# rll/rllab

Hardware: AMD Instinct MI355X
Metric: env steps/sec over full TRPO iterations (sample + process + update), 4096 envs per MI355X (higher is better)
Workload: dtype f32

## Files before the change

include/rllab_amd.h:

```cpp
#ifndef RLLAB_AMD_H
#define RLLAB_AMD_H

#include <stddef.h>
#include <stdint.h>

#ifdef __cplusplus
extern "C" {
#endif

enum rl_env_kind {
    RL_ENV_CARTPOLE = 0,
    RL_ENV_DOUBLE_PENDULUM = 1,
    RL_ENV_SWIMMER = 2,
    RL_ENV_HALF_CHEETAH = 3,
    RL_ENV_CARTPOLE_SWINGUP = 4,
    RL_ENV_WALKER2D = 5,
    RL_ENV_HOPPER = 6,
    RL_ENV_INVERTED_DOUBLE_PENDULUM = 7
};

enum rl_status {
    RL_OK = 0,
    RL_ERR_ARG = -1,
    RL_ERR_UNSUPPORTED = -2,
// ... 59 lines not shown
    double* reward_mean;
    double* reward_var;
    double obs_alpha, reward_alpha;
    int32_t normalize_obs, normalize_reward;
} rl_running_norm;

typedef struct rl_launch_opts {
    int32_t rollout_epw;
    int32_t rollout_wpb;
    int32_t swimmer_lane_kernel;
    int32_t swimmer_coop;
    int32_t two_leg_lane_kernel;
    int32_t two_leg_wave_kernel;
    int32_t fvp_split;
    int32_t fvp_split_wps;
    int32_t lfb_valu;
    int32_t reserved[7];
} rl_launch_opts;

typedef struct rl_rollout_args {
    int32_t kind;
    int32_t n_envs;
    int32_t horizon;
    int32_t max_path_length;
    int32_t normalize;
    int32_t reset_at_start;
    int32_t hidden0, hidden1;
    int32_t hidden2;
    int32_t env_offset;
    float scale_reward;
    float log_min_std;
    uint64_t seed;
    uint64_t step_counter;
    float* state;
    int32_t* ts;
    const float* theta;
    const float* eps;
    const float* reset_draws;
    float* obs;
    float* actions;
    float* means;
    float* rewards;
    uint8_t* dones;
    float* last_obs;
    const rl_env_cfg* cfg;
    const float* theta_std;
    float* log_stds;
    int32_t std_hidden0, std_hidden1, std_hidden2;
    int32_t layer_activations;
    const rl_launch_opts* opts;
    const rl_running_norm* norm;
    int32_t std_layer_activations;
    int32_t reserved_tail;
} rl_rollout_args;

int rl_rollout_gaussian_mlp(const rl_rollout_args* args, void* stream);

enum rl_rollout_kernel {
    RL_ROLLOUT_UNSUPPORTED = 0,
    RL_ROLLOUT_GENERIC = 1,
    RL_ROLLOUT_WIDE = 2,
    RL_ROLLOUT_DUAL = 3,
    RL_ROLLOUT_SWIMMER_QUAD = 4,
    RL_ROLLOUT_SWIMMER_QUAD_WIDE = 5,
    RL_ROLLOUT_SWIMMER_QUAD_COOP = 6,
    RL_ROLLOUT_TWO_LEG_WAVE = 7,
    RL_ROLLOUT_TWO_LEG_QUAD = 8,
    RL_ROLLOUT_TWO_LEG_QUAD_WIDE = 9
};
typedef struct rl_rollout_plan {
    int32_t kernel;
    int32_t envs_per_wavefront;
    int32_t wavefronts;
    int32_t wavefronts_per_workgroup;
    int32_t workgroups;
    int32_t lds_bytes;
    int32_t lds_limit;
    int32_t reserved;
    char name[96];
} rl_rollout_plan;
int rl_rollout_plan_query(const rl_rollout_args* args, rl_rollout_plan* plan);

int rl_rollout_lds_bytes(int env_kind, int hidden0, int hidden1, int hidden2, int std_hidden0, int std_hidden1,
                         int std_hidden2, size_t* bytes, size_t* limit);

typedef struct rl_population_args {
    int32_t kind;
    int32_t n_cand;
    int32_t n_evals;
    int32_t horizon;
    int32_t max_path_length;
    int32_t normalize;
    int32_t hidden;
    int32_t layer_activations;
    int32_t env_offset;
    float scale_reward;
    float log_min_std;
    int32_t reserved_pad;
    double discount;
    uint64_t seed;
    uint64_t step_counter;
    float* state;
    int32_t* ts;
    const float* theta_pop_T;
    const float* eps;
    const float* reset_draws;
// ... 157 lines not shown
                     const float* returns, const uint8_t* valid, void* workspace, size_t workspace_bytes,
                     double* out, int variant, void* stream);


size_t rl_reps_workspace_bytes(int T, int n);

int rl_reps_dual(int T, int n, int obs_dim, const float* obs, const float* rewards, const int32_t* tin,
                 const uint8_t* dones, const uint8_t* valid, double eta, const double* v_host, void* workspace,
                 size_t workspace_bytes, double* out, void* stream);

int rl_reps_weights(int T, int n, int obs_dim, const float* obs, const float* rewards, const int32_t* tin,
                    const uint8_t* dones, const uint8_t* valid, double eta, const double* v_host,
                    const double* dual_out, float* weights, void* stream);

typedef struct rl_policy_batch {
    int32_t n_samples;
    int32_t obs_dim, act_dim;
    int32_t hidden0, hidden1;
    int32_t hidden2;
    float inv_count;
    float log_min_std;
    const float* theta;
    const float* obs;
    const float* actions;
    const float* advantages;
    const float* old_means;
    const float* old_log_std;
    const float* weights;
    float* activations;
    float kl_penalty;
    int32_t activation;
    const rl_launch_opts* opts;
    int32_t layer_activations;
    int32_t reserved_pad;
    const int32_t* gate;
    float* obs_absmax;
} rl_policy_batch;

enum rl_activation { RL_ACT_TANH = 0, RL_ACT_RECTIFY = 1, RL_ACT_IDENTITY = 2 };

size_t rl_policy_workspace_bytes(int obs_dim, int act_dim, int hidden0, int hidden1, int hidden2);

size_t rl_policy_activation_bytes(int n_samples, int hidden0, int hidden1, int hidden2);

int rl_policy_loss_kl(const rl_policy_batch* batch, void* workspace, size_t workspace_bytes,
                      double* out4, void* stream);

int rl_policy_grad(const rl_policy_batch* batch, int vpg, void* workspace, size_t workspace_bytes,
                   double* grad_out, void* stream);

int rl_policy_grad_loss(const rl_policy_batch* batch, int vpg, void* workspace, size_t workspace_bytes,
                        double* grad_out, double* out4, void* stream);

int rl_policy_fvp(const rl_policy_batch* batch, const float* vec, void* workspace,
                  size_t workspace_bytes, double* fvp_out, void* stream);

int rl_policy_fvp_variant(const rl_policy_batch* batch);


int rl_mlp_forward(const rl_policy_batch* batch, const float* vec, float* out, float* dout, void* stream);
int rl_mlp_forward_ws(const rl_policy_batch* batch, const float* vec, void* workspace, size_t workspace_bytes, float* out,
                      float* dout, void* stream);

int rl_mlp_backward(const rl_policy_batch* batch, const float* cotangent, void* workspace, size_t workspace_bytes,
                    double* grad_out, void* stream);

size_t rl_gaussian_head_workspace_bytes(void);
int rl_gaussian_head(size_t n_samples, int act_dim, const float* mean, const float* log_std, const float* actions,
                     const float* advantages, const float* old_means, const float* old_log_stds,
                     const float* weights, float inv_count, float log_min_std, int vpg, float kl_penalty,
                     float* g_mean, float* g_log_std, void* workspace, size_t workspace_bytes, double* out4,
                     void* stream);

int rl_gaussian_fisher(size_t n_samples, int act_dim, const float* dmean, const float* dlog_std, const float* log_std,
                       const float* weights, float inv_count, float log_min_std, float* g_mean, float* g_log_std,
                       void* stream);

typedef struct rl_gridworld_args {
    int32_t n_envs, horizon, max_path_length, reset_at_start;
    int32_t n_row, n_col, n_act, start_state;
    int32_t env_offset, reserved;
    uint64_t seed, step_counter;
    const int8_t* cell;
    const float* prob;
    const float* u;
    int32_t* state;
    int32_t* ts;
    float* obs;
    float* actions;
    float* prob_out;
    float* rewards;
    uint8_t* dones;
} rl_gridworld_args;
int rl_rollout_gridworld(const rl_gridworld_args* args, void* stream);

typedef struct rl_gridworld_gru_args {
    int32_t n_envs, horizon, max_path_length, reset_at_start;
    int32_t n_row, n_col, n_act, start_state;
    int32_t env_offset, hidden, include_action, reserved;
    uint64_t seed, step_counter;
    const int8_t* cell;
    const float* theta;
    const float* u;
    int32_t* state;
    int32_t* ts;
    float* hidden_state;
// ... 62 lines not shown
```

profiles/make_index.py:

```python
#!/usr/bin/env python3
import fnmatch
import os
import subprocess

ROOT = os.path.dirname(os.path.dirname(os.path.abspath(__file__)))

RECIPES = [
    ("pmc_traffic.json", "HBM bytes + vector-instruction counters of the rollout kernels per workload, stamped with sha256(csrc/*); bench.py reads it",
     "profiles/run_profile.sh <tag> (traffic step: profiles/summarize.py traffic ...)"),
    ("gru_bptt_time.json", "loss + KL, gradient and Fisher-vector product of a GaussianGRUPolicy per call, and one whole TRPO update: the recurrent update kernels next to the float32 autograd closures, the sampler's batch for 4096 Cartpole envs, max_path_length 100 (105 rows x 4096 columns), 32 units",
     "python tools/exp/gru_bptt_time.py --out profiles/gru_bptt_time.json"),
    ("categorical_gru_bptt_time.json", "loss + KL, gradient and Fisher-vector product of a CategoricalGRUPolicy per call, and one whole TRPO update: the recurrent categorical update kernels next to the float32 autograd closures, the sampler's batch for 4096 GridWorld 4x4 envs, max_path_length 100, 32 units",
     "python tools/exp/categorical_gru_bptt_time.py --out profiles/categorical_gru_bptt_time.json"),
    ("update_batch_refactor_time.json", "parent commit against the update-batch / planes-ops refactor on one box, runs interleaved: headline bench (env steps/s, update phase) and whole TRPO iterations of GaussianMLPPolicy(adaptive_std=True) on Cartpole (1024 x 100) and CategoricalMLPPolicy on GridWorld (80 x 50); every run, medians, the parent's own spread",
     "python tools/exp/update_batch_refactor_ab.py --parent <built checkout of the parent> --out profiles/update_batch_refactor_time.json"),
    ("*_bench_line.json", "the default bench line of that tree", "python bench.py"),
    ("*_bench_under_rocprof.log", "bench stdout under the kernel-trace pass", "profiles/run_profile.sh <tag>"),
    ("*_c5_kernel_stats.csv", "kernel stats of C5's per-GPU shard", "profiles/run_profile.sh <tag> cheetah1024_trpo_gae"),
    ("*_c5_pmc_*.csv", "PMC passes of C5's per-GPU shard (one counter group per pass)", "profiles/run_profile.sh <tag> cheetah1024_trpo_gae"),
    ("*_c2_*.csv", "kernel stats / PMC passes of C2 (Cartpole 4096 envs, VPG)", "profiles/run_profile.sh <tag> cartpole4096_vpg"),
    ("r06_csplit_*.csv", "SQ counter passes / kernel stats of csplit_fvp_kernel on (100, 50, 25) and (128, 128) at 2.048 M samples", "tools/exp/r06_call8.sh"),
    ("r06_c7_csplit_ab.txt", "cooperative product per library: round start / one instruction stream per wavefront (off) / compile-time shapes + k-slices", "tools/exp/r06_call7.sh"),
    ("r06_c9_csplit_ab.txt", "cooperative product per library: k-slices + compile-time shapes / round start / + late fetch", "tools/exp/r06_call9.sh"),
    ("r06_c10_csplit_ab.txt", "cooperative product: the library of the round's start, timed in the call that ran the parity tests and the wide bench lines on the final one", "tools/exp/r06_call10.sh"),
    ("r06_f16_split.txt", "device facts of the two-way f16 split: subnormal inputs honoured, accuracy of five product forms against float64 over ten magnitude regimes, the five-instruction split bit for bit, instruction rates", "tools/ubench/f16_split.hip (tools/exp/r06_call15.sh)"),
    ("r06_c14_half*.txt", "what a two-part / three-term product would buy: RL_ABL_HALF timing ablation of the bf16 split kernels (wrong results)", "tools/exp/r06_call14.sh"),
    ("r06_c16_splith_ab*.txt", "fvp() per library: bf16 three-way / f16 two-way / ablations and variants of policy_splith_kernels.hip", "tools/exp/r06_call16.sh"),
    ("r06_c18_splith_check.txt", "two-way f16 / three-way bf16 / f32 products against float64 over shapes, direction and observation scales, with timings", "tools/exp/fvp_splith_check.py (tools/exp/r06_call18.sh)"),
    ("r06_c17_bench_*.json", "headline and C5 bench lines, f16 two-way (default) and bf16 three-way (RLLAB_FVP_SPLIT=5) interleaved in one call", "tools/exp/r06_call17.sh"),
    ("r06_c20_splith_ab_wide.txt", "fvp() of (20, 6) on (32, 32), 512 k samples: bf16 three-way against f16 two-way at one wavefront per SIMD", "tools/exp/r06_call20.sh"),
    ("r06_splith_*.csv", "SQ counter passes / FETCH_SIZE / kernel stats of the bf16 and the f16 split products, (32, 32) at 2.048 M and (64, 64) at 512 k samples", "tools/exp/r06_call19.sh"),
    ("curves/r06_splith_*", "learning under the f16 two-way and the bf16 three-way split products, same seeds; 1500-iteration soak", "tools/exp/r06_splith_curves.sh"),
    ("fvp_lds_tr_ab_product.txt", "fvp() of the parent and the new library swapped in alternately, (13, 2) on (32, 32) at 2.048 M samples: the unit operands transposed through LDS, and two variants not kept",
     "tools/exp/fvp_split_ab.py's loop with FVP_AB_WARM=400 FVP_AB_N=300 FVP_AB_READINGS=9, the parent as build/exp/lib_parent.so"),
    ("fvp_lds_tr_ab_bench.txt", "headline bench lines of the parent and the new library, interleaved, and their --dump-outputs compared", "tools/exp/lib_ab.py 'python bench.py --gpus 1 --steps 20 --warmup 3'"),
    ("fvp_lds_tr_*_pmc_product.csv", "one SQ counter pass over ten f16 split products at 2.048 M samples, parent / new library", "rocprofv3 --kernel-trace --pmc SQ_VALU_MFMA_BUSY_CYCLES SQ_INSTS_VALU SQ_ACTIVE_INST_VALU SQ_INSTS_LDS SQ_LDS_BANK_CONFLICT SQ_WAIT_INST_ANY SQ_WAVES GRBM_GUI_ACTIVE -- python tools/exp/fvp_splith_pmc.py 32"),
    ("perp_ab_bench.jsonl", "rollout launch, iteration time and headline of the parent and the new library (Swimmer sub-step without a materialised perpendicular), alternating in one session, parent first and last",
     "the two libraries swapped in place as tools/exp/lib_ab.py does, under 'python bench.py --gpus 1 --steps 20 --warmup 3', seven runs"),
    ("perp_before_kernel_stats.csv", "rocprofv3 --kernel-trace --stats summary of `bench.py --steps 5 --warmup 2`, the parent of the perpendicular-operand change", "profiles/run_profile.sh perp swimmer4096_trpo perp_before stats"),
    ("r06_c11_policy_time.txt", "wide loss / gradient / product passes with (.orig) and without (lib_before_wpf) the one-tile-ahead prefetch", "tools/exp/r06_call11.sh"),
    ("r06_wide_kernel_bench.txt", "loss / gradient / product passes of the wide nets at the final sources", "python tools/kernel_bench.py --configs ..."),
    ("*_split_kernel_stats.csv", "kernel stats of the three Fisher-vector-product kernels back to back", "tools/prof_split.sh"),
    ("*_split_pmc_*.csv", "PMC passes of the product kernels", "tools/prof_split.sh"),
    ("*_split64_*.csv", "kernel stats / PMC passes of the 64-unit split product", "tools/prof_split.sh 64"),
    ("*_wide*_pmc_*.csv", "PMC passes of the wide / deep kernels", "tools/prof_wide.sh"),
    ("*_wide*_stats.csv", "kernel stats of the wide / deep kernels", "tools/prof_wide.sh"),
    ("*_fvp_fixed_cost_stats.csv", "50 cached products back to back per batch size", "python tools/exp/fvp_fixed_cost.py under rocprofv3 --kernel-trace --stats"),
    ("*_step_kernel_roofline.jsonl", "rl_vecenv_step at 4 M envs, HIP-event timing", "python tools/step_kernel_roofline.py"),
    ("*_step_kernel_stats.csv", "the same under rocprofv3 --kernel-trace --stats", "profiles/run_profile.sh <tag>"),
    ("*_timeline.csv", "one iteration's dispatch timeline (start, duration, idle gap)", "profiles/run_profile.sh <tag> (summarize.py timeline)"),
    ("*_kernel_stats.csv", "rocprofv3 --kernel-trace --stats summary of `bench.py --steps 5 --warmup 2`", "profiles/run_profile.sh <tag>"),
    ("*_cheetah_pmc_*.csv", "PMC passes of the HalfCheetah shard", "profiles/run_profile.sh <tag> (cheetah leg)"),
    ("*_pmc_fetch_size.csv", "FETCH_SIZE pass (own run)", "profiles/run_profile.sh <tag>"),
    ("*_pmc_write_size.csv", "WRITE_SIZE pass (own run)", "profiles/run_profile.sh <tag>"),
    ("*_pmc_sq*.csv", "SQ_* counter passes (own runs)", "profiles/run_profile.sh <tag>"),
    ("*_bench_*.json", "side bench line: workload / size / switch in the file name", "python bench.py --workload ... | --n-envs ... | --hidden ... (tools/exp/r0N_final_bench.sh)"),
    ("*_resource_usage.txt", "-Rpass-analysis=kernel-resource-usage lines (registers, spills, LDS) of the named kernels", "tools/resource_usage.sh"),
    ("*_preflight*.json", "multi-GPU pre-flight record", "python tools/preflight_multigpu.py"),
    ("*_notes.md", "the round's measurements, experiments and dead ends in prose", "(written by hand from the files of that round)"),
    ("*_fallback_probe_*.txt", "which constructor options stay on the fused path, and the cost of an iteration (512 envs x 100 steps)",
     "python tools/exp/fallback_probe.py / tools/exp/fallback_probe_envs.py"),
    ("curves/r05_*", "tabular training logs of round 5's learning-curve runs", "tools/exp/r05_curves.sh, tools/exp/r05_call13.sh"),
    ("curves/*", "tabular training logs of the learning-curve runs", "tools/learning_curves.sh, tools/exp/r03_*curves*.sh"),
    ("run_profile.sh", "the profile recipe", "-"),
    ("summarize.py", "condenses rocprofv3 output directories into the CSVs kept here", "-"),
    ("make_index.py", "writes this index", "-"),
    ("INDEX.md", "this file", "python profiles/make_index.py"),
]
# ... 39 lines not shown
```

rllab_amd/_lib.py:

```python
import ctypes
import os

import torch

_HERE = os.path.dirname(os.path.abspath(__file__))
LIB_PATH = os.path.join(_HERE, "librllab_amd.so")

ENV_CARTPOLE = 0
ENV_DOUBLE_PENDULUM = 1
ENV_SWIMMER = 2
ENV_HALF_CHEETAH = 3
ENV_CARTPOLE_SWINGUP = 4
ENV_WALKER2D = 5
ENV_HOPPER = 6
ENV_INVERTED_DOUBLE_PENDULUM = 7

SYMBOLS = [
    "rl_last_error", "rl_abi_version", "rl_env_query", "rl_env_terminates", "rl_env_action_bounds", "rl_env_default_cfg", "rl_vecenv_com",
    "rl_vecenv_reset", "rl_vecenv_step", "rl_vecenv_step_graph", "rl_counter_add", "rl_vecenv_observe", "rl_rollout_gaussian_mlp", "rl_rollout_plan_query", "rl_rollout_lds_bytes", "rl_rollout_population", "rl_rollout_gaussian_gru",
    "rl_gru_workspace_bytes", "rl_gru_gaussian_eval", "rl_gru_gaussian_grad", "rl_gru_gaussian_fvp",
    "rl_gru_categorical_workspace_bytes", "rl_gru_categorical_eval", "rl_gru_categorical_grad", "rl_gru_categorical_fvp",
    "rl_rollout_population_gru", "rl_gae",
    "rl_discount_cumsum", "rl_debug_philox", "rl_policy_workspace_bytes", "rl_policy_activation_bytes", "rl_policy_loss_kl",
    "rl_policy_grad", "rl_policy_grad_loss", "rl_policy_fvp", "rl_policy_fvp_variant", "rl_policy_fvp_cg_step", "rl_cg_init", "rl_cg_step", "rl_trpo_step", "rl_line_search_point", "rl_line_search_decide", "rl_adam_step",
    "rl_path_scan", "rl_process_workspace_bytes", "rl_sample_stats_cols", "rl_sample_stats", "rl_adv_finish",
    "rl_lfb_normal_eq", "rl_reps_workspace_bytes", "rl_reps_dual", "rl_reps_weights",
    "rl_peer_mailbox_bytes", "rl_peer_alloc", "rl_peer_free", "rl_peer_export", "rl_peer_open", "rl_peer_close",
    "rl_peer_allreduce_sum",
    "rl_mlp_forward", "rl_mlp_forward_ws", "rl_mlp_backward", "rl_gaussian_head_workspace_bytes", "rl_gaussian_head", "rl_gaussian_fisher",
    "rl_rollout_gridworld", "rl_rollout_gridworld_gru", "rl_categorical_softmax", "rl_categorical_head_workspace_bytes", "rl_categorical_head",
    "rl_categorical_fisher", "rl_cmaes_cov_update",
]


class EnvCfg(ctypes.Structure):
    _fields_ = [
        ("ctrl_cost_coeff", ctypes.c_float), ("alive_coeff", ctypes.c_float), ("action_noise", ctypes.c_float),
        ("obs_noise", ctypes.c_float), ("frame_skip", ctypes.c_int32), ("flags", ctypes.c_int32),
        ("link_len", ctypes.c_float), ("reserved", ctypes.c_float), ("action_noise_z", ctypes.c_void_p), ("obs_noise_z", ctypes.c_void_p),
    ]


CFG_POLE_FOLLOWS_CART, CFG_FIXED_START, CFG_LIMIT_MUJOCO, CFG_CONTACT_MUJOCO = 1, 2, 4, 8


class RolloutArgs(ctypes.Structure):
    _fields_ = [
        ("kind", ctypes.c_int32), ("n_envs", ctypes.c_int32), ("horizon", ctypes.c_int32),
        ("max_path_length", ctypes.c_int32), ("normalize", ctypes.c_int32),
        ("reset_at_start", ctypes.c_int32), ("hidden0", ctypes.c_int32), ("hidden1", ctypes.c_int32),
        ("hidden2", ctypes.c_int32), ("env_offset", ctypes.c_int32), ("scale_reward", ctypes.c_float),
        ("log_min_std", ctypes.c_float), ("seed", ctypes.c_uint64), ("step_counter", ctypes.c_uint64),
        ("state", ctypes.c_void_p), ("ts", ctypes.c_void_p), ("theta", ctypes.c_void_p),
        ("eps", ctypes.c_void_p), ("reset_draws", ctypes.c_void_p), ("obs", ctypes.c_void_p),
        ("actions", ctypes.c_void_p), ("means", ctypes.c_void_p), ("rewards", ctypes.c_void_p),
        ("dones", ctypes.c_void_p), ("last_obs", ctypes.c_void_p), ("cfg", ctypes.POINTER(EnvCfg)),
        ("theta_std", ctypes.c_void_p), ("log_stds", ctypes.c_void_p), ("std_hidden0", ctypes.c_int32),
        ("std_hidden1", ctypes.c_int32), ("std_hidden2", ctypes.c_int32), ("layer_activations", ctypes.c_int32),
        ("opts", ctypes.c_void_p), ("norm", ctypes.c_void_p), ("std_layer_activations", ctypes.c_int32),
        ("reserved_tail", ctypes.c_int32),
    ]


class PopulationArgs(ctypes.Structure):
    _fields_ = [
        ("kind", ctypes.c_int32), ("n_cand", ctypes.c_int32), ("n_evals", ctypes.c_int32), ("horizon", ctypes.c_int32),
        ("max_path_length", ctypes.c_int32), ("normalize", ctypes.c_int32), ("hidden", ctypes.c_int32),
        ("layer_activations", ctypes.c_int32), ("env_offset", ctypes.c_int32), ("scale_reward", ctypes.c_float),
        ("log_min_std", ctypes.c_float), ("reserved_pad", ctypes.c_int32), ("discount", ctypes.c_double),
        ("seed", ctypes.c_uint64), ("step_counter", ctypes.c_uint64),
        ("state", ctypes.c_void_p), ("ts", ctypes.c_void_p), ("theta_pop_T", ctypes.c_void_p),
        ("eps", ctypes.c_void_p), ("reset_draws", ctypes.c_void_p), ("act_noise_z", ctypes.c_void_p),
        ("obs_noise_z", ctypes.c_void_p), ("obs", ctypes.c_void_p), ("actions", ctypes.c_void_p),
        ("means", ctypes.c_void_p), ("rewards", ctypes.c_void_p), ("dones", ctypes.c_void_p),
        ("first_path", ctypes.c_void_p), ("cfg", ctypes.POINTER(EnvCfg)), ("opts", ctypes.c_void_p),
    ]


class GruRolloutArgs(ctypes.Structure):
    _fields_ = [
        ("kind", ctypes.c_int32), ("n_envs", ctypes.c_int32), ("horizon", ctypes.c_int32),
        ("max_path_length", ctypes.c_int32), ("normalize", ctypes.c_int32), ("reset_at_start", ctypes.c_int32),
        ("hidden", ctypes.c_int32), ("include_action", ctypes.c_int32), ("env_offset", ctypes.c_int32),
        ("scale_reward", ctypes.c_float), ("seed", ctypes.c_uint64), ("step_counter", ctypes.c_uint64),
        ("state", ctypes.c_void_p), ("ts", ctypes.c_void_p), ("last_obs", ctypes.c_void_p),
        ("hidden_state", ctypes.c_void_p), ("prev_action", ctypes.c_void_p), ("theta", ctypes.c_void_p),
        ("eps", ctypes.c_void_p), ("reset_draws", ctypes.c_void_p), ("act_noise_z", ctypes.c_void_p),
        ("obs_noise_z", ctypes.c_void_p), ("obs", ctypes.c_void_p), ("actions", ctypes.c_void_p),
        ("means", ctypes.c_void_p), ("rewards", ctypes.c_void_p), ("dones", ctypes.c_void_p),
        ("cfg", ctypes.POINTER(EnvCfg)), ("opts", ctypes.c_void_p),
    ]


class GruBatch(ctypes.Structure):
    _fields_ = [
        ("n_envs", ctypes.c_int32), ("horizon", ctypes.c_int32), ("obs_dim", ctypes.c_int32), ("act_dim", ctypes.c_int32),
        ("hidden", ctypes.c_int32), ("include_action", ctypes.c_int32), ("inv_count", ctypes.c_double),
        ("theta", ctypes.c_void_p), ("obs", ctypes.c_void_p), ("actions", ctypes.c_void_p),
        ("advantages", ctypes.c_void_p), ("old_means", ctypes.c_void_p), ("old_log_std", ctypes.c_void_p),
        ("start", ctypes.c_void_p), ("weights", ctypes.c_void_p), ("means", ctypes.c_void_p),
        ("workspace", ctypes.c_void_p), ("workspace_bytes", ctypes.c_size_t),
    ]


class GruCategoricalBatch(ctypes.Structure):
    _fields_ = [
        ("n_envs", ctypes.c_int32), ("horizon", ctypes.c_int32), ("n_states", ctypes.c_int32), ("n_act", ctypes.c_int32),
        ("hidden", ctypes.c_int32), ("include_action", ctypes.c_int32), ("inv_count", ctypes.c_double),
        ("theta", ctypes.c_void_p), ("state", ctypes.c_void_p), ("action", ctypes.c_void_p),
        ("advantages", ctypes.c_void_p), ("old_prob", ctypes.c_void_p), ("start", ctypes.c_void_p),
        ("weights", ctypes.c_void_p), ("prob", ctypes.c_void_p), ("workspace", ctypes.c_void_p),
        ("workspace_bytes", ctypes.c_size_t),
    ]
# ... 121 lines not shown

def _load():
    if not os.path.exists(LIB_PATH):
        raise ImportError(
            "rllab_amd: %s is missing -- build it with `python -c 'import __graft_entry__ as g; g.build()'` "
            "(hipcc --offload-arch=gfx950).  There is no CPU fallback." % LIB_PATH)
    lib = ctypes.CDLL(LIB_PATH)
    vp, i32, u64, f32, f64 = ctypes.c_void_p, ctypes.c_int, ctypes.c_uint64, ctypes.c_float, ctypes.c_double
    u32 = ctypes.c_uint32
    ip = ctypes.POINTER(ctypes.c_int)
    fp = ctypes.POINTER(ctypes.c_float)
    lib.rl_last_error.restype = ctypes.c_char_p
    lib.rl_last_error.argtypes = []
    lib.rl_abi_version.restype = i32
    lib.rl_env_query.argtypes = [i32, ip, ip, ip, ip, ip]
    lib.rl_env_terminates.argtypes = [i32]
    lib.rl_env_action_bounds.argtypes = [i32, fp, fp]
    cfgp = ctypes.POINTER(EnvCfg)
    lib.rl_env_default_cfg.argtypes = [i32, cfgp]
    lib.rl_vecenv_com.argtypes = [i32, i32, vp, vp, vp]
    lib.rl_vecenv_reset.argtypes = [i32, i32, vp, vp, vp, vp, u64, u64, i32, cfgp, vp, vp]
    lib.rl_vecenv_observe.argtypes = [i32, i32, vp, vp, vp]
    lib.rl_vecenv_step_graph.argtypes = [i32, i32, i32, f32, i32, i32, vp, vp, vp, u64, vp, i32, cfgp, vp, vp, vp, vp]
    lib.rl_counter_add.argtypes = [vp, u64, vp]
    lib.rl_vecenv_step.argtypes = [i32, i32, i32, f32, i32, i32, vp, vp, vp, vp, u64, u64, i32, cfgp, vp, vp, vp, vp]
    lib.rl_rollout_gaussian_mlp.argtypes = [ctypes.POINTER(RolloutArgs), vp]
    lib.rl_rollout_plan_query.argtypes = [ctypes.POINTER(RolloutArgs), ctypes.POINTER(RolloutPlan)]
    lib.rl_rollout_lds_bytes.argtypes = [i32, i32, i32, i32, i32, i32, i32, ctypes.POINTER(ctypes.c_size_t),
                                         ctypes.POINTER(ctypes.c_size_t)]
    lib.rl_rollout_population.argtypes = [ctypes.POINTER(PopulationArgs), vp]
    lib.rl_rollout_gaussian_gru.argtypes = [ctypes.POINTER(GruRolloutArgs), vp]
    lib.rl_rollout_population_gru.argtypes = [ctypes.POINTER(PopulationGruArgs), vp]
    lib.rl_gru_workspace_bytes.restype = ctypes.c_size_t
    lib.rl_gru_workspace_bytes.argtypes = [i32, i32, i32, i32, i32, i32]
    lib.rl_gru_gaussian_eval.argtypes = [ctypes.POINTER(GruBatch), vp, vp]
    lib.rl_gru_gaussian_grad.argtypes = [ctypes.POINTER(GruBatch), vp, vp, vp]
    lib.rl_gru_gaussian_fvp.argtypes = [ctypes.POINTER(GruBatch), vp, vp, vp]
    lib.rl_gru_categorical_workspace_bytes.restype = ctypes.c_size_t
    lib.rl_gru_categorical_workspace_bytes.argtypes = [i32, i32, i32, i32, i32]
    lib.rl_gru_categorical_eval.argtypes = [ctypes.POINTER(GruCategoricalBatch), vp, vp]
    lib.rl_gru_categorical_grad.argtypes = [ctypes.POINTER(GruCategoricalBatch), vp, vp, vp]
    lib.rl_gru_categorical_fvp.argtypes = [ctypes.POINTER(GruCategoricalBatch), vp, vp, vp]
    lib.rl_gae.argtypes = [i32, i32, vp, vp, vp, f64, f64, vp, vp, vp, vp]
    lib.rl_discount_cumsum.argtypes = [i32, i32, vp, vp, f64, vp, vp]
    lib.rl_debug_philox.argtypes = [u32, u32, u32, u32, u32, u32, i32, vp, vp]
    pb = ctypes.POINTER(PolicyBatch)
    lib.rl_policy_workspace_bytes.restype = ctypes.c_size_t
    lib.rl_policy_workspace_bytes.argtypes = [i32, i32, i32, i32, i32]
    lib.rl_policy_activation_bytes.restype = ctypes.c_size_t
    lib.rl_policy_activation_bytes.argtypes = [i32, i32, i32, i32]
    lib.rl_policy_loss_kl.argtypes = [pb, vp, ctypes.c_size_t, vp, vp]
    lib.rl_policy_grad.argtypes = [pb, i32, vp, ctypes.c_size_t, vp, vp]
    lib.rl_policy_grad_loss.argtypes = [pb, i32, vp, ctypes.c_size_t, vp, vp, vp]
    lib.rl_policy_fvp.argtypes = [pb, vp, vp, ctypes.c_size_t, vp, vp]
    lib.rl_policy_fvp_variant.argtypes = [pb]
    lib.rl_policy_fvp_cg_step.argtypes = [pb, vp, ctypes.c_size_t, f64, f64, vp, vp, vp, vp, vp, vp, vp, vp]
    lib.rl_cg_init.argtypes = [i32, vp, vp, vp, vp, vp, vp, vp]
    lib.rl_cg_step.argtypes = [i32, vp, f64, f64, vp, vp, vp, vp, vp, vp]
    lib.rl_trpo_step.argtypes = [i32, vp, vp, vp, f64, f64, vp, vp, vp]
    lib.rl_line_search_point.argtypes = [i32, vp, vp, f64, vp, vp]
    lib.rl_line_search_decide.argtypes = [i32, vp, vp, f64, f64, i32, vp, vp, i32, vp, vp, f64, vp, vp]
    lib.rl_adam_step.argtypes = [i32, vp, vp, vp, vp, f64, f64, f64, f64, vp]
    sz = ctypes.c_size_t
    lib.rl_path_scan.argtypes = [i32, i32, i32, vp, vp, vp, i32, vp, vp, vp, vp]
    lib.rl_process_workspace_bytes.restype = sz
    lib.rl_process_workspace_bytes.argtypes = [i32]
    lib.rl_sample_stats_cols.restype = i32
    lib.rl_sample_stats.argtypes = [sz, vp, vp, vp, vp, vp, vp, f64, f64, vp, i32, vp, sz, vp, vp]
    lib.rl_adv_finish.argtypes = [sz, vp, vp, f64, f64, f64, vp, vp]
    lib.rl_lfb_normal_eq.argtypes = [sz, i32, vp, vp, vp, vp, vp, sz, vp, i32, vp]
    lib.rl_reps_workspace_bytes.restype = sz
    lib.rl_reps_workspace_bytes.argtypes = [i32, i32]
    lib.rl_reps_dual.argtypes = [i32, i32, i32, vp, vp, vp, vp, vp, f64, vp, vp, sz, vp, vp]
    lib.rl_reps_weights.argtypes = [i32, i32, i32, vp, vp, vp, vp, vp, f64, vp, vp, vp, vp]
    lib.rl_mlp_forward.argtypes = [pb, vp, vp, vp, vp]
    lib.rl_mlp_forward_ws.argtypes = [pb, vp, vp, sz, vp, vp, vp]
    lib.rl_mlp_backward.argtypes = [pb, vp, vp, sz, vp, vp]
    lib.rl_gaussian_head_workspace_bytes.restype = sz
    lib.rl_gaussian_head_workspace_bytes.argtypes = []
    lib.rl_gaussian_head.argtypes = [sz, i32, vp, vp, vp, vp, vp, vp, vp, f32, f32, i32, f32, vp, vp, vp, sz, vp, vp]
    lib.rl_gaussian_fisher.argtypes = [sz, i32, vp, vp, vp, vp, f32, f32, vp, vp, vp]
    lib.rl_rollout_gridworld.argtypes = [ctypes.POINTER(GridWorldArgs), vp]
    lib.rl_rollout_gridworld_gru.argtypes = [ctypes.POINTER(GridWorldGruArgs), vp]
    lib.rl_categorical_softmax.argtypes = [sz, i32, vp, vp, vp]
    lib.rl_categorical_head_workspace_bytes.restype = sz
    lib.rl_categorical_head_workspace_bytes.argtypes = []
    lib.rl_categorical_head.argtypes = [sz, i32, vp, vp, vp, vp, vp, f32, i32, f32, vp, vp, sz, vp, vp]
    lib.rl_categorical_fisher.argtypes = [sz, i32, vp, vp, vp, f32, vp, vp]
    lib.rl_cmaes_cov_update.argtypes = [i32, i32, i32, i32, vp, vp, vp, vp, vp, vp, vp, vp, vp, vp]
    vpp = ctypes.POINTER(ctypes.c_void_p)
    lib.rl_peer_mailbox_bytes.restype = sz
    lib.rl_peer_mailbox_bytes.argtypes = [i32, i32]
    lib.rl_peer_alloc.argtypes = [sz, vpp]
    lib.rl_peer_free.argtypes = [vp]
    lib.rl_peer_export.argtypes = [vp, vp]
    lib.rl_peer_open.argtypes = [vp, vpp]
    lib.rl_peer_close.argtypes = [vp]
    lib.rl_peer_allreduce_sum.argtypes = [i32, vp, i32, i32, vpp, i32, u64, vp, ctypes.c_int64, vp]
    for name in SYMBOLS:
        getattr(lib, name)
    return lib


lib = _load()


# ... 78 lines not shown
```

rllab_amd/csrc/env_kernels.hip:

```cpp
#include <hip/hip_runtime.h>
#include <stdlib.h>
#include <type_traits>
#include "../../include/rllab_amd.h"
#include "capi_util.h"
#include "device_rng.h"
#include "envs.h"
#include "policy_mfma.h"
#include "policy_wide.h"
#include "rollout_lane.h"

namespace rl {

constexpr int BLOCK = 64;

template <class Env>
__global__ void __launch_bounds__(BLOCK)
vecenv_reset_kernel(int n, float* __restrict__ state, int32_t* __restrict__ ts,
                    const uint8_t* __restrict__ mask, const float* __restrict__ draws, uint64_t seed,
                    uint64_t step, int env_offset, EnvCfg cfg, const float* __restrict__ obs_z,
                    float* __restrict__ obs) {
    int i = blockIdx.x * BLOCK + threadIdx.x;
    if (i >= n) return;
    if (mask && !mask[i]) return;
    float s[Env::STATE];
    load_state<Env>(state, n, i, s);
    reset_one<Env>(s, draws, n, i, seed, (uint32_t)(env_offset + i), step, cfg);
    store_state<Env>(state, n, i, s);
    ts[i] = 0;
    float o[Env::OBS];
    Env::template observe<float>(s, o);
    observed<Env>(o, cfg, obs_z, n, i, seed, (uint32_t)(env_offset + i), step);
#pragma unroll
    for (int k = 0; k < Env::OBS; ++k) obs[(size_t)k * n + i] = o[k];
}

template <class Env>
__global__ void __launch_bounds__(BLOCK)
vecenv_observe_kernel(int n, const float* __restrict__ state, float* __restrict__ obs) {
    int i = blockIdx.x * BLOCK + threadIdx.x;
    if (i >= n) return;
    float s[Env::STATE];
    load_state<Env>(state, n, i, s);
    float o[Env::OBS];
    Env::template observe<float>(s, o);
#pragma unroll
    for (int k = 0; k < Env::OBS; ++k) obs[(size_t)k * n + i] = o[k];
}

template <class Env>
__global__ void __launch_bounds__(BLOCK)
vecenv_com_kernel(int n, const float* __restrict__ state, float* __restrict__ com4) {
    int i = blockIdx.x * BLOCK + threadIdx.x;
    if (i >= n) return;
    float s[Env::STATE];
    load_state<Env>(state, n, i, s);
    float c[4];
    Env::template com<float>(s, c);
#pragma unroll
    for (int k = 0; k < 4; ++k) com4[(size_t)k * n + i] = c[k];
}

#ifndef RL_STEP_WPS
// ... 149 lines not shown
template <class Env, int H, bool ACTS = false>
struct RolloutPolicy16 {
    using N = Net<Env::OBS, Env::ACT, H>;
    static constexpr int DO = Env::OBS, DA = Env::ACT;
    static constexpr int NT = H / 16;
    static constexpr int KS0 = (DO + 1 + 3) / 4;
    static constexpr int KS1 = H / 4;

    float a0[NT][KS0];
    float a1[NT][KS1];
    float b1[NT][4];
    float w2[DA][NT][4];
    float b2[DA], lstd[DA];
    bool g0, g1, g2;
    int act0 = 0, act1 = 0;

    __device__ __forceinline__ void init(const float* __restrict__ th) {
        const int lane = threadIdx.x & 63, g = lane >> 4, n = lane & 15;
        g0 = g == 0; g1 = g == 1; g2 = g == 2;
#pragma unroll
        for (int t = 0; t < NT; ++t) {
#pragma unroll
            for (int m = 0; m < KS0; ++m) {
                const int d = 4 * m + g, u = 16 * t + n;
                a0[t][m] = d < DO ? th[N::W0 + d * H + u] : (d == DO ? th[N::B0 + u] : 0.0f);
            }
#pragma unroll
            for (int s_ = 0; s_ < KS1; ++s_)
                a1[t][s_] = th[N::W1 + (16 * (s_ / 4) + 4 * g + s_ % 4) * H + 16 * t + n];
#pragma unroll
            for (int j = 0; j < 4; ++j) {
                b1[t][j] = th[N::B1 + 16 * t + 4 * g + j];
#pragma unroll
                for (int k = 0; k < DA; ++k) w2[k][t][j] = th[N::W2 + (16 * t + 4 * g + j) * DA + k];
            }
        }
#pragma unroll
        for (int k = 0; k < DA; ++k) {
            b2[k] = th[N::B2 + k];
            lstd[k] = th[N::LSTD + k];
        }
    }

    __device__ __forceinline__ float log_std(int k) const { return lstd[k]; }

    __device__ __forceinline__ float pick(float c0, float c1, float c2, float c3) const {
        return g0 ? c0 : g1 ? c1 : g2 ? c2 : c3;
    }
    static __device__ __forceinline__ float input(const float* o, int d) {
        return d < DO ? o[d] : (d == DO ? 1.0f : 0.0f);
    }

    __device__ __forceinline__ void forward16(const float* o, float* mean) const {
        float xb[KS0];
#pragma unroll
        for (int m = 0; m < KS0; ++m)
            xb[m] = pick(input(o, 4 * m), input(o, 4 * m + 1), input(o, 4 * m + 2), input(o, 4 * m + 3));
        f32x4 h0[NT], h1[NT];
#pragma unroll
        for (int t = 0; t < NT; ++t) {
            f32x4 acc = {0.0f, 0.0f, 0.0f, 0.0f};
#pragma unroll
            for (int m = 0; m < KS0; ++m) acc = mfma16(a0[t][m], xb[m], acc);
#pragma unroll
            for (int j = 0; j < 4; ++j) h0[t][j] = ACTS ? act_one(acc[j], act0) : ftanh(acc[j]);
        }
#pragma unroll
        for (int t = 0; t < NT; ++t) {
            f32x4 acc;
#pragma unroll
            for (int j = 0; j < 4; ++j) acc[j] = b1[t][j];
#pragma unroll
            for (int s_ = 0; s_ < KS1; ++s_) acc = mfma16(a1[t][s_], h0[s_ / 4][s_ % 4], acc);
#pragma unroll
            for (int j = 0; j < 4; ++j) h1[t][j] = ACTS ? act_one(acc[j], act1) : ftanh(acc[j]);
        }
        float pm[DA];
#pragma unroll
        for (int k = 0; k < DA; ++k) {
            pm[k] = 0.0f;
#pragma unroll
            for (int t = 0; t < NT; ++t)
#pragma unroll
                for (int j = 0; j < 4; ++j) pm[k] = __builtin_fmaf(h1[t][j], w2[k][t][j], pm[k]);
        }
#pragma unroll
        for (int k = 0; k + 1 < DA; k += 2) {
            float s0, s1;
            group_sum2(pm[k], pm[k + 1], s0, s1);
            mean[k] = b2[k] + s0;
            mean[k + 1] = b2[k + 1] + s1;
        }
        if (DA & 1) mean[DA - 1] = b2[DA - 1] + group_sum(pm[DA - 1]);
    }
};

template <class Env>
struct RolloutPolicyWide {
    static constexpr int DO = Env::OBS, DA = Env::ACT;
    static constexpr int KS0 = (DO + 2) / 2;
    static constexpr int XROWS = 2 * KS0;
    WideShape s;
    float* f[WIDE_MAX_L];
    float* tail;
    float* xbuf;

    static size_t lds_floats(const WideShape& s, int threads) {
        size_t n = (size_t)s.HT[0] * KS0 * WV;
        for (int l = 1; l < s.L; ++l) n += (size_t)s.HT[l] * (s.H[l - 1] / 2) * WV;
        n += s.tail;
        n += (size_t)XROWS * threads;
// ... 275 lines not shown
                acc0 = mfma16(a0[0], b0[0], acc0);
                acc1 = mfma16(a0[1], b0[1], acc1);
                acc0 = mfma16(a0[2], b0[2], acc0);
                acc1 = mfma16(a0[3], b0[3], acc1);
                if (per == 8) {
                    acc0 = mfma16(a1[0], b1[0], acc0);
                    acc1 = mfma16(a1[1], b1[1], acc1);
                    acc0 = mfma16(a1[2], b1[2], acc0);
                    acc1 = mfma16(a1[3], b1[3], acc1);
                }
            } else {
                const int g0 = wave >> 1;
                const bool hi = (wave & 1) != 0;
                const f32x4 a0 = wov[g0 * 64], b0 = lv[g0 * 64];
                acc0 = mfma16(hi ? a0[2] : a0[0], hi ? b0[2] : b0[0], acc0);
                acc1 = mfma16(hi ? a0[3] : a0[1], hi ? b0[3] : b0[1], acc1);
            }
#pragma unroll
            for (int r = 0; r < 4; ++r)
                if (4 * q + r < DA) part[((4 * q + r) * 16 + n) * COOP_WAVES + wave] = acc0[r] + acc1[r];
        }
        __syncthreads();
#pragma unroll
        for (int k = 0; k < DA; ++k) {
            const f32x4 p = *reinterpret_cast<const f32x4*>(part + (k * 16 + n) * COOP_WAVES);
            mean[k] = tailo[k] + ((p[0] + p[1]) + (p[2] + p[3]));
        }
    }
};

struct RolloutDev {
    int n, T, max_path_length, normalize, reset_at_start, env_offset;
    float scale_reward, log_min_std;
    uint64_t seed, step_counter;
    float* state;
    int32_t* ts;
    const float* theta;
    const float* eps;
    const float* reset_draws;
    float* obs;
    float* actions;
    float* means;
    float* rewards;
    uint8_t* dones;
    float* last_obs;
    EnvCfg cfg;
    const float* act_noise_z;
    const float* obs_noise_z;
    float* log_stds;
    int act0, act1;
    double* nobs_mean; double* nobs_var; double* nrew_mean; double* nrew_var;
    double obs_alpha, rew_alpha;
    int norm_obs, norm_rew;
};

template <class Env>
struct RolloutPolicyDual {
    RolloutPolicyWide<Env> mean_net, std_net;
    static size_t lds_floats(const WideShape& ms, const WideShape& ss, int threads) {
        return RolloutPolicyWide<Env>::lds_floats(ms, threads) + RolloutPolicyWide<Env>::lds_floats(ss, threads);
    }
    __device__ __forceinline__ void init(float* smem, const float* __restrict__ th_mean, const WideShape& ms,
                                         const float* __restrict__ th_std, const WideShape& ss, size_t mean_floats) {
        mean_net.init(smem, th_mean, ms);
        std_net.init(smem + mean_floats, th_std, ss);
    }
    __device__ __forceinline__ float log_std(int) const { return 0.0f; }
    __device__ __forceinline__ void forward16(const float* o, float* mean) const { mean_net.forward16(o, mean); }
    __device__ __forceinline__ void forward(const float* o, float* mean) const { mean_net.forward(o, mean); }
    __device__ __forceinline__ void log_std16(const float* o, float* ls) const { std_net.forward16(o, ls); }
    __device__ __forceinline__ void log_std64(const float* o, float* ls) const { std_net.forward(o, ls); }
};
template <class P> struct state_std : std::false_type {};
template <class Env> struct state_std<RolloutPolicyDual<Env>> : std::true_type {};


constexpr int LANE_TPB = 256;

template <class Env, class Pol, int EPW, bool NORM = false>
__device__ __forceinline__ void rollout_body(const RolloutDev& a, const Pol& pol) {
    const int n = a.n, T = a.T;
    const int lane = threadIdx.x & 63;
    const int wave_global = blockIdx.x * (blockDim.x >> 6) + (threadIdx.x >> 6);
    const int i_raw = wave_global * EPW + (lane & (EPW - 1));
    const bool live = (i_raw < n) && (lane < EPW);
    const int i = (i_raw < n) ? i_raw : n - 1;
    const uint32_t env_global = (uint32_t)(a.env_offset + i);
    const size_t plane = (size_t)T * n;

    float std_[Env::ACT];
#pragma unroll
    for (int k = 0; k < Env::ACT; ++k) std_[k] = __expf(fmaxf(pol.log_std(k), a.log_min_std));

    float s[Env::STATE];
    load_state<Env>(a.state, n, i, s);
    int ts = a.ts[i];
    const size_t draws_slice = (size_t)Env::RESET_DRAWS * n;
    if (a.reset_at_start) {
        reset_one<Env>(s, a.reset_draws, n, i, a.seed, env_global, a.step_counter, a.cfg);
        ts = 0;
    }
    float o[Env::OBS];
    float zq[Env::ACT] = {};
    const size_t obs_z_slice = (size_t)Env::OBS * n;
    const bool resume_obs = !a.reset_at_start && a.last_obs != nullptr;
    if (resume_obs) {
// ... 128 lines not shown
    using Pol = typename std::conditional<EPW == 16, RolloutPolicy16<Env, H0, ACTS>, RolloutPolicy<Env, H0, ACTS>>::type;
    Pol pol;
    if constexpr (EPW == 16) {
        pol.init(a.theta);
        pol.act0 = a.act0; pol.act1 = a.act1;
    } else {
        __shared__ __attribute__((aligned(16))) float smem[RolloutPolicy<Env, H0, ACTS>::LDS_FLOATS];
        pol.init(smem, a.theta);
        pol.act0 = a.act0; pol.act1 = a.act1;
    }
    rollout_body<Env, Pol, EPW, NORM>(a, pol);
}

template <class Env, int EPW>
__global__ void __launch_bounds__(EPW == 16 ? LANE_TPB : BLOCK) rollout_wide_kernel(RolloutDev a, WideShape shape) {
    extern __shared__ __attribute__((aligned(16))) float wide_smem[];
    RolloutPolicyWide<Env> pol;
    pol.init(wide_smem, a.theta, shape);
    rollout_body<Env, RolloutPolicyWide<Env>, EPW>(a, pol);
}

template <class Env, int EPW>
__global__ void __launch_bounds__(EPW == 16 ? LANE_TPB : BLOCK) rollout_dual_kernel(RolloutDev a, WideShape mean_shape,
                                                                                    WideShape std_shape,
                                                                                    const float* __restrict__ theta_std,
                                                                                    int mean_floats) {
    extern __shared__ __attribute__((aligned(16))) float wide_smem[];
    RolloutPolicyDual<Env> pol;
    pol.init(wide_smem, a.theta, mean_shape, theta_std, std_shape, (size_t)mean_floats);
    rollout_body<Env, RolloutPolicyDual<Env>, EPW>(a, pol);
}

struct DppQuad {
    template <int CTRL> __device__ __forceinline__ float qp(float v) const {
        return __builtin_bit_cast(float, __builtin_amdgcn_update_dpp(0, __builtin_bit_cast(int, v), CTRL, 0xF, 0xF, true));
    }
};

__device__ __forceinline__ float prefix3(const DppQuad& x, float v, int b) {
    constexpr int PAR1 = 0x93;
    const float p1 = x.qp<PAR1>(v) + v;
    const float p2 = x.qp<PAR1>(p1) + v;
    return (b == 0) ? v : (b == 1) ? p1 : (b == 2) ? p2 : 0.0f;
}

constexpr int QUAD_ENVS = 16;
#ifndef RL_SWIMMER_SUBSTEP_UNROLL
#define RL_SWIMMER_SUBSTEP_UNROLL 5
#endif
#ifndef RL_TWO_LEG_SUBSTEP_UNROLL
#define RL_TWO_LEG_SUBSTEP_UNROLL 4
#endif

template <class Pol, bool COOP = false, bool PLAIN = false>
__device__ __forceinline__ void swimmer_quad_body(const RolloutDev& a, const Pol& pol) {
    using Env = Swimmer;
    using Chain = Env::Chain;

    const int n = a.n, T = a.T;
    const float* const eps = PLAIN ? nullptr : a.eps;
    const float* const reset_draws = PLAIN ? nullptr : a.reset_draws;
    const float action_noise = PLAIN ? 0.0f : a.cfg.action_noise;
    const int lane = threadIdx.x & 63;
    const int wave_global = COOP ? (int)blockIdx.x : (int)(blockIdx.x * (blockDim.x >> 6) + (threadIdx.x >> 6));
    const int el = lane & (QUAD_ENVS - 1);
    const int i_raw = wave_global * QUAD_ENVS + el;
    const bool live = (i_raw < n) && (lane < QUAD_ENVS) && (!COOP || threadIdx.x < 64);
    const int i = (i_raw < n) ? i_raw : n - 1;
    const uint32_t env_global = (uint32_t)(a.env_offset + i);
    const size_t plane = (size_t)T * n;
    const int q_src = lane >> 2, b = lane & 3;
    Chain::LaneConst<float> kc = Chain::lane_const<float>(b);
    asm volatile("" : "+v"(kc.lim_k), "+v"(kc.lim_b));
    const DppQuad dpp;

    float std_[Env::ACT];
#pragma unroll
    for (int k = 0; k < Env::ACT; ++k) std_[k] = __expf(fmaxf(pol.log_std(k), a.log_min_std));

    float s[Env::STATE];
    load_state<Env>(a.state, n, i, s);
    int ts = a.ts[i];
    const size_t draws_slice = (size_t)Env::RESET_DRAWS * n;
    if (a.reset_at_start) {
        reset_one<Env>(s, reset_draws, n, i, a.seed, env_global, a.step_counter, a.cfg);
        ts = 0;
    }
    float o[Env::OBS];
    float zq[Env::ACT] = {};
    Env::template observe<float>(s, o);
    const size_t obs_z_slice = (size_t)Env::OBS * n;
    if constexpr (!PLAIN) observed<Env>(o, a.cfg, a.obs_noise_z, n, i, a.seed, env_global, a.step_counter);

    uint32_t vo_obs[Env::OBS], vo_act[Env::ACT];
#pragma unroll
    for (int k = 0; k < Env::OBS; ++k) {
        vo_obs[k] = (uint32_t)(((size_t)k * plane + (size_t)i) * 4);
        asm volatile("" : "+v"(vo_obs[k]));
    }
#pragma unroll
    for (int k = 0; k < Env::ACT; ++k) {
        vo_act[k] = (uint32_t)(((size_t)k * plane + (size_t)i) * 4);
        asm volatile("" : "+v"(vo_act[k]));
    }
    uint32_t vo_row = (uint32_t)i * 4, vo_done = (uint32_t)i;
    asm volatile("" : "+v"(vo_row), "+v"(vo_done));
    typedef __attribute__((address_space(1))) float* global_f32;
    typedef __attribute__((address_space(1))) uint8_t* global_u8;
    auto at = [](uintptr_t row_ptr, uint32_t& byte_off) {
        asm volatile("" : "+v"(byte_off));
        return row_ptr + byte_off;
    };
    uintptr_t row_obs = reinterpret_cast<uintptr_t>(a.obs), row_act = reinterpret_cast<uintptr_t>(a.actions),
              row_mean = reinterpret_cast<uintptr_t>(a.means), row_rew = reinterpret_cast<uintptr_t>(a.rewards),
              row_done = reinterpret_cast<uintptr_t>(a.dones);
    const size_t row_bytes = (size_t)n * sizeof(float);

    Chain::Lane<float> ls;
    PlanarKin<float, 3> kin;
    float sn_b = 0.0f, cs_b = 1.0f;
    bool chain_valid = false;

    for (int t = 0; t < T; ++t) {
        asm volatile("" : "+s"(row_obs), "+s"(row_act), "+s"(row_mean), "+s"(row_rew), "+s"(row_done));
        float mean[Env::ACT], act[Env::ACT], z[Env::ACT];
        if (eps) {
#pragma unroll
            for (int k = 0; k < Env::ACT; ++k) z[k] = eps[k * plane + (size_t)t * n + i];
            landed<Env::ACT>(z);
        } else {
            if ((t & 3) == 0)
                philox_draws<Env::ACT, true>(zq, a.seed, env_global, a.step_counter + (uint64_t)(t + (lane >> 4)),
                                             RNG_POLICY);
#pragma unroll
            for (int k = 0; k < Env::ACT; ++k) z[k] = __shfl(zq[k], el + 16 * (t & 3), 64);
        }
        pol.forward16(o, mean);
#pragma unroll
        for (int k = 0; k < Env::ACT; ++k) act[k] = __builtin_fmaf(z[k], std_[k], mean[k]);
        if (live) {
#pragma unroll
            for (int k = 0; k < Env::OBS; ++k) *reinterpret_cast<global_f32>(at(row_obs, vo_obs[k])) = o[k];
#pragma unroll
            for (int k = 0; k < Env::ACT; ++k) {
                *reinterpret_cast<global_f32>(at(row_act, vo_act[k])) = act[k];
                *reinterpret_cast<global_f32>(at(row_mean, vo_act[k])) = mean[k];
            }
        }

        float eact[2], ctrl[3];
        if (action_noise != 0.0f) {
            float zn[Env::ACT], dact[Env::ACT];
            noise_draws<Env::ACT>(zn, a.act_noise_z ? a.act_noise_z + (size_t)t * Env::ACT * n : nullptr, n, i, a.seed,
                                  env_global, a.step_counter + (uint64_t)t, RNG_ACT_NOISE);
            action_perturbation<Env, float>(a.cfg, zn, dact);
            Env::template step_begin<float>(act, a.normalize, eact, ctrl, dact);
        } else {
            Env::template step_begin<float>(act, a.normalize, eact, ctrl);
        }
        {
            const float c1 = __shfl(ctrl[1], q_src, 64), c2 = __shfl(ctrl[2], q_src, 64);
            const float lact = (b == 1) ? c1 : (b == 2) ? c2 : 0.0f;
            if (!chain_valid) {
                float g[10];
#pragma unroll
                for (int k = 0; k < 10; ++k) g[k] = __shfl(s[k], q_src, 64);
                ls.r = V2<float>{g[0], g[1]};
                ls.v = V2<float>{g[5], g[6]};
                const float phi1 = g[2] + g[3], om1 = g[7] + g[8];
                const float phi2 = phi1 + g[4], om2 = om1 + g[9];
                const float phi = (b == 0) ? g[2] : (b == 1) ? phi1 : (b == 2) ? phi2 : 0.0f;
                ls.om = (b == 0) ? g[7] : (b == 1) ? om1 : (b == 2) ? om2 : 0.0f;
                ls.th = (b == 0) ? g[2] : (b == 1) ? g[3] : (b == 2) ? g[4] : 0.0f;
                rl_sincos(phi, sn_b, cs_b);
            } else {
                ls.om = prefix3(dpp, ls.qd, b);
                ls.th = (b < 3) ? ls.th : 0.0f;
            }
            ls.set_direction(cs_b, sn_b);
            ls.qd = Chain::joint_rate(dpp, ls.om);
#pragma unroll RL_SWIMMER_SUBSTEP_UNROLL
            for (int it = 0; it < Env::FRAME_SKIP; ++it)
                Chain::template substep_quad<float>(dpp, kc, ls, lact, 0.001f);
            rl_sincos(prefix3(dpp, ls.th, b), sn_b, cs_b);
            chain_valid = true;
            const int base = 4 * el;
            s[0] = __shfl(ls.r.x, base, 64);
            s[1] = __shfl(ls.r.y, base, 64);
            s[5] = __shfl(ls.v.x, base, 64);
            s[6] = __shfl(ls.v.y, base, 64);
#pragma unroll
            for (int j = 0; j < 3; ++j) {
                s[2 + j] = __shfl(ls.th, base + j, 64);
                s[7 + j] = __shfl(ls.qd, base + j, 64);
                kin.sn[j] = __shfl(sn_b, base + j, 64);
                kin.cs[j] = __shfl(cs_b, base + j, 64);
            }
        }
        float r;
        bool d;
        Env::template step_end_sc<float>(s, eact, kin, o, r, d, a.cfg.ctrl_cost_coeff);

        ts += 1;
        if (a.max_path_length > 0 && ts >= a.max_path_length) d = true;
        if (live) {
            *reinterpret_cast<global_f32>(at(row_rew, vo_row)) = r * a.scale_reward;
            *reinterpret_cast<global_u8>(at(row_done, vo_done)) = d ? 1 : 0;
        }
        row_obs += row_bytes; row_act += row_bytes; row_mean += row_bytes; row_rew += row_bytes; row_done += (size_t)n;
        if (d) {
            const float* dr = reset_draws ? reset_draws + (size_t)(t + 1) * draws_slice : nullptr;
            reset_one<Env>(s, dr, n, i, a.seed, env_global, a.step_counter + (uint64_t)t + 1, a.cfg);
            Env::template observe<float>(s, o);
            ts = 0;
        }
        if (__builtin_amdgcn_ballot_w64(d) != 0) chain_valid = false;
        if constexpr (!PLAIN)
            observed<Env>(o, a.cfg, a.obs_noise_z ? a.obs_noise_z + (size_t)(t + 1) * obs_z_slice : nullptr, n, i, a.seed,
                          env_global, a.step_counter + (uint64_t)t + 1);
    }
    if (live) {
        store_state<Env>(a.state, n, i, s);
        a.ts[i] = ts;
        if (a.last_obs) {
#pragma unroll
            for (int k = 0; k < Env::OBS; ++k) a.last_obs[(size_t)k * n + i] = o[k];
        }
    }
}

template <int H, bool ACTS = false, bool PLAIN = false>
__global__ void __launch_bounds__(LANE_TPB) rollout_swimmer_quad_kernel(RolloutDev a) {
    RolloutPolicy16<Swimmer, H, ACTS> pol;
    pol.init(a.theta);
    pol.act0 = a.act0; pol.act1 = a.act1;
    swimmer_quad_body<RolloutPolicy16<Swimmer, H, ACTS>, false, PLAIN>(a, pol);
}

__global__ void __launch_bounds__(LANE_TPB) rollout_swimmer_quad_wide_kernel(RolloutDev a, WideShape shape) {
    extern __shared__ __attribute__((aligned(16))) float wide_smem[];
    RolloutPolicyWide<Swimmer> pol;
    pol.init(wide_smem, a.theta, shape);
    swimmer_quad_body(a, pol);
}

__global__ void __launch_bounds__(64 * COOP_WAVES) rollout_swimmer_quad_coop_kernel(RolloutDev a, WideShape shape) {
    extern __shared__ __attribute__((aligned(16))) float wide_smem[];
    RolloutPolicyCoop<Swimmer> pol;
    pol.init(wide_smem, a.theta, shape);
    swimmer_quad_body<RolloutPolicyCoop<Swimmer>, true>(a, pol);
}

struct TwoLegQuadMoves {
    enum : int {
        UP = 0 | 0 << 2 | 1 << 4 | 2 << 6,
        DOWN = 1 | 2 << 2 | 3 << 4 | 3 << 6,
        NXT = 0 | 2 << 2 | 3 << 4 | 1 << 6,
        PRV = 0 | 3 << 2 | 1 << 4 | 2 << 6,
        ROOT = 0,
        FIRST = 1 | 1 << 2 | 1 << 4 | 1 << 6,
        OTHER_ROW_ROR8 = 0x128
    };
    template <int CTRL> __device__ __forceinline__ static float mv(float v) {
        return __builtin_bit_cast(float, __builtin_amdgcn_update_dpp(0, __builtin_bit_cast(int, v), CTRL, 0xF, 0xF, true));
    }
};
struct DppBodyLanes : TwoLegQuadMoves {
    bool is_root, is_leaf;
    __device__ __forceinline__ float up(float v) const { return mv<UP>(v); }
    __device__ __forceinline__ float down(float v) const { return mv<DOWN>(v); }
    __device__ __forceinline__ float nxt(float v) const { return mv<NXT>(v); }
    __device__ __forceinline__ float prv(float v) const { return mv<PRV>(v); }
    __device__ __forceinline__ float root(float v) const { return mv<ROOT>(v); }
    __device__ __forceinline__ float first(float v) const { return mv<FIRST>(v); }
    __device__ __forceinline__ float other(float v) const { return mv<OTHER_ROW_ROR8>(v); }
    __device__ __forceinline__ float sel_root(float a, float b) const { return is_root ? a : b; }
    __device__ __forceinline__ float sel_leaf(float a, float b) const { return is_leaf ? a : b; }
};
struct DppBodyPairs : TwoLegQuadMoves {
    using P = V2<float>;
    bool is_root, is_leaf;
    __device__ __forceinline__ P up(P v) const { return P{mv<UP>(v.x), mv<UP>(v.y)}; }
    __device__ __forceinline__ P down(P v) const { return P{mv<DOWN>(v.x), mv<DOWN>(v.y)}; }
    __device__ __forceinline__ P nxt(P v) const { return P{mv<NXT>(v.x), mv<NXT>(v.y)}; }
    __device__ __forceinline__ P prv(P v) const { return P{mv<PRV>(v.x), mv<PRV>(v.y)}; }
    __device__ __forceinline__ P root(P v) const { return P{mv<ROOT>(v.x), mv<ROOT>(v.y)}; }
    __device__ __forceinline__ P first(P v) const { return P{mv<FIRST>(v.x), mv<FIRST>(v.y)}; }
    __device__ __forceinline__ P other(P v) const { return v.yx; }
    __device__ __forceinline__ P sel_root(P a, P b) const { return is_root ? a : b; }
// ... 524 lines not shown
    int rc = device_cfg<Env>(cfg, c);
    if (rc) return rc;
    if constexpr (has_mjc<Env>::value && !is_mjc_env<Env>::value) {
        if (c.flags & (RL_CFG_LIMIT_MUJOCO | RL_CFG_CONTACT_MUJOCO))
            return launch_step<MjcEnv<Env>>(n, normalize, scale_reward, mpl, auto_reset, state, ts, actions, reset_draws, seed,
                                            step, step_dev, env_offset, cfg, obs, reward, done, st);
    }
    hipLaunchKernelGGL(vecenv_step_kernel<Env>, grid, dim3(BLOCK), 0, st, n, normalize, scale_reward, mpl,
                       auto_reset, state, ts, actions, reset_draws, seed, step, step_dev, env_offset, c,
                       cfg ? cfg->action_noise_z : nullptr, cfg ? cfg->obs_noise_z : nullptr, obs, reward, done);
    return check_launch("vecenv_step_kernel");
}

static const rl_launch_opts NO_OPTS = {};
static const char* env_name(int kind) {
    static const char* const names[] = {"Cartpole", "DoublePendulum", "Swimmer", "HalfCheetah", "CartpoleSwingup", "Walker2D",
                                        "Hopper", "InvertedDoublePendulum"};
    return (kind >= 0 && kind < 8) ? names[kind] : "?";
}

static int lane_group_wpb(int waves, const rl_launch_opts& o) {
    const int v = o.rollout_wpb;
    if (v == 1 || v == 2 || v == 4) return v;
    return waves <= 256 ? 1 : LANE_TPB / 64;
}

constexpr size_t LDS_LIMIT = 160 * 1024;
template <class LdsFn>
static int fit_wpb(int wpb, LdsFn lds_bytes) {
    for (; wpb >= 1; wpb >>= 1)
        if (lds_bytes(64 * wpb) <= LDS_LIMIT) return wpb;
    return 0;
}

template <class Env>
static size_t rollout_lds_bytes(int h0, int h1, int h2, int s0, int s1, int s2) {
    WideShape ms, ss;
    if (!wide_shape(Env::OBS, Env::ACT, h0, h1, h2, ms)) return 0;
    if (s0 == 0) return RolloutPolicyWide<Env>::lds_floats(ms, 64) * sizeof(float);
    if (!wide_shape(Env::OBS, Env::ACT, s0, s1, s2, ss)) return 0;
    return RolloutPolicyDual<Env>::lds_floats(ms, ss, 64) * sizeof(float);
}

static void plan_fill(rl_rollout_plan* p, int kernel, int epw, int waves, int wpb, size_t lds, const char* name) {
    p->kernel = kernel;
    p->envs_per_wavefront = epw;
    p->wavefronts = waves;
    p->wavefronts_per_workgroup = wpb;
    p->workgroups = wpb > 0 ? (waves + wpb - 1) / wpb : 0;
    p->lds_bytes = (int32_t)lds;
    p->lds_limit = (int32_t)LDS_LIMIT;
    p->reserved = 0;
    snprintf(p->name, sizeof(p->name), "%s", name);
}

template <class Env>
static int plan_rollout(const rl_rollout_args* g, rl_rollout_plan* p) {
    const rl_launch_opts& o = g->opts ? *g->opts : NO_OPTS;
    const int n = g->n_envs, T = g->horizon;
    const int cfg_flags = g->cfg ? g->cfg->flags : 0;
    plan_fill(p, RL_ROLLOUT_UNSUPPORTED, 0, 0, 0, 0, "");
    char nm[96];
    const bool equal = g->hidden2 == 0 && g->hidden0 == g->hidden1 && (g->hidden0 == 32 || g->hidden0 == 64);
    WideShape act_probe;
    act_probe.L = g->hidden2 > 0 ? 3 : 2;
    const bool wide_acts_ok = wide_activations(g->layer_activations, act_probe);
    WideShape std_probe;
    std_probe.L = g->std_hidden2 > 0 ? 3 : 2;
    const bool std_acts_ok = wide_activations(g->std_layer_activations, std_probe);
    if ((g->layer_activations != 0 && !wide_acts_ok && (!equal || g->theta_std != nullptr)) ||
        (g->theta_std != nullptr && !std_acts_ok))
        return set_error(RL_ERR_UNSUPPORTED, "rl_rollout_gaussian_mlp: rectify hidden layers run on the (32,32) / (64,64) "
                         "kernels only (and not next to a log-std network), identity layers on those and on the wide / two-"
                         "network kernels (hidden %d,%d,%d, layers 0x%x / 0x%x)", g->hidden0, g->hidden1, g->hidden2,
                         g->layer_activations, g->std_layer_activations);
    const bool small_offsets = (size_t)Env::OBS * (size_t)T * (size_t)n * 4 < ((size_t)1 << 32);
    const int epw_req = (o.rollout_epw == 16 || o.rollout_epw == 64) ? o.rollout_epw : 0;
    const int epw_generic = epw_req ? epw_req : (n <= 16 * 1024 ? 16 : 64);
    const bool norm = g->norm != nullptr && (g->norm->normalize_obs || g->norm->normalize_reward);
    if (norm) {
        if (!equal || g->theta_std != nullptr)
            return set_error(RL_ERR_UNSUPPORTED, "rl_rollout_gaussian_mlp: running observation / reward normalisation runs on "
                             "the (32,32) / (64,64) kernels only (hidden %d,%d,%d)", g->hidden0, g->hidden1, g->hidden2);
        if (!g->reset_at_start && !g->last_obs && g->state)
            return set_error(RL_ERR_ARG, "rl_rollout_gaussian_mlp: a continuation under running normalisation starts from "
                             "last_obs (the whitened observation the previous launch ended on)");
        if (g->cfg && g->cfg->obs_noise != 0.0f && g->norm->normalize_obs)
            return set_error(RL_ERR_UNSUPPORTED, "rl_rollout_gaussian_mlp: obs_noise together with normalize_obs is sampled "
                             "through rl_vecenv_step (the terminal observation's noise draw)");
        const int epw = epw_generic, waves = (n + epw - 1) / epw;
        snprintf(nm, sizeof(nm), "rollout_kernel<%s, %d, %d, %d, acts, norm>", env_name(Env::KIND), g->hidden0, g->hidden1, epw);
        plan_fill(p, RL_ROLLOUT_GENERIC, epw, waves, (epw == 16) ? lane_group_wpb(waves, o) : 1, 0, nm);
        return RL_OK;
    }
    if (g->theta_std != nullptr) {
        if (!g->log_stds) return set_error(RL_ERR_ARG, "rl_rollout_gaussian_mlp: theta_std without log_stds");
        WideShape ms, ss;
        if (!wide_shape(Env::OBS, Env::ACT, g->hidden0, g->hidden1, g->hidden2, ms) ||
            !wide_shape(Env::OBS, Env::ACT, g->std_hidden0, g->std_hidden1, g->std_hidden2, ss))
            return set_error(RL_ERR_UNSUPPORTED,
                             "rl_rollout_gaussian_mlp: mean net (%d,%d,%d) / log-std net (%d,%d,%d): each two or three tanh "
                             "layers of 32 / 64 / 128 units", g->hidden0, g->hidden1, g->hidden2, g->std_hidden0,
                             g->std_hidden1, g->std_hidden2);
        const int epw = epw_generic, waves = (n + epw - 1) / epw;
        const int wpb = fit_wpb((epw == 16) ? lane_group_wpb(waves, o) : 1, [&](int threads) {
            return RolloutPolicyDual<Env>::lds_floats(ms, ss, threads) * sizeof(float); });
        if (wpb == 0)
            return set_error(RL_ERR_UNSUPPORTED, "rollout of the two networks needs %zu B of LDS (a CU has %zu)",
                             RolloutPolicyDual<Env>::lds_floats(ms, ss, 64) * sizeof(float), LDS_LIMIT);
        snprintf(nm, sizeof(nm), "rollout_dual_kernel<%s, %d>", env_name(Env::KIND), epw);
        plan_fill(p, RL_ROLLOUT_DUAL, epw, waves, wpb, RolloutPolicyDual<Env>::lds_floats(ms, ss, 64 * wpb) * sizeof(float), nm);
        return RL_OK;
    }
    WideShape shape;
    const bool wide_ok = wide_shape(Env::OBS, Env::ACT, g->hidden0, g->hidden1, g->hidden2, shape);
    const int quad_waves = (n + QUAD_ENVS - 1) / QUAD_ENVS;
    if constexpr (std::is_same<Env, Swimmer>::value) {
        const bool lane_kernel = o.swimmer_lane_kernel == 1 || (cfg_flags & RL_CFG_LIMIT_MUJOCO) != 0;
        if (!lane_kernel && small_offsets && equal) {
            snprintf(nm, sizeof(nm), "rollout_swimmer_quad_kernel<%d>", g->hidden0);
            plan_fill(p, RL_ROLLOUT_SWIMMER_QUAD, QUAD_ENVS, quad_waves, lane_group_wpb(quad_waves, o), 0, nm);
            return RL_OK;
        }
        if (!lane_kernel && small_offsets && !equal && epw_req == 0 && wide_ok) {
            const size_t coop_lds = RolloutPolicyCoop<Env>::lds_floats(shape) * sizeof(float);
            const bool coop = o.swimmer_coop == 1 || (o.swimmer_coop != 2 && quad_waves * COOP_WAVES <= 1024);
            if (coop && coop_lds <= LDS_LIMIT) {
                plan_fill(p, RL_ROLLOUT_SWIMMER_QUAD_COOP, QUAD_ENVS, quad_waves * COOP_WAVES, COOP_WAVES, coop_lds,
                          "rollout_swimmer_quad_coop_kernel");
                return RL_OK;
            }
            const int wpb = fit_wpb(lane_group_wpb(quad_waves, o), [&](int threads) {
                return RolloutPolicyWide<Env>::lds_floats(shape, threads) * sizeof(float); });
            if (wpb > 0) {
                plan_fill(p, RL_ROLLOUT_SWIMMER_QUAD_WIDE, QUAD_ENVS, quad_waves, wpb,
                          RolloutPolicyWide<Env>::lds_floats(shape, 64 * wpb) * sizeof(float), "rollout_swimmer_quad_wide_kernel");
                return RL_OK;
            }
        }
    }
    if constexpr (std::is_same<Env, HalfCheetah>::value || std::is_same<Env, Walker2D>::value) {
        const bool lanes_on = o.two_leg_lane_kernel != 2 && epw_req == 0 &&
                              (cfg_flags & (RL_CFG_LIMIT_MUJOCO | RL_CFG_CONTACT_MUJOCO)) == 0;
        const bool wave_shape = o.two_leg_wave_kernel == 1 || (o.two_leg_wave_kernel != 2 && n <= 2048);
        if (lanes_on && wave_shape && small_offsets && equal) {
            snprintf(nm, sizeof(nm), "rollout_two_leg_wave_kernel<%s, %d>", env_name(Env::KIND), g->hidden0);
            plan_fill(p, RL_ROLLOUT_TWO_LEG_WAVE, 1, n, lane_group_wpb(n, o), 0, nm);
            return RL_OK;
        }
        if (lanes_on && small_offsets && n <= 16 * 1024 && equal) {
            snprintf(nm, sizeof(nm), "rollout_two_leg_quad_kernel<%s, %d>", env_name(Env::KIND), g->hidden0);
            plan_fill(p, RL_ROLLOUT_TWO_LEG_QUAD, QUAD_ENVS, quad_waves, lane_group_wpb(quad_waves, o), 0, nm);
            return RL_OK;
        }
        if (lanes_on && small_offsets && n <= 16 * 1024 && !equal && wide_ok) {
            const int wpb = fit_wpb(lane_group_wpb(quad_waves, o), [&](int threads) {
                return RolloutPolicyWide<Env>::lds_floats(shape, threads) * sizeof(float); });
            if (wpb > 0) {
                snprintf(nm, sizeof(nm), "rollout_two_leg_quad_wide_kernel<%s>", env_name(Env::KIND));
                plan_fill(p, RL_ROLLOUT_TWO_LEG_QUAD_WIDE, QUAD_ENVS, quad_waves, wpb,
                          RolloutPolicyWide<Env>::lds_floats(shape, 64 * wpb) * sizeof(float), nm);
                return RL_OK;
            }
        }
    }
    const int epw = epw_generic, waves = (n + epw - 1) / epw;
    int wpb = (epw == 16) ? lane_group_wpb(waves, o) : 1;
    if (equal) {
        snprintf(nm, sizeof(nm), "rollout_kernel<%s, %d, %d, %d>", env_name(Env::KIND), g->hidden0, g->hidden1, epw);
        plan_fill(p, RL_ROLLOUT_GENERIC, epw, waves, wpb, 0, nm);
        return RL_OK;
    }
    if (!wide_ok)
        return set_error(RL_ERR_UNSUPPORTED,
                         "rl_rollout_gaussian_mlp: hidden sizes (%d,%d,%d) have no fused kernel (two or three tanh "
                         "layers of 32 / 64 / 128 units each); use the per-step rl_vecenv_step path",
                         g->hidden0, g->hidden1, g->hidden2);
    wpb = fit_wpb(wpb, [&](int threads) { return RolloutPolicyWide<Env>::lds_floats(shape, threads) * sizeof(float); });
    if (wpb == 0)
        return set_error(RL_ERR_UNSUPPORTED, "wide rollout policy needs %zu B of LDS (a CU has %zu)",
                         RolloutPolicyWide<Env>::lds_floats(shape, 64) * sizeof(float), LDS_LIMIT);
    snprintf(nm, sizeof(nm), "rollout_wide_kernel<%s, %d>", env_name(Env::KIND), epw);
    plan_fill(p, RL_ROLLOUT_WIDE, epw, waves, wpb, RolloutPolicyWide<Env>::lds_floats(shape, 64 * wpb) * sizeof(float), nm);
    return RL_OK;
}

template <class K>
static int allow_big_lds(K kern, bool& done) {
    if (done) return 0;
    hipError_t e = hipFuncSetAttribute(reinterpret_cast<const void*>(kern), hipFuncAttributeMaxDynamicSharedMemorySize,
                                       160 * 1024);
    if (e != hipSuccess) return set_error(RL_ERR_HIP, "hipFuncSetAttribute: %s", hipGetErrorString(e));
    done = true;
    return 0;
}

template <class Env>
static int launch_rollout(const rl_rollout_args* g, hipStream_t st) {
    if constexpr (has_mjc<Env>::value && !is_mjc_env<Env>::value) {
        if (g->cfg && (g->cfg->flags & (RL_CFG_LIMIT_MUJOCO | RL_CFG_CONTACT_MUJOCO))) return launch_rollout<MjcEnv<Env>>(g, st);
    }
    rl_rollout_plan pl;
    int rc = plan_rollout<Env>(g, &pl);
    if (rc) return rc;
    RolloutDev a;
    a.n = g->n_envs; a.T = g->horizon; a.max_path_length = g->max_path_length;
    a.normalize = g->normalize; a.reset_at_start = g->reset_at_start; a.env_offset = g->env_offset;
    a.scale_reward = g->scale_reward; a.log_min_std = g->log_min_std;
    a.seed = g->seed; a.step_counter = g->step_counter;
    a.state = g->state; a.ts = g->ts; a.theta = g->theta; a.eps = g->eps; a.reset_draws = g->reset_draws;
    a.obs = g->obs; a.actions = g->actions; a.means = g->means; a.rewards = g->rewards; a.dones = g->dones;
    a.last_obs = g->last_obs;
    rc = device_cfg<Env>(g->cfg, a.cfg);
    if (rc) return rc;
    a.act_noise_z = g->cfg ? g->cfg->action_noise_z : nullptr;
    a.obs_noise_z = g->cfg ? g->cfg->obs_noise_z : nullptr;
    a.log_stds = g->log_stds;
    a.act0 = layer_act(RL_ACT_TANH, g->layer_activations, 0);
    a.act1 = layer_act(RL_ACT_TANH, g->layer_activations, 1);
    const bool acts = a.act0 != RL_ACT_TANH || a.act1 != RL_ACT_TANH;
    const bool norm = g->norm != nullptr && (g->norm->normalize_obs || g->norm->normalize_reward);
    a.norm_obs = a.norm_rew = 0;
    if (norm) {
        const rl_running_norm& q = *g->norm;
        if ((q.normalize_obs && (!q.obs_mean || !q.obs_var)) || (q.normalize_reward && (!q.reward_mean || !q.reward_var)))
            return set_error(RL_ERR_ARG, "rl_running_norm: null estimate array");
        a.nobs_mean = q.obs_mean; a.nobs_var = q.obs_var; a.nrew_mean = q.reward_mean; a.nrew_var = q.reward_var;
        a.obs_alpha = q.obs_alpha; a.rew_alpha = q.reward_alpha;
        a.norm_obs = q.normalize_obs ? 1 : 0; a.norm_rew = q.normalize_reward ? 1 : 0;
    }
    const dim3 grid(pl.workgroups), block(64 * pl.wavefronts_per_workgroup);
    const size_t lds = (size_t)pl.lds_bytes;
    const int H = g->hidden0, epw = pl.envs_per_wavefront;
    WideShape shape, sshape;
    if (wide_shape(Env::OBS, Env::ACT, g->hidden0, g->hidden1, g->hidden2, shape))
        wide_activations(g->layer_activations, shape);
    switch (pl.kernel) {
        case RL_ROLLOUT_DUAL: {
            wide_shape(Env::OBS, Env::ACT, g->std_hidden0, g->std_hidden1, g->std_hidden2, sshape);
            wide_activations(g->std_layer_activations, sshape);
            const size_t mean_floats = RolloutPolicyWide<Env>::lds_floats(shape, 64 * pl.wavefronts_per_workgroup);
            static bool a16 = false, a64 = false;
            if (epw == 16) {
                if ((rc = allow_big_lds(rollout_dual_kernel<Env, 16>, a16))) return rc;
                hipLaunchKernelGGL((rollout_dual_kernel<Env, 16>), grid, block, lds, st, a, shape, sshape, g->theta_std, (int)mean_floats);
            } else {
                if ((rc = allow_big_lds(rollout_dual_kernel<Env, 64>, a64))) return rc;
                hipLaunchKernelGGL((rollout_dual_kernel<Env, 64>), grid, block, lds, st, a, shape, sshape, g->theta_std, (int)mean_floats);
            }
            break;
        }
        case RL_ROLLOUT_GENERIC:
#define RL_GEN(HH, EE) do { if (norm) hipLaunchKernelGGL((rollout_kernel<Env, HH, HH, EE, true, true>), grid, block, 0, st, a); \
                            else if (acts) hipLaunchKernelGGL((rollout_kernel<Env, HH, HH, EE, true>), grid, block, 0, st, a); \
                            else hipLaunchKernelGGL((rollout_kernel<Env, HH, HH, EE, false>), grid, block, 0, st, a); } while (0)
            if (H == 32 && epw == 16) RL_GEN(32, 16);
            else if (H == 32) RL_GEN(32, 64);
            else if (epw == 16) RL_GEN(64, 16);
            else RL_GEN(64, 64);
#undef RL_GEN
            break;
        case RL_ROLLOUT_WIDE: {
            static bool a16 = false, a64 = false;
            if (epw == 16) {
                if ((rc = allow_big_lds(rollout_wide_kernel<Env, 16>, a16))) return rc;
                hipLaunchKernelGGL((rollout_wide_kernel<Env, 16>), grid, block, lds, st, a, shape);
            } else {
                if ((rc = allow_big_lds(rollout_wide_kernel<Env, 64>, a64))) return rc;
                hipLaunchKernelGGL((rollout_wide_kernel<Env, 64>), grid, block, lds, st, a, shape);
            }
            break;
        }
        default:
            if constexpr (std::is_same<Env, Swimmer>::value) {
                if (pl.kernel == RL_ROLLOUT_SWIMMER_QUAD) {
                    const bool plain = !a.eps && !a.reset_draws && !a.act_noise_z && !a.obs_noise_z &&
                                       a.cfg.action_noise == 0.0f && a.cfg.obs_noise == 0.0f;
#define RL_SWQ(HH, AA) do { if (plain) hipLaunchKernelGGL((rollout_swimmer_quad_kernel<HH, AA, true>), grid, block, 0, st, a); \
                            else hipLaunchKernelGGL((rollout_swimmer_quad_kernel<HH, AA, false>), grid, block, 0, st, a); } while (0)
                    if (H == 32 && !acts) RL_SWQ(32, false);
                    else if (H == 32) RL_SWQ(32, true);
                    else if (!acts) RL_SWQ(64, false);
                    else RL_SWQ(64, true);
#undef RL_SWQ
                    break;
                }
                if (pl.kernel == RL_ROLLOUT_SWIMMER_QUAD_COOP) {
                    static bool ca = false;
                    if ((rc = allow_big_lds(rollout_swimmer_quad_coop_kernel, ca))) return rc;
                    hipLaunchKernelGGL(rollout_swimmer_quad_coop_kernel, grid, block, lds, st, a, shape);
                    break;
                }
                if (pl.kernel == RL_ROLLOUT_SWIMMER_QUAD_WIDE) {
                    static bool wa = false;
                    if ((rc = allow_big_lds(rollout_swimmer_quad_wide_kernel, wa))) return rc;
                    hipLaunchKernelGGL(rollout_swimmer_quad_wide_kernel, grid, block, lds, st, a, shape);
                    break;
                }
            }
            if constexpr (std::is_same<Env, HalfCheetah>::value || std::is_same<Env, Walker2D>::value) {
                if (pl.kernel == RL_ROLLOUT_TWO_LEG_WAVE) {
                    if (H == 32 && !acts) hipLaunchKernelGGL((rollout_two_leg_wave_kernel<Env, 32, false>), grid, block, 0, st, a);
                    else if (H == 32) hipLaunchKernelGGL((rollout_two_leg_wave_kernel<Env, 32, true>), grid, block, 0, st, a);
                    else if (!acts) hipLaunchKernelGGL((rollout_two_leg_wave_kernel<Env, 64, false>), grid, block, 0, st, a);
                    else hipLaunchKernelGGL((rollout_two_leg_wave_kernel<Env, 64, true>), grid, block, 0, st, a);
                    break;
                }
                if (pl.kernel == RL_ROLLOUT_TWO_LEG_QUAD) {
                    if (H == 32 && !acts) hipLaunchKernelGGL((rollout_two_leg_quad_kernel<Env, 32, false>), grid, block, 0, st, a);
                    else if (H == 32) hipLaunchKernelGGL((rollout_two_leg_quad_kernel<Env, 32, true>), grid, block, 0, st, a);
                    else if (!acts) hipLaunchKernelGGL((rollout_two_leg_quad_kernel<Env, 64, false>), grid, block, 0, st, a);
                    else hipLaunchKernelGGL((rollout_two_leg_quad_kernel<Env, 64, true>), grid, block, 0, st, a);
                    break;
                }
                if (pl.kernel == RL_ROLLOUT_TWO_LEG_QUAD_WIDE) {
                    static bool ta = false;
                    if ((rc = allow_big_lds(rollout_two_leg_quad_wide_kernel<Env>, ta))) return rc;
                    hipLaunchKernelGGL((rollout_two_leg_quad_wide_kernel<Env>), grid, block, lds, st, a, shape);
                    break;
                }
            }
            return set_error(RL_ERR_UNSUPPORTED, "rollout plan %d has no launch for this env", pl.kernel);
    }
    return check_launch(pl.name);
}

}

using namespace rl;

template <class Env>
static void fill_default_cfg(rl_env_cfg* cfg) {
    const EnvCfg c = default_cfg<Env, float>();
// ... 117 lines not shown
```

rllab_amd/csrc/policy_splith_kernels.hip:

```cpp
#include <hip/hip_runtime.h>
#include <cstdlib>
#include "../../include/rllab_amd.h"
#include "capi_util.h"
#include "policy_mfma.h"
#include "lds_tr_image.h"

namespace rl {

int launch_reduce_rows(const float* partial, int rows, int cols, double* out, hipStream_t st);

namespace splith {

typedef _Float16 f16;
typedef __attribute__((ext_vector_type(8))) _Float16 f16x8;
typedef __attribute__((ext_vector_type(4))) _Float16 f16x4;
typedef __attribute__((ext_vector_type(2))) _Float16 f16x2;
typedef __attribute__((ext_vector_type(2))) float f32x2;
typedef __attribute__((ext_vector_type(4))) float f32x4;
typedef __attribute__((address_space(1))) const void* gptr_t;
typedef __attribute__((address_space(3))) void* lptr_t;

struct Args {
    int B;
    const float* theta;
    const float* vec;
    const float* acts;
    const float* obs;
    const float* weight;
    const float* xmax;
    float inv_count;
    float log_min_std;
    float* partial;
};

struct PB { f16x8 hi, lo; };
struct PA { f16x8 hi, lo, hs; };

#ifndef RL_ABL_FETCH
#define RL_ABL_FETCH 0
#endif
#ifndef RL_ABL_MFMA
#define RL_ABL_MFMA 0
#endif
#ifndef RL_ABL_SPLIT
#define RL_ABL_SPLIT 0
#endif
#ifndef RL_ABL_TRANSPOSE
#define RL_ABL_TRANSPOSE 0
#endif

__device__ __forceinline__ f32x16 mf(f16x8 a, f16x8 b, f32x16 c) {
#if RL_ABL_MFMA
    asm volatile("" : "+v"(c) : "v"(a), "v"(b));
    return c;
#else
    return __builtin_amdgcn_mfma_f32_32x32x16_f16(a, b, c, 0, 0, 0);
#endif
}
__device__ __forceinline__ f32x16 mm_ab(const PA& A, const PB& b, f32x16 c) {
    c = mf(A.hs, b.lo, c);
    c = mf(A.lo, b.hi, c);
    c = mf(A.hi, b.hi, c);
    return c;
}
__device__ __forceinline__ void mm_bb(const PB& a, const PB& b, f32x16& c0, f32x16& c1) {
    c1 = mf(a.hi, b.lo, c1);
    c1 = mf(a.lo, b.hi, c1);
    c0 = mf(a.hi, b.hi, c0);
}
__device__ __forceinline__ PA as_image(const PB& a) {
    const f16 k = (f16)0.00048828125f;
    PA r;
    r.hi = a.hi; r.lo = a.lo * k; r.hs = a.hi * k;
    return r;
}

__device__ __forceinline__ float half_sum_swap(float v) {
    const auto r = __builtin_amdgcn_permlane32_swap(__float_as_uint(v), __float_as_uint(v), false, false);
    return __uint_as_float(r[0]) + __uint_as_float(r[1]);
}

#ifndef RL_SPLITH_MIX
#define RL_SPLITH_MIX 1
#endif
__device__ __forceinline__ void split_pair(float a0, float a1, PB& out, int j) {
// ... 104 lines not shown
    for (int kb = 0; kb < 2; ++kb) {
        *reinterpret_cast<f16x8*>(w + lds_tr::TR_KB_STORE * kb) = f[kb].hi;
        *reinterpret_cast<f16x8*>(w + lds_tr::TR_PART_BYTES + lds_tr::TR_KB_STORE * kb) = f[kb].lo;
    }
}
__device__ __forceinline__ f16x8 tr_read8(const char* r) {
    typedef short v4i16 __attribute__((vector_size(8)));
    typedef __attribute__((address_space(3))) v4i16* lp_t;
    const f16x4 t0 = __builtin_bit_cast(f16x4, __builtin_amdgcn_ds_read_tr16_b64_v4i16((lp_t)r));
    const f16x4 t1 = __builtin_bit_cast(f16x4, __builtin_amdgcn_ds_read_tr16_b64_v4i16((lp_t)(r + lds_tr::TR_T_READ)));
    return __builtin_shufflevector(t0, t1, 0, 1, 2, 3, 4, 5, 6, 7);
}
__device__ __forceinline__ void tr_load(const char* r, PB (&out)[2]) {
#pragma unroll
    for (int kb = 0; kb < 2; ++kb) {
        out[kb].hi = tr_read8(r + lds_tr::TR_KB_READ * kb);
        out[kb].lo = tr_read8(r + lds_tr::TR_PART_BYTES + lds_tr::TR_KB_READ * kb);
    }
}
template <int KB0>
__device__ __forceinline__ void transpose_inputs(const PB (&f)[KB0], const f16x8 (&Idx)[KB0], PB (&out)[2]) {
#if RL_ABL_TRANSPOSE
    out[0] = f[0]; out[1] = f[KB0 - 1];
    return;
#endif
    f32x16 d;
#pragma unroll
    for (int r = 0; r < 16; ++r) d[r] = 0.0f;
#pragma unroll
    for (int kb = 0; kb < KB0; ++kb) d = mf(f[kb].hi, Idx[kb], d);
    pack_exact(d, out[0].hi, out[1].hi);
#pragma unroll
    for (int r = 0; r < 16; ++r) d[r] = 0.0f;
#pragma unroll
    for (int kb = 0; kb < KB0; ++kb) d = mf(f[kb].lo, Idx[kb], d);
    pack_exact(d, out[0].lo, out[1].lo);
}

__device__ __forceinline__ f32x2 pair_of(const f32x16& v, int j) { return f32x2{v[2 * j], v[2 * j + 1]}; }
__device__ __forceinline__ void set_pair(f32x16& v, int j, f32x2 p) { v[2 * j] = p[0]; v[2 * j + 1] = p[1]; }
__device__ __forceinline__ void times_dtanh(const f32x16& acc, const f32x16& h, f32x16& out, float k = 1.0f) {
#pragma unroll
    for (int j = 0; j < 8; ++j) {
        const f32x2 hh = pair_of(h, j);
        const f32x2 d = __builtin_elementwise_fma(-hh, hh, f32x2{1.0f, 1.0f});
        set_pair(out, j, k == 1.0f ? pair_of(acc, j) * d : (pair_of(acc, j) * f32x2{k, k}) * d);
    }
}

__device__ __forceinline__ int exp_of(float x) {
    const int e = (int)((__float_as_uint(x) >> 23) & 255u) - 126;
    return e < -30 ? -30 : e;
}
__device__ __forceinline__ float pow2(int e) { return __builtin_ldexpf(1.0f, e < -126 ? -126 : (e > 127 ? 127 : e)); }
__device__ __forceinline__ float uniform(float v) { return __uint_as_float(__builtin_amdgcn_readfirstlane(__float_as_uint(v))); }
__device__ __forceinline__ int imin(int a, int b) { return a < b ? a : b; }
__device__ __forceinline__ int imax(int a, int b) { return a > b ? a : b; }
struct Scales {
    float sx;
    float sb;
    float sv0;
    float sv0b;
    float sw1;
    float s1;
    float eg2;
    float kg;
    float u1;
    float u0;
    float u0b;
};
template <int HL, int DAL>
__device__ __forceinline__ Scales make_scales(float bx, float bv0, float bv1, float bv2, float bw1, float bw2, float fkmax) {
    const int Ex = exp_of(fmaxf(bx, 1.0f)), Ev0 = exp_of(bv0), Ev1 = exp_of(bv1), Ev2 = exp_of(bv2), EW1 = exp_of(bw1),
              EW2 = exp_of(bw2), Efk = exp_of(fkmax);
    const int e_x = 6 - exp_of(bx), e_b = imin(e_x, 5), e_w1 = 7 - EW1;
    const int xt = e_x <= 5 ? 11 : 1 + imax(11, e_x);
    const int e_v0 = imin(15 - xt - Ev0, 14 - Ev1 - e_w1 - e_x);
    const int s0 = e_v0 + e_x, s1 = s0 + e_w1;
    const int EZ0 = 5 + Ev0 + Ex;
    const int EZ1 = 1 + imax(HL + 1 + Ev1, HL + EW1 + EZ0);
    const int EM = 1 + imax(HL + 1 + Ev2, HL + EW2 + EZ1);
    const int EG1 = DAL + EW2 + EM + Efk;
    int sg = 15 - EG1;
    sg = sg < -100 ? -100 : (sg > 100 ? 100 : sg);
    const int kg = -(HL + 7);
    Scales s;
    s.sx = uniform(pow2(e_x)); s.sb = uniform(pow2(e_b)); s.sv0 = uniform(pow2(e_v0)); s.sv0b = uniform(pow2(e_v0 + e_x - e_b));
    s.sw1 = uniform(pow2(e_w1)); s.s1 = uniform(pow2(s1));
    s.eg2 = uniform(pow2(sg - s1)); s.kg = uniform(pow2(kg));
    s.u1 = uniform(pow2(-sg)); s.u0 = uniform(pow2(-(sg + e_w1 + kg + e_x + 8)));
    s.u0b = uniform(pow2(-(sg + e_w1 + kg + e_b + 8)));
    return s;
}
template <class N, int NT>
__device__ __forceinline__ void block_maxima(const float* __restrict__ th, const float* __restrict__ vc, float* red,
                                             float (&m)[5]) {
#pragma unroll
    for (int i = 0; i < 5; ++i) m[i] = 0.0f;
    constexpr int PER = (N::LSTD + NT - 1) / NT;
    float vv[PER], ww[PER];
#pragma unroll
    for (int i = 0; i < PER; ++i) {
        const int e = threadIdx.x + i * NT, ec = e < N::LSTD ? e : N::LSTD - 1;
        vv[i] = vc[ec];
        ww[i] = (e >= N::W1 && e < N::B2) ? th[ec] : 0.0f;
    }
#pragma unroll
    for (int i = 0; i < PER; ++i) {
        const int e = threadIdx.x + i * NT;
        const float v = e < N::LSTD ? fabsf(vv[i]) : 0.0f, w = fabsf(ww[i]);
        if (e < N::W1) m[0] = fmaxf(m[0], v);
        else if (e < N::W2) m[1] = fmaxf(m[1], v);
        else m[2] = fmaxf(m[2], v);
        if (e >= N::W1 && e < N::B1) m[3] = fmaxf(m[3], w);
        if (e >= N::W2 && e < N::B2) m[4] = fmaxf(m[4], w);
    }
    const int wave = threadIdx.x / WV, lane = threadIdx.x % WV;
#pragma unroll
    for (int i = 0; i < 5; ++i) {
        m[i] = wave_max(m[i]);
        if (lane == 0) red[wave * 5 + i] = m[i];
    }
    __syncthreads();
#pragma unroll
    for (int i = 0; i < 5; ++i) {
        float v = 0.0f;
#pragma unroll
        for (int w = 0; w < NT / WV; ++w) v = fmaxf(v, red[w * 5 + i]);
        m[i] = v;
    }
}
__host__ __device__ constexpr int ceil_log2(int n) { return n <= 1 ? 0 : n <= 2 ? 1 : n <= 4 ? 2 : 3; }

constexpr int H = 32;
constexpr int LAND_BYTES = 2 * H * TS * 4;
constexpr int ops_count(int kb0) { return kb0 + 6; }
constexpr int ops_bytes(int kb0) { return ops_count(kb0) * 3 * WV * 16; }
#ifndef RL_SPLITH_TWO_ACC
#define RL_SPLITH_TWO_ACC 0
#endif
#ifndef RL_SPLITH_TWO_ACC_W0
#define RL_SPLITH_TWO_ACC_W0 0
#endif
constexpr float XT_SCALE = 256.0f;

template <int DO, int DA, int WPS>
__global__ void __launch_bounds__(4 * WPS * WV, 1) fvp_splith_kernel(Args a) {
    using N = Net<DO, DA, H>;
    constexpr int P = N::P;
    constexpr int WAVES = 4 * WPS;
    constexpr int KB0 = (DO + 1 + 15) / 16;
    constexpr int N_OPS = ops_count(KB0), OPS_BYTES = ops_bytes(KB0);
    constexpr int TAILV = 16 * DA * 2 + 16;
    constexpr int SPILL_BYTES = 2 * lds_tr::TR_PART_BYTES;
    constexpr int XPIECES = (DO + 1 + 7) / 8;
    constexpr int XLAND_BYTES = XPIECES * WV * 16;
    constexpr int WAVE_BYTES = LAND_BYTES + SPILL_BYTES + XLAND_BYTES;
    constexpr int LDS_TOTAL = WAVES * WAVE_BYTES + OPS_BYTES + 2 * TAILV * 4 + WAVES * 5 * 4;
    static_assert(DO + 1 <= 32 && (DA <= 2 || WPS == 1), "two k-blocks of inputs + the bias slot; thin heads at two per SIMD");
    static_assert(LDS_TOTAL >= WAVES * P * 4 && LDS_TOTAL <= 160 * 1024, "LDS budget; the fold rows alias the landing zones");
    extern __shared__ __attribute__((aligned(16))) char smem[];
    const int wave = threadIdx.x / WV, lane = threadIdx.x % WV;
    const int lj = lane & 31, lh = lane >> 5;
    char* const land = smem + wave * WAVE_BYTES;
    char* const spill = land + LAND_BYTES;
    char* const xland = spill + SPILL_BYTES;
    char* const tr_w = spill + lds_tr::tr_store_lane(lane);
    const char* const tr_r = spill + lds_tr::tr_read_lane(lane);
    char* const ops = smem + WAVES * WAVE_BYTES;
    float* const tailv = reinterpret_cast<float*>(ops + OPS_BYTES);
    float* const red = tailv + 2 * TAILV;

    const int B = a.B;
    const int n_tiles = B / TS;
    const int wave_global = blockIdx.x * WAVES + wave;
    const int waves_total = gridDim.x * WAVES;

    const unsigned xland_lds = __builtin_amdgcn_readfirstlane((unsigned)(size_t)(lptr_t)xland);
    auto fetch = [&](int tile) {
#pragma unroll
        for (int p = 0; p < XPIECES; ++p) {
            const int d = 8 * p + (lane >> 3);
            const float* g = (d < DO ? a.obs + (size_t)d * B : a.weight) + tile * TS + 4 * (lane & 7);
            asm volatile("s_mov_b32 m0, %1\n\tglobal_load_lds_dwordx4 %0, off" :: "v"(g), "s"(xland_lds + p * (WV * 16)) : "memory");
        }
    };
    const unsigned land_lds = __builtin_amdgcn_readfirstlane((unsigned)(size_t)(lptr_t)land);
    auto fetch_acts = [&](int tile) {
        const float* src = a.acts + ((size_t)tile * 8 * WV + lane) * 4;
        asm volatile("s_mov_b32 m0, %2\n\t"
                     "global_load_lds_dwordx4 %0, off\n\t"
                     "global_load_lds_dwordx4 %0, off offset:1024\n\t"
                     "global_load_lds_dwordx4 %0, off offset:2048\n\t"
                     "global_load_lds_dwordx4 %0, off offset:3072\n\t"
                     "s_mov_b32 m0, %3\n\t"
                     "global_load_lds_dwordx4 %1, off\n\t"
                     "global_load_lds_dwordx4 %1, off offset:1024\n\t"
                     "global_load_lds_dwordx4 %1, off offset:2048\n\t"
                     "global_load_lds_dwordx4 %1, off offset:3072"
                     :: "v"(src), "v"(src + 4 * WV * 4), "s"(land_lds), "s"(land_lds + 4096u) : "memory");
    };
    if (wave_global < n_tiles) {
        fetch(wave_global);
        fetch_acts(wave_global);
    }
    asm volatile("" ::: "memory");

    const float* __restrict__ th = a.theta;
    const float* __restrict__ vc = a.vec;
    float db2[DA], fkS[DA], var_[DA];
    bool floored[DA];
    float fkmax = 0.0f;
#pragma unroll
    for (int k = 0; k < DA; ++k) {
        const float raw = th[N::LSTD + k];
        floored[k] = raw < a.log_min_std;
        const float ls = fmaxf(raw, a.log_min_std);
        var_[k] = __expf(2.0f * ls);
        fkS[k] = 2.0f / (2.0f * var_[k] + 1e-8f) * a.inv_count;
        fkmax = fmaxf(fkmax, fkS[k]);
    }
    float mx[5];
    block_maxima<N, WAVES * WV>(th, vc, red, mx);
    const Scales S = make_scales<5, ceil_log2(DA)>(*a.xmax, mx[0], mx[1], mx[2], mx[3], mx[4], fkmax);
#pragma unroll
    for (int k = 0; k < DA; ++k) {
        fkS[k] *= S.eg2;
        db2[k] = vc[N::B2 + k] * S.s1;
    }

    for (int o = wave; o < N_OPS; o += WAVES) {
        float t[8];
#pragma unroll
        for (int j = 0; j < 8; ++j) {
            if (o < KB0) {
                const int d = 16 * o + 8 * lh + j;
                t[j] = d < DO ? vc[N::W0 + d * H + lj] * S.sv0 : (d == DO ? vc[N::B0 + lj] * S.sv0b : 0.0f);
            } else {
                const int q = o - KB0, kb = q & 1, u = frag_unit(8 * kb + j, lh);
                t[j] = q < 2 ? vc[N::W1 + u * H + lj] * S.s1
                     : q < 4 ? th[N::W1 + u * H + lj] * S.sw1
                             : th[N::W1 + lj * H + u] * S.sw1;
            }
        }
        const PA im = image8(t);
        *reinterpret_cast<f16x8*>(ops + ((o * 3 + 0) * WV + lane) * 16) = im.hi;
        *reinterpret_cast<f16x8*>(ops + ((o * 3 + 1) * WV + lane) * 16) = im.lo;
        *reinterpret_cast<f16x8*>(ops + ((o * 3 + 2) * WV + lane) * 16) = im.hs;
    }
    for (int e = threadIdx.x; e < 2 * 16; e += WAVES * WV) {
        const int hh = e / 16, r = e % 16, u = frag_unit(r, hh);
        float* tv = tailv + hh * TAILV;
#pragma unroll
        for (int k = 0; k < DA; ++k) {
            tv[k * 16 + r] = th[N::W2 + u * DA + k];
            tv[(DA + k) * 16 + r] = vc[N::W2 + u * DA + k] * S.s1;
        }
        tv[2 * DA * 16 + r] = vc[N::B1 + u] * S.s1;
    }
    __syncthreads();
    auto op = [&](int o) -> PA {
        PA t;
        t.hi = *reinterpret_cast<const f16x8*>(ops + ((o * 3 + 0) * WV + lane) * 16);
        t.lo = *reinterpret_cast<const f16x8*>(ops + ((o * 3 + 1) * WV + lane) * 16);
        t.hs = *reinterpret_cast<const f16x8*>(ops + ((o * 3 + 2) * WV + lane) * 16);
        return t;
    };
    auto chain_ahead = [&](int base, int nb, const PB* Bk, f32x16 acc_, PA& cur, int nxt_o) -> f32x16 {
#pragma unroll
        for (int kb = 0; kb < 2; ++kb) {
            if (kb < nb) {
                PA nxtp = cur;
                const int o = kb + 1 < nb ? base + kb + 1 : nxt_o;
                if (o >= 0) nxtp = op(o);
                __builtin_amdgcn_sched_barrier(0);
                acc_ = mm_ab(cur, Bk[kb], acc_);
                cur = nxtp;
            }
        }
        return acc_;
    };
    f16x8 Idx[KB0];
#pragma unroll
    for (int j = 0; j < 8; ++j)
#pragma unroll
        for (int kb = 0; kb < KB0; ++kb) Idx[kb][j] = (f16)(16 * kb + 8 * lh + j == lj ? XT_SCALE : 0.0f);

    f32x16 gW1, gW0, gW1c, gW0c;
    float gW2l[16][DA], gb1l[16], gb2[DA], wsum = 0.0f;
#pragma unroll
    for (int r = 0; r < 16; ++r) {
        gW1[r] = 0.0f; gW0[r] = 0.0f; gW1c[r] = 0.0f; gW0c[r] = 0.0f; gb1l[r] = 0.0f;
#pragma unroll
        for (int k = 0; k < DA; ++k) gW2l[r][k] = 0.0f;
    }
#pragma unroll
    for (int k = 0; k < DA; ++k) gb2[k] = 0.0f;

    __builtin_amdgcn_s_waitcnt(0x0F70);
    for (int tile = wave_global; tile < n_tiles; tile += waves_total) {
        asm volatile("s_waitcnt vmcnt(0)" ::: "memory");
        f32x16 h0, h1;
#pragma unroll
        for (int q = 0; q < 4; ++q) {
            const f32x4 v0 = *reinterpret_cast<const f32x4*>(land + (q * WV + lane) * 16);
            const f32x4 v1 = *reinterpret_cast<const f32x4*>(land + ((4 + q) * WV + lane) * 16);
#pragma unroll
            for (int e = 0; e < 4; ++e) { h0[4 * q + e] = v0[e]; h1[4 * q + e] = v1[e]; }
        }
        float xb[KB0][8], wgt;
        {
            const float* xl = reinterpret_cast<const float*>(xland) + lj;
#pragma unroll
            for (int kb = 0; kb < KB0; ++kb)
#pragma unroll
                for (int j = 0; j < 8; ++j) {
                    const int d = 16 * kb + 8 * lh + j;
                    const float v = xl[32 * (d < DO ? d : DO)];
                    xb[kb][j] = d < DO ? v * S.sx : (d == DO ? S.sb : 0.0f);
                }
            wgt = xl[32 * DO];
        }
        asm volatile("s_waitcnt lgkmcnt(0)" ::: "memory");
        {
            const int nxt = tile + waves_total < n_tiles ? tile + waves_total : tile;
#if !RL_ABL_FETCH
            fetch(nxt);
            fetch_acts(nxt);
#else
            (void)nxt;
#endif
        }
        const float* tv = tailv + lh * TAILV;
        auto stage = [&]() { asm volatile("" ::: "memory"); };

        PA opcur = op(0);
        __builtin_amdgcn_sched_barrier(0);
        PB Xs[KB0], H0s[2];
#pragma unroll
        for (int kb = 0; kb < KB0; ++kb) split8(xb[kb], Xs[kb]);
        split_frag(h0, H0s);

        f32x16 acc;
#pragma unroll
        for (int r = 0; r < 16; ++r) acc[r] = 0.0f;
        acc = chain_ahead(0, KB0, Xs, acc, opcur, KB0);
        f32x16 dh0;
        times_dtanh(acc, h0, dh0);
#pragma unroll
        for (int r = 0; r < 16; ++r) acc[r] = tv[2 * DA * 16 + r];
        acc = chain_ahead(KB0, 2, H0s, acc, opcur, KB0 + 2);
        wave_sync();
        tr_store(tr_w, H0s);
        stage();
        {
            PB D0s[2];
            split_frag(dh0, D0s);
            acc = chain_ahead(KB0 + 2, 2, D0s, acc, opcur, -1);
        }
        stage();
        f32x16 dz1, gz1;
        float gmu[DA];
#pragma unroll
        for (int j = 0; j < 8; ++j) {
            const f32x2 hh = pair_of(h1, j);
            const f32x2 d = __builtin_elementwise_fma(-hh, hh, f32x2{1.0f, 1.0f});
            set_pair(dz1, j, d);
            set_pair(acc, j, pair_of(acc, j) * d);
        }
        auto rows_of = [&](int which, int k, f32x4 (&out_)[4]) {
#pragma unroll
            for (int q = 0; q < 4; ++q) out_[q] = *reinterpret_cast<const f32x4*>(tv + (which * DA + k) * 16 + 4 * q);
        };
#pragma unroll
        for (int k = 0; k < DA; ++k) {
            f32x4 wq[4], dq[4];
            rows_of(0, k, wq);
            rows_of(1, k, dq);
            f32x2 pa[2], pb[2];
            pa[0] = pa[1] = pb[0] = pb[1] = f32x2{0.0f, 0.0f};
#pragma unroll
            for (int j = 0; j < 8; ++j) {
                const int q = j >> 1, e = 2 * (j & 1);
                pa[j & 1] = __builtin_elementwise_fma(pair_of(h1, j), f32x2{dq[q][e], dq[q][e + 1]}, pa[j & 1]);
                pb[j & 1] = __builtin_elementwise_fma(pair_of(acc, j), f32x2{wq[q][e], wq[q][e + 1]}, pb[j & 1]);
            }
            const f32x2 pd = (pa[0] + pb[0]) + (pa[1] + pb[1]);
            const float dmu = db2[k] + half_sum_swap(pd[0] + pd[1]);
            gmu[k] = wgt * (dmu * fkS[k]);
        }
        if (lh == 0) {
            wsum += wgt * a.inv_count;
#pragma unroll
            for (int k = 0; k < DA; ++k) gb2[k] += gmu[k];
        }
        stage();
        {
            f32x2 g[8];
#pragma unroll
            for (int j = 0; j < 8; ++j) g[j] = f32x2{0.0f, 0.0f};
#pragma unroll
            for (int k = 0; k < DA; ++k) {
                f32x4 wq[4];
                rows_of(0, k, wq);
                const f32x2 gk = {gmu[k], gmu[k]};
#pragma unroll
                for (int j = 0; j < 8; ++j) {
                    const int q = j >> 1, e = 2 * (j & 1);
                    g[j] = __builtin_elementwise_fma(f32x2{wq[q][e], wq[q][e + 1]}, gk, g[j]);
                    const f32x2 w2 = __builtin_elementwise_fma(pair_of(h1, j), gk, f32x2{gW2l[2 * j][k], gW2l[2 * j + 1][k]});
                    gW2l[2 * j][k] = w2[0]; gW2l[2 * j + 1][k] = w2[1];
                }
            }
#pragma unroll
            for (int j = 0; j < 8; ++j) {
                const f32x2 gz = g[j] * pair_of(dz1, j);
                set_pair(gz1, j, gz);
                const f32x2 b1n = f32x2{gb1l[2 * j], gb1l[2 * j + 1]} + gz;
                gb1l[2 * j] = b1n[0]; gb1l[2 * j + 1] = b1n[1];
            }
        }
        stage();
        opcur = op(KB0 + 4);
        __builtin_amdgcn_sched_barrier(0);
        PB G1s[2], H0t[2], G1t[2];
        split_frag(gz1, G1s);
#pragma unroll
        for (int r = 0; r < 16; ++r) acc[r] = 0.0f;
        acc = chain_ahead(KB0 + 4, 2, G1s, acc, opcur, -1);
        wave_sync();
        tr_load(tr_r, H0t);
        wave_sync();
        tr_store(tr_w, G1s);
        wave_sync();
        tr_load(tr_r, G1t);
        __builtin_amdgcn_sched_barrier(0);
        stage();
        f32x16 gz0;
        times_dtanh(acc, h0, gz0, S.kg);
        {
            PB G0s[2], G0t[2], Xt[2];
            split_frag(gz0, G0s);
            wave_sync();
            tr_store(tr_w, G0s);
            wave_sync();
            tr_load(tr_r, G0t);
            __builtin_amdgcn_sched_barrier(0);
#pragma unroll
            for (int kb = 0; kb < 2; ++kb) {
#if RL_SPLITH_TWO_ACC
                mm_bb(H0t[kb], G1t[kb], gW1, gW1c);
#else
                gW1 = mm_ab(as_image(H0t[kb]), G1t[kb], gW1);
#endif
            }
            transpose_inputs<KB0>(Xs, Idx, Xt);
#pragma unroll
            for (int kb = 0; kb < 2; ++kb) {
#if RL_SPLITH_TWO_ACC_W0
                mm_bb(Xt[kb], G0t[kb], gW0, gW0c);
#else
                gW0 = mm_ab(as_image(Xt[kb]), G0t[kb], gW0);
#endif
            }
        }
    }
    asm volatile("s_waitcnt vmcnt(0)" ::: "memory");

    float b1s[16], w2s[16][DA];
#pragma unroll
    for (int r = 0; r < 16; ++r) {
        float v = gb1l[r];
#pragma unroll
        for (int o = 16; o > 0; o >>= 1) v += __shfl_xor(v, o, WV);
        b1s[r] = v;
#pragma unroll
        for (int k = 0; k < DA; ++k) {
            float w = gW2l[r][k];
#pragma unroll
            for (int o = 16; o > 0; o >>= 1) w += __shfl_xor(w, o, WV);
            w2s[r][k] = w;
        }
    }
    float b2s[DA];
#pragma unroll
    for (int k = 0; k < DA; ++k) b2s[k] = wave_sum(gb2[k]);
    const float ws = wave_sum(wsum);
    __syncthreads();
    float* const myrow = reinterpret_cast<float*>(smem) + wave * P;
    constexpr float CROSS = 0.00048828125f;
#pragma unroll
    for (int r = 0; r < 16; ++r) {
        const int u = frag_unit(r, lh);
        myrow[N::W1 + u * H + lj] = __builtin_fmaf(gW1c[r], CROSS, gW1[r]) * S.u1;
        const float g0 = __builtin_fmaf(gW0c[r], CROSS, gW0[r]);
        if (u < DO) myrow[N::W0 + u * H + lj] = g0 * S.u0;
        else if (u == DO) myrow[N::B0 + lj] = g0 * S.u0b;
    }
    if (lj == 0) {
#pragma unroll
        for (int r = 0; r < 16; ++r) {
            const int u = frag_unit(r, lh);
            myrow[N::B1 + u] = b1s[r] * S.u1;
#pragma unroll
            for (int k = 0; k < DA; ++k) myrow[N::W2 + u * DA + k] = w2s[r][k] * S.u1;
        }
    }
    if (lane == 0) {
#pragma unroll
        for (int k = 0; k < DA; ++k) {
            myrow[N::B2 + k] = b2s[k] * S.u1;
            const float vv = var_[k], e = 1e-8f;
            const float cc = floored[k] ? 0.0f : 4.0f * vv * (2.0f * vv - e) / ((2.0f * vv + e) * (2.0f * vv + e));
            myrow[N::LSTD + k] = cc * vc[N::LSTD + k] * ws;
        }
    }
    __syncthreads();
    float* row = a.partial + (size_t)blockIdx.x * P;
    for (int k = threadIdx.x; k < P; k += WAVES * WV) {
        float t = 0.0f;
#pragma unroll
        for (int w = 0; w < WAVES; ++w) t += reinterpret_cast<const float*>(smem)[w * P + k];
        row[k] = t;
    }
}

template <int DO, int DA>
__global__ void __launch_bounds__(4 * WV, 1) fvp_splith64_kernel(Args a) {
    constexpr int HT = 2, HH = 64;
    using N = Net<DO, DA, HH>;
    constexpr int P = N::P;
    constexpr int WAVES = 4;
    constexpr int KB0 = (DO + 1 + 15) / 16;
    constexpr int KBH = 2 * HT;
    constexpr int O_DW0 = 0, O_DW1 = O_DW0 + HT * KB0, O_W1T = O_DW1 + HT * KBH, O_W1 = O_W1T + HT * KBH,
                  N_OPS = O_W1 + HT * KBH;
    constexpr int OPS_BYTES = N_OPS * 3 * WV * 16;
    constexpr int TAILV = HT * 16 * DA * 2 + HT * 16;
    constexpr int LAND64 = 2 * HH * TS * 4;
    constexpr int GMU_BYTES = TS * 8 * 4;
    constexpr int WAVE_BYTES = LAND64 + GMU_BYTES;
    constexpr int LDS_TOTAL = WAVES * WAVE_BYTES + OPS_BYTES + 2 * TAILV * 4 + WAVES * 5 * 4;
    static_assert(DO + 1 <= 32 && DA <= 8, "two k-blocks of inputs + the bias slot; at most eight actions");
    static_assert(LDS_TOTAL >= WAVES * P * 4 && LDS_TOTAL <= 160 * 1024, "LDS budget; the fold rows alias everything");
    extern __shared__ __attribute__((aligned(16))) char smem[];
    const int wave = threadIdx.x / WV, lane = threadIdx.x % WV;
    const int lj = lane & 31, lh = lane >> 5;
    char* const land = smem + wave * WAVE_BYTES;
    float* const gmub = reinterpret_cast<float*>(land + LAND64);
    char* const ops = smem + WAVES * WAVE_BYTES;
    float* const tailv = reinterpret_cast<float*>(ops + OPS_BYTES);
    float* const red = tailv + 2 * TAILV;

    const int B = a.B;
    const int n_tiles = B / TS;
    const int wave_global = blockIdx.x * WAVES + wave;
    const int waves_total = gridDim.x * WAVES;

    auto fetch = [&](int tile, float (&xq)[KB0][8], float& wq) {
        const int b = tile * TS + lj;
        wq = a.weight[b];
#pragma unroll
        for (int kb = 0; kb < KB0; ++kb)
#pragma unroll
            for (int j = 0; j < 8; ++j) {
                const int d = 16 * kb + 8 * lh + j;
                xq[kb][j] = a.obs[(size_t)(d < DO ? d : DO - 1) * B + b];
            }
    };
    auto fetch_acts = [&](int tile) {
        const float* src = a.acts + ((size_t)tile * (4 * 2 * HT) * WV + lane) * 4;
#pragma unroll
        for (int q = 0; q < 4 * 2 * HT; ++q)
            __builtin_amdgcn_global_load_lds((gptr_t)(src + q * WV * 4), (lptr_t)(land + q * WV * 16), 16, 0, 0);
    };
    float xb[KB0][8], xb_next[KB0][8];
// ... 382 lines not shown
    constexpr int KB0 = (DO + 1 + 15) / 16;
    constexpr int LDS_BYTES = WAVES * (LAND_BYTES + 2 * 2 * WV * 16 + ((DO + 1 + 7) / 8) * WV * 16) + ops_bytes(KB0) +
                              2 * (16 * DA * 2 + 16) * 4 + WAVES * 5 * 4;
    Args a = make_args(g, vec);
    const int n_tiles = a.B / TS;
    int grid = (n_tiles + WAVES - 1) / WAVES;
    if (grid > 256) grid = 256;
    const size_t need = (size_t)grid * N::P * sizeof(float);
    if (ws_bytes < need) return set_error(RL_ERR_ARG, "policy pass workspace too small: %zu < %zu bytes", ws_bytes, need);
    a.partial = (float*)ws;
    auto kern = fvp_splith_kernel<DO, DA, WPS>;
    static bool attr_set = false;
    if (!attr_set) {
        hipError_t e = hipFuncSetAttribute(reinterpret_cast<const void*>(kern), hipFuncAttributeMaxDynamicSharedMemorySize,
                                           LDS_BYTES);
        if (e != hipSuccess) return set_error(RL_ERR_HIP, "hipFuncSetAttribute: %s", hipGetErrorString(e));
        attr_set = true;
    }
    hipLaunchKernelGGL(kern, dim3(grid), dim3(WAVES * WV), LDS_BYTES, st, a);
    int rc = check_launch("fvp_splith_kernel");
    if (rc) return rc;
    return launch_reduce_rows(a.partial, grid, N::P, out, st);
}

template <int DO, int DA>
static int launch64(const rl_policy_batch* g, const float* vec, void* ws, size_t ws_bytes, double* out, hipStream_t st) {
    using N = Net<DO, DA, 64>;
    constexpr int HT = 2, WAVES = 4;
    constexpr int KB0 = (DO + 1 + 15) / 16;
    constexpr int N_OPS = HT * KB0 + 3 * HT * 2 * HT;
    constexpr int LDS_BYTES = WAVES * (2 * 64 * TS * 4 + TS * 8 * 4) + N_OPS * 3 * WV * 16 + 2 * (HT * 16 * DA * 2 + HT * 16) * 4 +
                              WAVES * 5 * 4;
    Args a = make_args(g, vec);
    const int n_tiles = a.B / TS;
    int grid = (n_tiles + WAVES - 1) / WAVES;
    if (grid > 256) grid = 256;
    const size_t need = (size_t)grid * N::P * sizeof(float);
    if (ws_bytes < need) return set_error(RL_ERR_ARG, "policy pass workspace too small: %zu < %zu bytes", ws_bytes, need);
    a.partial = (float*)ws;
    auto kern = fvp_splith64_kernel<DO, DA>;
    static bool attr_set = false;
    if (!attr_set) {
        hipError_t e = hipFuncSetAttribute(reinterpret_cast<const void*>(kern), hipFuncAttributeMaxDynamicSharedMemorySize,
                                           LDS_BYTES);
        if (e != hipSuccess) return set_error(RL_ERR_HIP, "hipFuncSetAttribute: %s", hipGetErrorString(e));
        attr_set = true;
    }
    hipLaunchKernelGGL(kern, dim3(grid), dim3(WAVES * WV), LDS_BYTES, st, a);
    int rc = check_launch("fvp_splith64_kernel");
    if (rc) return rc;
    return launch_reduce_rows(a.partial, grid, N::P, out, st);
}

}

#define SPLITH_SHAPES(X) X(4, 1) X(6, 1) X(11, 1) X(13, 2) X(13, 1) X(20, 3) X(20, 6) X(21, 6)
#define SPLITH64_SHAPES(X) X(4, 1) X(6, 1) X(11, 1) X(13, 2) X(20, 3) X(20, 6) X(21, 6)
bool split_fvp_takes(const rl_policy_batch* g);
bool splith_fvp_takes(const rl_policy_batch* g) {
    if (!split_fvp_takes(g) || !g->obs_absmax) return false;
    const int req = g->opts ? g->opts->fvp_split : 0;
    if (req != 0 && req != 4) return false;
    if (g->opts && g->opts->fvp_split_wps == 1) return false;
#define SPLITCASE(DO, DA) if (g->obs_dim == DO && g->act_dim == DA) return true;
    if (g->hidden0 == 64) { SPLITH64_SHAPES(SPLITCASE) }
    else { SPLITH_SHAPES(SPLITCASE) }
#undef SPLITCASE
    return false;
}
int splith_fvp_dispatch(const rl_policy_batch* g, const float* vec, void* ws, size_t ws_bytes, double* out, hipStream_t st) {
    if (!splith_fvp_takes(g)) return RL_SPLIT_NOT_TAKEN;
    if (g->hidden0 == 64) {
#define SPLITCASE(DO, DA) if (g->obs_dim == DO && g->act_dim == DA) return splith::launch64<DO, DA>(g, vec, ws, ws_bytes, out, st);
        SPLITH64_SHAPES(SPLITCASE)
#undef SPLITCASE
        return RL_SPLIT_NOT_TAKEN;
    }
#define SPLITCASE(DO, DA) if (g->obs_dim == DO && g->act_dim == DA) return splith::launch32<DO, DA>(g, vec, ws, ws_bytes, out, st);
    SPLITH_SHAPES(SPLITCASE)
#undef SPLITCASE
    return RL_SPLIT_NOT_TAKEN;
}

}
```

rllab_amd/envs/hip_env.py:

```python
import ctypes
import math

import numpy as np
import torch

from rllab_amd import _lib, spaces
from rllab_amd.core.serializable import Serializable
from rllab_amd.envs.base import Env, Step
from rllab_amd.misc import ext
from rllab_amd.sampler.trajectories import Trajectories

BIG = 1e6


def _require_device():
    if not torch.cuda.is_available():
        raise RuntimeError("rllab_amd: no HIP device visible -- env kernels have no CPU fallback")
    return torch.device("cuda", torch.cuda.current_device())


def _fresh_seed():
    s = ext.get_seed()
    if s is None:
        s = int(np.random.randint(0, 2 ** 31 - 1))
# ... 117 lines not shown
        out = torch.empty((4, self.n), dtype=torch.float32, device=self.device)
        _lib.check(_lib.lib.rl_vecenv_com(self.kind, self.n, _lib.ptr(self.state), _lib.ptr(out), _lib.stream_ptr()),
                   "rl_vecenv_com")
        return out.t()

    def get_state(self):
        return self.state.t().cpu().numpy().astype(np.float64)

    def set_state(self, state):
        st = torch.as_tensor(np.asarray(state, dtype=np.float32).reshape(self.n, self.q["state_dim"]))
        self.state.copy_(st.t().contiguous())
        self.ts.zero_()
        self.observe()

    def takes_rollout_of(self, policy):
        if getattr(policy, "recurrent", False):
            return self._takes_recurrent_rollout_of(policy)
        return self.rollout_plan(policy) is not None

    def _takes_recurrent_rollout_of(self, policy):
        if not hasattr(policy, "rollout_layout") or policy.rollout_layout() is None:
            return False
        if self.position_ids is not None:
            raise NotImplementedError("Box2DEnv(position_only=True) with a recurrent policy: the recurrent rollout kernel "
                                      "feeds the GRU the full observation")
        return True

    def rollout_plan(self, policy, horizon=None, norm=None):
        layout = policy.kernel_layout() if hasattr(policy, "kernel_layout") else None
        dual = policy.rollout_networks() if (layout is None and hasattr(policy, "rollout_networks")) else None
        if layout is None and dual is None:
            return None
        T = int(horizon if horizon is not None else max(1, self.max_path_length))
        flags = int(self.cfg.flags)
        hs, hs_std = (layout.hidden3, (0, 0, 0)) if layout is not None else (tuple(dual[1]), tuple(dual[3]))
        _lib.launch_opts()
        acts = layout.layer_activations if layout is not None else int(dual[4])
        acts_std = 0 if layout is not None else int(dual[5])
        key = (hs, hs_std, T, flags, acts, acts_std, norm, float(self.cfg.obs_noise), bytes(_lib._OPTS))
        cache = self.__dict__.setdefault("_plan_cache", {})
        if key not in cache:
            if len(cache) > 64:
                cache.clear()
            cache[key] = _lib.rollout_plan(self.kind, self.n, T, hs, hs_std, cfg_flags=flags, layer_activations=acts,
                                           norm=norm, obs_noise=float(self.cfg.obs_noise), std_layer_activations=acts_std)
        return cache[key]

    def _first_layer_on_full_obs(self, theta, h0):
        kept, do = len(self.position_ids), self.q["obs_dim"]
        w0 = torch.zeros((do, h0), dtype=torch.float32, device=self.device)
        w0.index_copy_(0, self._pos_index, theta[:kept * h0].view(kept, h0))
        return torch.cat([w0.view(-1), theta[kept * h0:]])

    def rollout(self, policy, horizon, reset_at_start=True, eps=None, reset_draws=None, action_noise_z=None,
                obs_noise_z=None, norm=None, scale_reward=None):
        if getattr(policy, "recurrent", False):
            if norm is not None:
                raise NotImplementedError("NormalizedEnv(normalize_obs / normalize_reward) with a recurrent policy: the "
                                          "running estimates are not built into the recurrent rollout kernel")
            return self._rollout_recurrent(policy, horizon, reset_at_start, eps, reset_draws, action_noise_z, obs_noise_z,
                                           scale_reward)
        if self.position_ids is not None and norm is not None:
            raise NotImplementedError("position_only observations under running normalisation: the estimates are over "
                                      "the kept rows; sample through the per-transition path")
        T, n = int(horizon), self.n
        do, da = self.q["obs_dim"], self.q["act_dim"]
        layout = policy.kernel_layout() if hasattr(policy, "kernel_layout") else None
        dual = policy.rollout_networks() if (layout is None and hasattr(policy, "rollout_networks")) else None
        if layout is None and dual is None:
            raise NotImplementedError("fused rollout needs a GaussianMLPPolicy with two or three tanh hidden layers of "
                                      "at most 128 units (policies/kernel_layout.py)")
        hs = layout.hidden3 if dual is None else dual[1]
        dev = self.device
        f32 = dict(dtype=torch.float32, device=dev)
        obs = torch.empty((do, T, n), **f32)
        act = torch.empty((da, T, n), **f32)
        mean = torch.empty((da, T, n), **f32)
        rew = torch.empty((T, n), **f32)
        done = torch.empty((T, n), dtype=torch.uint8, device=dev)
        theta = layout.theta() if dual is None else dual[0]
        theta_std = None if dual is None else dual[2]
        hs_std = (0, 0, 0) if dual is None else dual[3]
        log_stds = None if dual is None else torch.empty((da, T, n), **f32)
        if self.position_ids is not None:
            theta = self._first_layer_on_full_obs(theta, hs[0])
            if theta_std is not None:
                theta_std = self._first_layer_on_full_obs(theta_std, hs_std[0])
        assert theta.is_cuda and theta.dtype == torch.float32 and theta.is_contiguous()
        if eps is not None:
            eps = torch.as_tensor(eps, **f32).contiguous()
            assert eps.shape == (da, T, n)
        if reset_draws is not None:
            reset_draws = torch.as_tensor(reset_draws, **f32).contiguous()
            assert reset_draws.shape == (T + 1, self.q["reset_draws"], n)
        az = self._plane(action_noise_z, (T, da, n))
        oz = self._plane(obs_noise_z, (T + 1, do, n))
        log_min_std = math.log(policy.min_std) if policy.min_std is not None else -1e30
        self._cfg_with(az, oz)
        args = _lib.RolloutArgs(
            kind=self.kind, n_envs=n, horizon=T, max_path_length=self.max_path_length,
            normalize=int(self.normalize), reset_at_start=int(reset_at_start),
            hidden0=hs[0], hidden1=hs[1], hidden2=hs[2], env_offset=self.env_offset,
            scale_reward=self.scale_reward, log_min_std=log_min_std, seed=self.seed,
            step_counter=self.step_counter,
            state=self.state.data_ptr(), ts=self.ts.data_ptr(), theta=theta.data_ptr(),
            eps=eps.data_ptr() if eps is not None else None,
            reset_draws=reset_draws.data_ptr() if reset_draws is not None else None,
            obs=obs.data_ptr(), actions=act.data_ptr(), means=mean.data_ptr(),
            rewards=rew.data_ptr(), dones=done.data_ptr(), last_obs=self._obs.data_ptr(),
            cfg=ctypes.pointer(self.cfg),
            theta_std=None if theta_std is None else theta_std.data_ptr(),
            log_stds=None if log_stds is None else log_stds.data_ptr(),
            std_hidden0=hs_std[0], std_hidden1=hs_std[1], std_hidden2=hs_std[2],
            layer_activations=layout.layer_activations if layout is not None else int(dual[4]),
            std_layer_activations=0 if dual is None else int(dual[5]), opts=_lib.launch_opts())
        if scale_reward is not None:
            args.scale_reward = float(scale_reward)
        nrm = None
        if norm is not None:
            nrm = _lib.RunningNorm(
                obs_mean=norm.obs_mean.data_ptr(), obs_var=norm.obs_var.data_ptr(),
                reward_mean=norm.reward_mean.data_ptr(), reward_var=norm.reward_var.data_ptr(),
                obs_alpha=norm.obs_alpha, reward_alpha=norm.reward_alpha,
                normalize_obs=int(norm.normalize_obs), normalize_reward=int(norm.normalize_reward))
            args.norm = ctypes.addressof(nrm)
        _lib.check(_lib.lib.rl_rollout_gaussian_mlp(ctypes.byref(args), _lib.stream_ptr()),
                   "rl_rollout_gaussian_mlp")
        self.step_counter += T + 1
        if self._pos_index is not None:
            obs = obs.index_select(0, self._pos_index)
        return Trajectories(obs, act, mean, policy.recorded_log_std(), rew, done,
                            self.max_path_length, log_std_planes=log_stds)

    def _rollout_recurrent(self, policy, horizon, reset_at_start, eps, reset_draws, action_noise_z, obs_noise_z,
                           scale_reward):
        if not self._takes_recurrent_rollout_of(policy):
            why = policy.why_no_rollout_kernel() if hasattr(policy, "why_no_rollout_kernel") else None
            raise NotImplementedError("no recurrent rollout kernel for this policy: %s" % (
                why or "%s is not a GaussianGRUPolicy" % type(policy).__name__))
        T, n = int(horizon), self.n
        do, da = self.q["obs_dim"], self.q["act_dim"]
        assert (policy.obs_dim, policy.action_dim) == (do, da), "policy built for another env"
        H = policy.kernel_hidden
        theta = policy.rollout_layout()
        assert theta.is_cuda and theta.dtype == torch.float32 and theta.is_contiguous()
        f32 = dict(dtype=torch.float32, device=self.device)
        if getattr(self, "hidden_state", None) is None or tuple(self.hidden_state.shape) != (H, n):
            if not reset_at_start:
                raise ValueError("rollout(reset_at_start=False) of a recurrent policy needs the hidden state a previous "
                                 "launch of that policy left on this executor")
            self.hidden_state = torch.zeros((H, n), **f32)
            self.prev_action = torch.zeros((da, n), **f32)
        obs = torch.empty((do, T, n), **f32)
        act = torch.empty((da, T, n), **f32)
        mean = torch.empty((da, T, n), **f32)
        rew = torch.empty((T, n), **f32)
        done = torch.empty((T, n), dtype=torch.uint8, device=self.device)
        eps = self._plane(eps, (da, T, n))
        reset_draws = self._plane(reset_draws, (T + 1, self.q["reset_draws"], n))
        az = self._plane(action_noise_z, (T, da, n))
        oz = self._plane(obs_noise_z, (T + 1, do, n))
        self._cfg_with(None, None)
        args = _lib.GruRolloutArgs(
            kind=self.kind, n_envs=n, horizon=T, max_path_length=self.max_path_length, normalize=int(self.normalize),
            reset_at_start=int(bool(reset_at_start)), hidden=H, include_action=int(policy.state_include_action),
            env_offset=self.env_offset, scale_reward=self.scale_reward if scale_reward is None else float(scale_reward),
            seed=self.seed, step_counter=self.step_counter,
            state=self.state.data_ptr(), ts=self.ts.data_ptr(), last_obs=self._obs.data_ptr(),
            hidden_state=self.hidden_state.data_ptr(), prev_action=self.prev_action.data_ptr(), theta=theta.data_ptr(),
            eps=None if eps is None else eps.data_ptr(),
            reset_draws=None if reset_draws is None else reset_draws.data_ptr(),
            act_noise_z=None if az is None else az.data_ptr(), obs_noise_z=None if oz is None else oz.data_ptr(),
            obs=obs.data_ptr(), actions=act.data_ptr(), means=mean.data_ptr(), rewards=rew.data_ptr(),
            dones=done.data_ptr(), cfg=ctypes.pointer(self.cfg), opts=_lib.launch_opts())
        _lib.check(_lib.lib.rl_rollout_gaussian_gru(ctypes.byref(args), _lib.stream_ptr()), "rl_rollout_gaussian_gru")
        self.step_counter += T + 1
        return Trajectories(obs, act, mean, policy.recorded_log_std(), rew, done, self.max_path_length,
                            prev_action_info=bool(policy.state_include_action))

    def rollout_population(self, theta_pop, n_evals, horizon, discount, record=True, eps=None, reset_draws=None,
                           action_noise_z=None, obs_noise_z=None, layer_activations=0, log_min_std=None):
# ... 144 lines not shown
```

rllab_amd/policies/fused_ops.py:

```python
import ctypes
import math
import os

import torch

from rllab_amd import _lib
from rllab_amd.core.serializable import Serializable
from rllab_amd.misc.device_io import read_async
from rllab_amd.policies.update_batch import GaussianBatch
from rllab_amd.sampler import dist as D


class FusedGaussianMLPOps(object):
    device_line_search = True

    def __init__(self, policy):
        layout = policy.kernel_layout()
        assert layout is not None
        self._bind(policy, layout, (policy.obs_dim, policy.action_dim) + layout.hidden3)
        self.wide_kernels = layout.wide or (policy.obs_dim, policy.action_dim) not in self.NARROW_PAIRS

    def _bind(self, policy, layout, dims):
        self.policy, self.layout, self.dims = policy, layout, dims
        self.n_kernel = layout.P_pad
        self._ws = None
        self._loss_cache = None
        self._bound = {}
        self._acts = None
        self._absmax = None
        self._acts_tag = None

    @property
    def _epoch(self):
        return getattr(self.policy, "_raw_writes", 0)

    @_epoch.setter
    def _epoch(self, value):
        self.policy._raw_writes = value

    NARROW_PAIRS = ((4, 1), (6, 1), (11, 1), (13, 2), (20, 3), (20, 6), (21, 6))

    @staticmethod
    def supported(policy):
        layout = policy.kernel_layout() if hasattr(policy, "kernel_layout") else None
        return layout is not None

    def accepts(self, inputs):
        if len(inputs) != len(GaussianBatch._fields):
            return False
        b = GaussianBatch._make(inputs)
        return b.old_log_std.numel() == self.dims[1] and b.obs.is_cuda

    def _workspace(self, device):
        if self._ws is None or self._ws.device != device:
            n = _lib.lib.rl_policy_workspace_bytes(*self.dims)
            self._ws = torch.empty(n, dtype=torch.uint8, device=device)
        return self._ws

    def _batch(self, inputs):
        self.layout.theta()
        key = tuple(id(t) for t in inputs)
        hit = self._bound.get(key)
        if hit is not None:
            return hit
        named = GaussianBatch._make(inputs)
        theta = self.layout.theta()
        keep = [t.contiguous() for t in (named.obs, named.actions, named.advantages, named.old_mean,
                                         named.old_log_std.reshape(-1).float(), named.weights, theta)]
        obs, act, adv, old_mean, old_ls, w, theta = keep
        assert theta.data_ptr() == self.layout.theta().data_ptr()
        pol = self.policy
        inv = float(named.inv_count)
        b = _lib.PolicyBatch(
            n_samples=obs.shape[-1], obs_dim=self.dims[0], act_dim=self.dims[1], hidden0=self.dims[2],
            hidden1=self.dims[3], hidden2=self.dims[4], inv_count=inv,
            log_min_std=math.log(pol.min_std) if pol.min_std is not None else -1e30,
            theta=theta.data_ptr(), obs=obs.data_ptr(), actions=act.data_ptr(), advantages=adv.data_ptr(),
            old_means=old_mean.data_ptr(), old_log_std=old_ls.data_ptr(), weights=w.data_ptr(),
            layer_activations=self.layout.layer_activations,
            opts=_lib.launch_opts())
        if len(self._bound) >= 2:
            self._bound.clear()
        self._bound[key] = (b, keep + list(inputs), inv)
# ... 19 lines not shown
            return c
        b, keep, inv = self._batch(inputs)
        ws = self._workspace(keep[0].device)
        out = torch.empty(4, dtype=torch.float64, device=keep[0].device)
        _lib.check(_lib.lib.rl_policy_loss_kl(ctypes.byref(b), _lib.ptr(ws), ws.numel(), _lib.ptr(out),
                                              _lib.stream_ptr()), "rl_policy_loss_kl")
        return self._loss_record(tag, out, inv)

    @staticmethod
    def _resolve(c):
        if c["host"] is None:
            h = c["read"].get().reshape(-1, 4)
            sums = h[:, :3].sum(axis=0) * c["inv"]
            c["host"] = (float(sums[0]), float(sums[1]), float(sums[2]), float(h[:, 3].max()))
        return c["host"]

    def loss_stats(self, inputs):
        c = self._loss_eval(inputs)
        if c["dev"] is None:
            c["dev"] = torch.as_tensor(self._resolve(c), dtype=torch.float64, device=c["out"].device)
        return c["dev"]

    def loss_stats_host(self, inputs):
        return self._resolve(self._loss_eval(inputs))

    def loss_and_kl(self, inputs):
        s = self.loss_stats_host(inputs)
        return -s[0], s[1]

    def loss_stats_deferred(self, inputs):
        c = self._loss_eval(inputs)
        return lambda: self._resolve(c)

    def loss_and_kl_deferred(self, inputs):
        c = self._loss_eval(inputs)

        def get():
            s = self._resolve(c)
            return -s[0], s[1]
        get.record = c
        return get

    def _eval_point(self, inputs):
        return (tuple(id(t) for t in inputs), self.policy.flat_params._version, self._epoch)

    def loss_grad(self, inputs, vpg=False, keep_activations=False, with_loss=False):
        b, keep, inv = self._batch(inputs)
        ws = self._workspace(keep[0].device)
        out = torch.empty(self.n_kernel, dtype=torch.float64, device=keep[0].device)
        self._acts_tag = None
        b.activations = None
        need = _lib.lib.rl_policy_activation_bytes(b.n_samples, self.dims[2], self.dims[3], self.dims[4]) \
            if keep_activations and not vpg else 0
        if need:
            if self._acts is None or self._acts.numel() < need or self._acts.device != keep[0].device:
                self._acts = torch.empty(need, dtype=torch.uint8, device=keep[0].device)
            b.activations = self._acts.data_ptr()
            if self._absmax is None or self._absmax.device != keep[0].device:
                self._absmax = torch.zeros(1, dtype=torch.float32, device=keep[0].device)
            b.obs_absmax = self._absmax.data_ptr()
        tag = self._eval_point(inputs)
        have_loss = self._loss_cache is not None and self._loss_cache["tag"] == tag
        try:
            if with_loss and not have_loss:
                both = torch.empty(self.n_kernel + 4, dtype=torch.float64, device=keep[0].device)
                out, out4 = both[:self.n_kernel], both[self.n_kernel:]
                _lib.check(_lib.lib.rl_policy_grad_loss(ctypes.byref(b), int(vpg), _lib.ptr(ws), ws.numel(),
                                                        _lib.ptr(out), _lib.ptr(out4), _lib.stream_ptr()),
                           "rl_policy_grad_loss")
                if D.is_distributed() and D.peer_reducer() is None:
                    rows = D.all_gather_rows(both)
                    self._loss_record(tag, out4, inv, rows=rows[:, self.n_kernel:].contiguous())
                    if b.activations:
                        self._acts_tag = tag
                    return self._mask_frozen(self.layout.unpack(rows[:, :self.n_kernel].sum(dim=0)))
                self._loss_record(tag, out4, inv)
            else:
                _lib.check(_lib.lib.rl_policy_grad(ctypes.byref(b), int(vpg), _lib.ptr(ws), ws.numel(),
                                                   _lib.ptr(out), _lib.stream_ptr()), "rl_policy_grad")
            if b.activations:
                self._acts_tag = tag
        finally:
            b.activations = None
            b.obs_absmax = None
        return self._mask_frozen(self.layout.unpack(D.update_sum_(out)))

    @property
    def masks_frozen(self):
        return self._frozen_index() is not None

    def _frozen_index(self):
        if not hasattr(self, "_frozen_idx"):
            pol = self.policy
            tr = pol._flat_index(trainable=True)
            if tr is None:
                self._frozen_idx = None
            else:
                keep = torch.ones(pol.flat_params.numel(), dtype=torch.bool, device=pol.flat_params.device)
                keep[tr] = False
                self._frozen_idx = torch.nonzero(keep).reshape(-1)
        return self._frozen_idx

    def _mask_frozen(self, g):
        idx = self._frozen_index()
        if idx is not None:
            g.index_fill_(0, idx, 0.0)
        return g

    def value_and_grad(self, inputs, penalty=0.0, vpg=False):
        assert not (vpg and penalty), "the log-likelihood objective has no KL penalty"
        b, keep, inv = self._batch(inputs)
        dev = keep[0].device
        ws = self._workspace(dev)
        grad = torch.empty(self.n_kernel, dtype=torch.float64, device=dev)
        out4 = torch.empty(4, dtype=torch.float64, device=dev)
        self._acts_tag = None
        b.activations = None
        b.kl_penalty = float(penalty)
        try:
            _lib.check(_lib.lib.rl_policy_grad_loss(ctypes.byref(b), int(bool(vpg)), _lib.ptr(ws), ws.numel(),
                                                    _lib.ptr(grad), _lib.ptr(out4), _lib.stream_ptr()),
                       "rl_policy_grad_loss")
# ... 206 lines not shown
```

rllab_amd/sampler/vectorized_sampler.py:

```python
import math
import os
import time

import torch

import rllab_amd.misc.logger as logger
from rllab_amd import _lib
from rllab_amd.sampler import dist as D
from rllab_amd.sampler.base import BaseSampler
from rllab_amd.sampler.trajectories import PathList, Trajectories


class VectorizedSampler(BaseSampler):
    def __init__(self, algo, n_envs=None, seed=None, use_graph=True):
        super(VectorizedSampler, self).__init__(algo)
        self.n_envs = n_envs
        self.seed = seed
        self.use_graph = use_graph
        self.vec_env = None
        self.last_sample_time = None
        self.last_num_samples = None

    def start_worker(self):
        algo = self.algo
# ... 43 lines not shown
            elif getattr(policy, "state_dependent_std", False):
                why = "the policy's two networks have no rollout kernel (each: two or three tanh layers of at most 128 units)"
            elif hasattr(policy, "why_no_kernel_layout"):
                why = policy.why_no_kernel_layout()
            else:
                why = "%s is not a GaussianMLPPolicy" % type(policy).__name__
        graph = self.use_graph and getattr(ve, "graphable", True) and not os.environ.get("RLLAB_NO_GRAPH") \
            and hasattr(policy, "recorded_log_std")
        name = "per-transition loop (%s), one policy evaluation + one env-step launch per step" % (
            "hipGraph replay" if graph else "eager")
        return name, why

    def shutdown_worker(self):
        if self.vec_env is not None:
            self.vec_env.terminate()

    def __getstate__(self):
        d = dict(self.__dict__)
        d["vec_env"] = None
        d.pop("_step_graph", None)
        d.pop("_prefetched", None)
        d.pop("_carry_obs", None)
        d.pop("_launch_start", None)
        return d

    def _takes_fused_rollout(self, policy):
        ve = self.vec_env
        if ve is None:
            return False
        if hasattr(ve, "takes_rollout_of"):
            return ve.takes_rollout_of(policy)
        return (hasattr(policy, "kernel_layout") and policy.kernel_layout() is not None) or \
            (hasattr(policy, "rollout_networks") and policy.rollout_networks() is not None)

    def prefetch(self, itr):
        policy = self.algo.policy
        pre = getattr(self, "_prefetched", None)
        if pre is not None and pre[0] == itr and hasattr(policy, "param_version") and pre[1] == policy.param_version():
            return
        self._drop_prefetched()
        if not hasattr(policy, "param_version") or not self._takes_fused_rollout(policy):
            return
        if getattr(self.vec_env, "stateful_rollouts", False):
            return
        counter = self.vec_env.step_counter
        first = self._rollout_chunk(policy, self.algo.max_path_length, True)
        self._prefetched = (itr, policy.param_version(), first, counter)

    def _drop_prefetched(self):
        pre = getattr(self, "_prefetched", None)
        self._prefetched = None
        if pre is not None and self.vec_env is not None:
            self.vec_env.step_counter = pre[3]

    def obtain_samples(self, itr):
        algo = self.algo
        policy = algo.policy
        pre = getattr(self, "_prefetched", None)
        first = None
        if pre is not None:
            if pre[0] == itr and pre[1] is not None and pre[1] == policy.param_version():
                first = pre[2]
                self._prefetched = None
            else:
                self._drop_prefetched()
        t_start = time.time()
        if first is None:
            first = self._launch(policy, algo.max_path_length, True)
        traj = self._meet_batch_size(policy, first)
        self.last_num_samples = traj.B
        self.last_sample_time = time.time() - t_start
        return PathList(traj)

    def _rollout_chunk(self, policy, steps, first):
        graphable = getattr(self.vec_env, "graphable", True)
        if self._takes_fused_rollout(policy):
            return self.vec_env.rollout(policy, steps, reset_at_start=first)
        if self.use_graph and graphable and not os.environ.get("RLLAB_NO_GRAPH") and hasattr(policy, "recorded_log_std"):
            try:
                return self._stepwise_rollout_graph(policy, steps, first)
            except RuntimeError as err:
                logger.log("hipGraph capture of the per-transition loop failed (%s); using the eager loop"
                           % str(err).split("\n")[0])
                self.use_graph = False
                self._step_graph = None
                torch.cuda.synchronize()
        return self._stepwise_rollout(policy, steps, first)

    MAX_STALLED_CHUNKS = 8

    def _launch(self, policy, steps, first):
        v = self.vec_env
        self._launch_start = None
        if getattr(v, "stateful_rollouts", False):
            self._launch_start = (v.snapshot(), getattr(self, "_carry_obs", None), bool(first))
        return self._rollout_chunk(policy, steps, first)

    def _commit_first_steps(self, policy, chunk, steps):
        start = getattr(self, "_launch_start", None)
        if start is None:
            return
        v = self.vec_env
        snap, carry, first = start
        v.restore(snap)
        self._carry_obs = carry
        self._launch_start = None
        if self._takes_fused_rollout(policy):
            self._rollout_chunk(policy, steps, first)
            return
        obs = v.reset() if first else carry
        for t in range(steps):
            obs = v.step(chunk.actions[:, t, :].t())[0]
        self._carry_obs = obs

    def _path_index(self, traj):
        T, N = traj.T, traj.N
        tin = torch.empty((T, N), dtype=torch.int32, device=traj.device)
        valid = torch.empty((T, N), dtype=torch.uint8, device=traj.device)
        _lib.check(_lib.lib.rl_path_scan(T, N, 0, _lib.ptr(traj.dones), None, None, 1, _lib.ptr(tin), _lib.ptr(valid),
                                         None, _lib.stream_ptr()), "rl_path_scan")
        return tin, valid.view(torch.bool)

    def _finished_by_step(self, traj, carry=None):
        tin = self._path_index(traj)[0].to(torch.int64)
        done = traj.dones.to(torch.int64)
        if carry is not None:
            t_idx = torch.arange(traj.T, device=traj.device).unsqueeze(1)
            tin = tin + (tin == t_idx).to(torch.int64) * carry.unsqueeze(0)
            carry.copy_((tin[-1] + 1) * (1 - done[-1]))
# ... 178 lines not shown
```

Before: 287.2 million.

## Record hidden activations during swimmer rollout and reuse them in the policy gradient

The swimmer quad rollout kernel gains a recording variant for (32,32) tanh nets. It writes both hidden-layer activations, tiled in the layout the update kernels expect, to a buffer during sampling, and tracks the maximum absolute observation value. A new cached grad+loss entry point then reads those activations instead of recomputing the forward pass for the first gradient evaluation of the TRPO update. In exchange the rollout gains extra nontemporal stores and an atomic per wave. The sampler also needs versioning checks so it only uses recordings that match the current parameters and sample planes.

```diff
diff --git a/include/rllab_amd.h b/include/rllab_amd.h
--- a/include/rllab_amd.h
+++ b/include/rllab_amd.h
@@ -135,6 +135,8 @@
     const rl_running_norm* norm;
     int32_t std_layer_activations;
     int32_t reserved_tail;
+    float* activations;
+    float* obs_absmax;
 } rl_rollout_args;
 
 int rl_rollout_gaussian_mlp(const rl_rollout_args* args, void* stream);
@@ -398,6 +400,9 @@
 int rl_policy_grad_loss(const rl_policy_batch* batch, int vpg, void* workspace, size_t workspace_bytes,
                         double* grad_out, double* out4, void* stream);
 
+int rl_policy_grad_loss_cached(const rl_policy_batch* batch, const float* cotangent_bound, void* workspace,
+                               size_t workspace_bytes, double* grad_out, double* out4, void* stream);
+
 int rl_policy_fvp(const rl_policy_batch* batch, const float* vec, void* workspace,
                   size_t workspace_bytes, double* fvp_out, void* stream);
 
diff --git a/profiles/make_index.py b/profiles/make_index.py
--- a/profiles/make_index.py
+++ b/profiles/make_index.py
@@ -14,6 +14,14 @@
      "python tools/exp/categorical_gru_bptt_time.py --out profiles/categorical_gru_bptt_time.json"),
     ("update_batch_refactor_time.json", "parent commit against the update-batch / planes-ops refactor on one box, runs interleaved: headline bench (env steps/s, update phase) and whole TRPO iterations of GaussianMLPPolicy(adaptive_std=True) on Cartpole (1024 x 100) and CategoricalMLPPolicy on GridWorld (80 x 50); every run, medians, the parent's own spread",
      "python tools/exp/update_batch_refactor_ab.py --parent <built checkout of the parent> --out profiles/update_batch_refactor_time.json"),
+    ("recorded_acts_ab_*.jsonl", "parent tree and new tree alternately in one GPU session, one bench line each: the headline (seven lines) and cheetah1024_trpo_gae (four)",
+     "python bench.py --gpus 1 [--workload cheetah1024_trpo_gae] --steps 20 --warmup 3, in the parent's checkout and in this one by turns"),
+    ("recorded_acts_outputs_cmp.txt", "bench.py --dump-outputs of the parent and the new tree array by array, next to the parent's f16 against bf16 product arithmetic",
+     "python bench.py --gpus 1 --steps 3 --warmup 1 --dump-outputs DIR in both checkouts (and with RLLAB_FVP_SPLIT=5), numpy.array_equal + largest relative difference per array"),
+    ("curves/recorded_acts_swimmer.csv", "200 TRPO iterations of the headline configuration on the recording rollout + cached gradient",
+     "python examples/run_trpo.py --env swimmer --n-envs 4096 --n-itr 200 --hidden 32 --gae-lambda 1.0 --quiet --csv <file>"),
+    ("recorded_acts_before_kernel_stats.csv", "kernel stats of the parent of the recorded-activations change", "profiles/run_profile.sh recorded_acts swimmer4096_trpo recorded_acts_before stats"),
+    ("recorded_acts_after_*.csv", "kernel stats, counter passes and timeline at the recorded-activations sources", "profiles/run_profile.sh recorded_acts swimmer4096_trpo recorded_acts_after"),
     ("*_bench_line.json", "the default bench line of that tree", "python bench.py"),
     ("*_bench_under_rocprof.log", "bench stdout under the kernel-trace pass", "profiles/run_profile.sh <tag>"),
     ("*_c5_kernel_stats.csv", "kernel stats of C5's per-GPU shard", "profiles/run_profile.sh <tag> cheetah1024_trpo_gae"),
diff --git a/rllab_amd/_lib.py b/rllab_amd/_lib.py
--- a/rllab_amd/_lib.py
+++ b/rllab_amd/_lib.py
@@ -22,7 +22,7 @@
     "rl_gru_categorical_workspace_bytes", "rl_gru_categorical_eval", "rl_gru_categorical_grad", "rl_gru_categorical_fvp",
     "rl_rollout_population_gru", "rl_gae",
     "rl_discount_cumsum", "rl_debug_philox", "rl_policy_workspace_bytes", "rl_policy_activation_bytes", "rl_policy_loss_kl",
-    "rl_policy_grad", "rl_policy_grad_loss", "rl_policy_fvp", "rl_policy_fvp_variant", "rl_policy_fvp_cg_step", "rl_cg_init", "rl_cg_step", "rl_trpo_step", "rl_line_search_point", "rl_line_search_decide", "rl_adam_step",
+    "rl_policy_grad", "rl_policy_grad_loss", "rl_policy_grad_loss_cached", "rl_policy_fvp", "rl_policy_fvp_variant", "rl_policy_fvp_cg_step", "rl_cg_init", "rl_cg_step", "rl_trpo_step", "rl_line_search_point", "rl_line_search_decide", "rl_adam_step",
     "rl_path_scan", "rl_process_workspace_bytes", "rl_sample_stats_cols", "rl_sample_stats", "rl_adv_finish",
     "rl_lfb_normal_eq", "rl_reps_workspace_bytes", "rl_reps_dual", "rl_reps_weights",
     "rl_peer_mailbox_bytes", "rl_peer_alloc", "rl_peer_free", "rl_peer_export", "rl_peer_open", "rl_peer_close",
@@ -58,7 +58,8 @@
         ("theta_std", ctypes.c_void_p), ("log_stds", ctypes.c_void_p), ("std_hidden0", ctypes.c_int32),
         ("std_hidden1", ctypes.c_int32), ("std_hidden2", ctypes.c_int32), ("layer_activations", ctypes.c_int32),
         ("opts", ctypes.c_void_p), ("norm", ctypes.c_void_p), ("std_layer_activations", ctypes.c_int32),
-        ("reserved_tail", ctypes.c_int32),
+        ("reserved_tail", ctypes.c_int32), ("activations", ctypes.c_void_p),
+        ("obs_absmax", ctypes.c_void_p),
     ]
 
 
@@ -286,6 +287,7 @@
     lib.rl_policy_loss_kl.argtypes = [pb, vp, ctypes.c_size_t, vp, vp]
     lib.rl_policy_grad.argtypes = [pb, i32, vp, ctypes.c_size_t, vp, vp]
     lib.rl_policy_grad_loss.argtypes = [pb, i32, vp, ctypes.c_size_t, vp, vp, vp]
+    lib.rl_policy_grad_loss_cached.argtypes = [pb, vp, vp, ctypes.c_size_t, vp, vp, vp]
     lib.rl_policy_fvp.argtypes = [pb, vp, vp, ctypes.c_size_t, vp, vp]
     lib.rl_policy_fvp_variant.argtypes = [pb]
     lib.rl_policy_fvp_cg_step.argtypes = [pb, vp, ctypes.c_size_t, f64, f64, vp, vp, vp, vp, vp, vp, vp, vp]
diff --git a/rllab_amd/csrc/acts_layout.h b/rllab_amd/csrc/acts_layout.h
--- /dev/null
+++ b/rllab_amd/csrc/acts_layout.h
@@ -0,0 +1,30 @@
+#pragma once
+#include <cstddef>
+
+namespace rl {
+namespace acts_layout {
+
+constexpr int TILE_SAMPLES = 32;
+constexpr int CHUNK_BYTES = 16;
+constexpr int PIECE_BYTES = 64 * CHUNK_BYTES;
+constexpr int PIECES_PER_LAYER = 4;
+constexpr int TILE_BYTES = 2 * PIECES_PER_LAYER * PIECE_BYTES;
+
+constexpr size_t tile_offset(size_t tile) { return tile * (size_t)TILE_BYTES; }
+constexpr int chunk_offset(int layer, int q, int lh, int lj) {
+    return (layer * PIECES_PER_LAYER + q) * PIECE_BYTES + (lh * 32 + lj) * CHUNK_BYTES;
+}
+constexpr int chunk_unit(int q, int lh) { return 8 * q + 4 * lh; }
+
+constexpr int writer_unit(int tt, int g) { return 16 * tt + 4 * g; }
+constexpr int writer_q(int tt, int g) { return 2 * tt + (g >> 1); }
+constexpr int writer_lh(int g) { return g & 1; }
+constexpr int writer_chunk_offset(int layer, int tt, int g, int lj) {
+    return chunk_offset(layer, writer_q(tt, g), writer_lh(g), lj);
+}
+constexpr size_t writer_offset(size_t s, int layer, int tt, int g) {
+    return tile_offset(s >> 5) + (size_t)writer_chunk_offset(layer, tt, g, (int)(s & 31));
+}
+
+}
+}
diff --git a/rllab_amd/csrc/env_kernels.hip b/rllab_amd/csrc/env_kernels.hip
--- a/rllab_amd/csrc/env_kernels.hip
+++ b/rllab_amd/csrc/env_kernels.hip
@@ -8,6 +8,7 @@
 #include "policy_mfma.h"
 #include "policy_wide.h"
 #include "rollout_lane.h"
+#include "acts_layout.h"
 
 namespace rl {
 
@@ -263,11 +264,14 @@
     }
 
     __device__ __forceinline__ void forward16(const float* o, float* mean) const {
+        f32x4 h0[NT], h1[NT];
+        forward16_keep(o, mean, h0, h1);
+    }
+    __device__ __forceinline__ void forward16_keep(const float* o, float* mean, f32x4 (&h0)[NT], f32x4 (&h1)[NT]) const {
         float xb[KS0];
 #pragma unroll
         for (int m = 0; m < KS0; ++m)
             xb[m] = pick(input(o, 4 * m), input(o, 4 * m + 1), input(o, 4 * m + 2), input(o, 4 * m + 3));
-        f32x4 h0[NT], h1[NT];
 #pragma unroll
         for (int t = 0; t < NT; ++t) {
             f32x4 acc = {0.0f, 0.0f, 0.0f, 0.0f};
@@ -649,6 +653,8 @@
     double* nobs_mean; double* nobs_var; double* nrew_mean; double* nrew_var;
     double obs_alpha, rew_alpha;
     int norm_obs, norm_rew;
+    float* activations;
+    unsigned* obs_absmax;
 };
 
 template <class Env>
@@ -883,7 +889,7 @@
 #define RL_TWO_LEG_SUBSTEP_UNROLL 4
 #endif
 
-template <class Pol, bool COOP = false, bool PLAIN = false>
+template <class Pol, bool COOP = false, bool PLAIN = false, bool RECORD = false>
 __device__ __forceinline__ void swimmer_quad_body(const RolloutDev& a, const Pol& pol) {
     using Env = Swimmer;
     using Chain = Env::Chain;
@@ -936,6 +942,10 @@
     }
     uint32_t vo_row = (uint32_t)i * 4, vo_done = (uint32_t)i;
     asm volatile("" : "+v"(vo_row), "+v"(vo_done));
+    const bool rec_live = RECORD && i_raw < n;
+    uint32_t rec_sample = (uint32_t)i;
+    const uintptr_t rec_base = RECORD ? reinterpret_cast<uintptr_t>(a.activations) : 0;
+    float rec_xmax = 0.0f;
     typedef __attribute__((address_space(1))) float* global_f32;
     typedef __attribute__((address_space(1))) uint8_t* global_u8;
     auto at = [](uintptr_t row_ptr, uint32_t& byte_off) {
@@ -966,7 +976,26 @@
 #pragma unroll
             for (int k = 0; k < Env::ACT; ++k) z[k] = __shfl(zq[k], el + 16 * (t & 3), 64);
         }
-        pol.forward16(o, mean);
+        if constexpr (RECORD) {
+            static_assert(Pol::NT == 2 && !COOP, "the activation cache of the (32, 32) nets");
+            typedef __attribute__((address_space(1))) f32x4* global_f32x4;
+            f32x4 h0k[2], h1k[2];
+            pol.forward16_keep(o, mean, h0k, h1k);
+            if (rec_live) {
+#pragma unroll
+                for (int tt = 0; tt < 2; ++tt) {
+                    __builtin_nontemporal_store(h0k[tt], reinterpret_cast<global_f32x4>(
+                        rec_base + (uint32_t)acts_layout::writer_offset(rec_sample, 0, tt, lane >> 4)));
+                    __builtin_nontemporal_store(h1k[tt], reinterpret_cast<global_f32x4>(
+                        rec_base + (uint32_t)acts_layout::writer_offset(rec_sample, 1, tt, lane >> 4)));
+                }
+            }
+            rec_sample += (uint32_t)n;
+#pragma unroll
+            for (int k = 0; k < Env::OBS; ++k) rec_xmax = fmaxf(rec_xmax, fabsf(o[k]));
+        } else {
+            pol.forward16(o, mean);
+        }
 #pragma unroll
         for (int k = 0; k < Env::ACT; ++k) act[k] = __builtin_fmaf(z[k], std_[k], mean[k]);
         if (live) {
@@ -1058,14 +1087,20 @@
             for (int k = 0; k < Env::OBS; ++k) a.last_obs[(size_t)k * n + i] = o[k];
         }
     }
-}
-
-template <int H, bool ACTS = false, bool PLAIN = false>
+    if constexpr (RECORD) {
+        if (a.obs_absmax != nullptr) {
+            rec_xmax = wave_max(rec_xmax);
+            if (lane == 0) atomicMax(a.obs_absmax, __float_as_uint(rec_xmax));
+        }
+    }
+}
+
+template <int H, bool ACTS = false, bool PLAIN = false, bool RECORD = false>
 __global__ void __launch_bounds__(LANE_TPB) rollout_swimmer_quad_kernel(RolloutDev a) {
     RolloutPolicy16<Swimmer, H, ACTS> pol;
     pol.init(a.theta);
     pol.act0 = a.act0; pol.act1 = a.act1;
-    swimmer_quad_body<RolloutPolicy16<Swimmer, H, ACTS>, false, PLAIN>(a, pol);
+    swimmer_quad_body<RolloutPolicy16<Swimmer, H, ACTS>, false, PLAIN, RECORD>(a, pol);
 }
 
 __global__ void __launch_bounds__(LANE_TPB) rollout_swimmer_quad_wide_kernel(RolloutDev a, WideShape shape) {
@@ -1696,6 +1731,13 @@
     p->lds_limit = (int32_t)LDS_LIMIT;
     p->reserved = 0;
     snprintf(p->name, sizeof(p->name), "%s", name);
+}
+
+static bool records_activations(const rl_rollout_args* g) {
+    const size_t samples = (size_t)g->n_envs * (size_t)g->horizon;
+    return g->activations != nullptr && g->hidden0 == 32 && g->hidden1 == 32 && g->hidden2 == 0 &&
+           g->layer_activations == 0 && samples % acts_layout::TILE_SAMPLES == 0 &&
+           acts_layout::tile_offset(samples / acts_layout::TILE_SAMPLES) < ((size_t)1 << 32);
 }
 
 template <class Env>
@@ -1762,7 +1804,8 @@
     if constexpr (std::is_same<Env, Swimmer>::value) {
         const bool lane_kernel = o.swimmer_lane_kernel == 1 || (cfg_flags & RL_CFG_LIMIT_MUJOCO) != 0;
         if (!lane_kernel && small_offsets && equal) {
-            snprintf(nm, sizeof(nm), "rollout_swimmer_quad_kernel<%d>", g->hidden0);
+            snprintf(nm, sizeof(nm), records_activations(g) ? "rollout_swimmer_quad_kernel<%d, recording>"
+                                                            : "rollout_swimmer_quad_kernel<%d>", g->hidden0);
             plan_fill(p, RL_ROLLOUT_SWIMMER_QUAD, QUAD_ENVS, quad_waves, lane_group_wpb(quad_waves, o), 0, nm);
             return RL_OK;
         }
@@ -1860,6 +1903,8 @@
     a.act_noise_z = g->cfg ? g->cfg->action_noise_z : nullptr;
     a.obs_noise_z = g->cfg ? g->cfg->obs_noise_z : nullptr;
     a.log_stds = g->log_stds;
+    a.activations = nullptr;
+    a.obs_absmax = nullptr;
     a.act0 = layer_act(RL_ACT_TANH, g->layer_activations, 0);
     a.act1 = layer_act(RL_ACT_TANH, g->layer_activations, 1);
     const bool acts = a.act0 != RL_ACT_TANH || a.act1 != RL_ACT_TANH;
@@ -1922,7 +1967,16 @@
                                        a.cfg.action_noise == 0.0f && a.cfg.obs_noise == 0.0f;
 #define RL_SWQ(HH, AA) do { if (plain) hipLaunchKernelGGL((rollout_swimmer_quad_kernel<HH, AA, true>), grid, block, 0, st, a); \
                             else hipLaunchKernelGGL((rollout_swimmer_quad_kernel<HH, AA, false>), grid, block, 0, st, a); } while (0)
-                    if (H == 32 && !acts) RL_SWQ(32, false);
+                    if (records_activations(g)) {
+                        a.activations = g->activations;
+                        a.obs_absmax = reinterpret_cast<unsigned*>(g->obs_absmax);
+                        if (g->obs_absmax) {
+                            hipError_t e = hipMemsetAsync(g->obs_absmax, 0, sizeof(float), st);
+                            if (e != hipSuccess) return set_error(RL_ERR_HIP, "hipMemsetAsync(obs_absmax): %s", hipGetErrorString(e));
+                        }
+                        if (plain) hipLaunchKernelGGL((rollout_swimmer_quad_kernel<32, false, true, true>), grid, block, 0, st, a);
+                        else hipLaunchKernelGGL((rollout_swimmer_quad_kernel<32, false, false, true>), grid, block, 0, st, a);
+                    } else if (H == 32 && !acts) RL_SWQ(32, false);
                     else if (H == 32) RL_SWQ(32, true);
                     else if (!acts) RL_SWQ(64, false);
                     else RL_SWQ(64, true);
diff --git a/rllab_amd/csrc/policy_splith_kernels.hip b/rllab_amd/csrc/policy_splith_kernels.hip
--- a/rllab_amd/csrc/policy_splith_kernels.hip
+++ b/rllab_amd/csrc/policy_splith_kernels.hip
@@ -4,10 +4,12 @@
 #include "capi_util.h"
 #include "policy_mfma.h"
 #include "lds_tr_image.h"
+#include "acts_layout.h"
 
 namespace rl {
 
 int launch_reduce_rows(const float* partial, int rows, int cols, double* out, hipStream_t st);
+int launch_reduce_loss(const double* partial, int rows, double* out, hipStream_t st);
 
 namespace splith {
 
@@ -31,6 +33,11 @@
     float inv_count;
     float log_min_std;
     float* partial;
+    const float* act;
+    const float* mean;
+    const float* adv;
+    const float* gmax;
+    double* partial_loss;
 };
 
 struct PB { f16x8 hi, lo; };
@@ -241,6 +248,7 @@
     const int e = (int)((__float_as_uint(x) >> 23) & 255u) - 126;
     return e < -30 ? -30 : e;
 }
+__device__ __forceinline__ float inv_var(float log_std) { return __expf(-2.0f * log_std); }
 __device__ __forceinline__ float pow2(int e) { return __builtin_ldexpf(1.0f, e < -126 ? -126 : (e > 127 ? 127 : e)); }
 __device__ __forceinline__ float uniform(float v) { return __uint_as_float(__builtin_amdgcn_readfirstlane(__float_as_uint(v))); }
 __device__ __forceinline__ int imin(int a, int b) { return a < b ? a : b; }
@@ -281,6 +289,22 @@
     s.u0b = uniform(pow2(-(sg + e_w1 + kg + e_b + 8)));
     return s;
 }
+template <int HL, int DAL>
+__device__ __forceinline__ Scales make_scales_grad(float bx, float bw1, float bw2, float gmax, float inv_count) {
+    const int EW1 = exp_of(bw1), EW2 = exp_of(bw2), EG = exp_of(gmax);
+    const int e_x = 6 - exp_of(bx), e_b = imin(e_x, 5), e_w1 = 7 - EW1;
+    int sg = 15 - (DAL + EW2 + EG);
+    sg = sg < -100 ? -100 : (sg > 100 ? 100 : sg);
+    const int kg = -(HL + 7);
+    Scales s;
+    s.sx = uniform(pow2(e_x)); s.sb = uniform(pow2(e_b)); s.sw1 = uniform(pow2(e_w1));
+    s.sv0 = s.sv0b = s.s1 = 0.0f;
+    s.eg2 = uniform(pow2(sg)); s.kg = uniform(pow2(kg));
+    s.u1 = uniform(pow2(-sg) * inv_count);
+    s.u0 = uniform(pow2(-(sg + e_w1 + kg + e_x + 8)) * inv_count);
+    s.u0b = uniform(pow2(-(sg + e_w1 + kg + e_b + 8)) * inv_count);
+    return s;
+}
 template <class N, int NT>
 __device__ __forceinline__ void block_maxima(const float* __restrict__ th, const float* __restrict__ vc, float* red,
                                              float (&m)[5]) {
@@ -325,6 +349,7 @@
 constexpr int LAND_BYTES = 2 * H * TS * 4;
 constexpr int ops_count(int kb0) { return kb0 + 6; }
 constexpr int ops_bytes(int kb0) { return ops_count(kb0) * 3 * WV * 16; }
+constexpr int xland_bytes(int d_o, int d_a, bool grad) { return ((d_o + 1 + (grad ? 2 * d_a + 1 : 0) + 7) / 8) * WV * 16; }
 #ifndef RL_SPLITH_TWO_ACC
 #define RL_SPLITH_TWO_ACC 0
 #endif
@@ -333,7 +358,7 @@
 #endif
 constexpr float XT_SCALE = 256.0f;
 
-template <int DO, int DA, int WPS>
+template <int DO, int DA, int WPS, bool GRAD = false>
 __global__ void __launch_bounds__(4 * WPS * WV, 1) fvp_splith_kernel(Args a) {
     using N = Net<DO, DA, H>;
     constexpr int P = N::P;
@@ -342,10 +367,12 @@
     constexpr int N_OPS = ops_count(KB0), OPS_BYTES = ops_bytes(KB0);
     constexpr int TAILV = 16 * DA * 2 + 16;
     constexpr int SPILL_BYTES = 2 * lds_tr::TR_PART_BYTES;
-    constexpr int XPIECES = (DO + 1 + 7) / 8;
+    constexpr int R_ACT = DO + 1, R_MEAN = R_ACT + DA, R_ADV = R_MEAN + DA;
+    constexpr int XPIECES = ((GRAD ? R_ADV + 1 : DO + 1) + 7) / 8;
     constexpr int XLAND_BYTES = XPIECES * WV * 16;
     constexpr int WAVE_BYTES = LAND_BYTES + SPILL_BYTES + XLAND_BYTES;
     constexpr int LDS_TOTAL = WAVES * WAVE_BYTES + OPS_BYTES + 2 * TAILV * 4 + WAVES * 5 * 4;
+    static_assert(XLAND_BYTES == xland_bytes(DO, DA, GRAD), "the launcher's LDS size");
     static_assert(DO + 1 <= 32 && (DA <= 2 || WPS == 1), "two k-blocks of inputs + the bias slot; thin heads at two per SIMD");
     static_assert(LDS_TOTAL >= WAVES * P * 4 && LDS_TOTAL <= 160 * 1024, "LDS budget; the fold rows alias the landing zones");
     extern __shared__ __attribute__((aligned(16))) char smem[];
@@ -371,10 +398,19 @@
         for (int p = 0; p < XPIECES; ++p) {
             const int d = 8 * p + (lane >> 3);
             const float* g = (d < DO ? a.obs + (size_t)d * B : a.weight) + tile * TS + 4 * (lane & 7);
+            if constexpr (GRAD)
+                g = (d < DO ? a.obs + (size_t)d * B
+                            : d >= R_ACT && d < R_MEAN ? a.act + (size_t)(d - R_ACT) * B
+                            : d >= R_MEAN && d < R_ADV ? a.mean + (size_t)(d - R_MEAN) * B : d == R_ADV ? a.adv : a.weight) +
+                    tile * TS + 4 * (lane & 7);
             asm volatile("s_mov_b32 m0, %1\n\tglobal_load_lds_dwordx4 %0, off" :: "v"(g), "s"(xland_lds + p * (WV * 16)) : "memory");
         }
     };
     const unsigned land_lds = __builtin_amdgcn_readfirstlane((unsigned)(size_t)(lptr_t)land);
+    static_assert(acts_layout::TILE_BYTES == 8 * WV * 16 && acts_layout::chunk_offset(0, 1, 0, 0) == 1024 &&
+                  acts_layout::chunk_offset(1, 0, 0, 0) == 4 * WV * 16 && acts_layout::chunk_offset(0, 0, 1, 5) == (32 + 5) * 16 &&
+                  acts_layout::chunk_unit(3, 1) == frag_unit(4 * 3, 1) && acts_layout::chunk_unit(1, 0) + 2 == frag_unit(4 + 2, 0),
+                  "fetch_acts reads the cache as acts_layout.h lays it out");
     auto fetch_acts = [&](int tile) {
         const float* src = a.acts + ((size_t)tile * 8 * WV + lane) * 4;
         asm volatile("s_mov_b32 m0, %2\n\t"
@@ -398,6 +434,7 @@
     const float* __restrict__ th = a.theta;
     const float* __restrict__ vc = a.vec;
     float db2[DA], fkS[DA], var_[DA];
+    float lstd_[DA], ivar[DA];
     bool floored[DA];
     float fkmax = 0.0f;
 #pragma unroll
@@ -408,21 +445,29 @@
         var_[k] = __expf(2.0f * ls);
         fkS[k] = 2.0f / (2.0f * var_[k] + 1e-8f) * a.inv_count;
         fkmax = fmaxf(fkmax, fkS[k]);
+        lstd_[k] = ls;
+        ivar[k] = inv_var(ls);
     }
     float mx[5];
-    block_maxima<N, WAVES * WV>(th, vc, red, mx);
-    const Scales S = make_scales<5, ceil_log2(DA)>(*a.xmax, mx[0], mx[1], mx[2], mx[3], mx[4], fkmax);
-#pragma unroll
-    for (int k = 0; k < DA; ++k) {
-        fkS[k] *= S.eg2;
-        db2[k] = vc[N::B2 + k] * S.s1;
-    }
-
-    for (int o = wave; o < N_OPS; o += WAVES) {
+    if constexpr (GRAD) block_maxima<N, WAVES * WV>(th, th, red, mx);
+    else block_maxima<N, WAVES * WV>(th, vc, red, mx);
+    const Scales S = GRAD ? make_scales_grad<5, ceil_log2(DA)>(*a.xmax, mx[3], mx[4], *a.gmax, a.inv_count)
+                          : make_scales<5, ceil_log2(DA)>(*a.xmax, mx[0], mx[1], mx[2], mx[3], mx[4], fkmax);
+    if constexpr (!GRAD) {
+#pragma unroll
+        for (int k = 0; k < DA; ++k) {
+            fkS[k] *= S.eg2;
+            db2[k] = vc[N::B2 + k] * S.s1;
+        }
+    }
+
+    for (int o = (GRAD ? KB0 + 4 : 0) + wave; o < N_OPS; o += WAVES) {
         float t[8];
 #pragma unroll
         for (int j = 0; j < 8; ++j) {
-            if (o < KB0) {
+            if constexpr (GRAD) {
+                t[j] = th[N::W1 + lj * H + frag_unit(8 * ((o - KB0) & 1) + j, lh)] * S.sw1;
+            } else if (o < KB0) {
                 const int d = 16 * o + 8 * lh + j;
                 t[j] = d < DO ? vc[N::W0 + d * H + lj] * S.sv0 : (d == DO ? vc[N::B0 + lj] * S.sv0b : 0.0f);
             } else {
@@ -443,9 +488,9 @@
 #pragma unroll
         for (int k = 0; k < DA; ++k) {
             tv[k * 16 + r] = th[N::W2 + u * DA + k];
-            tv[(DA + k) * 16 + r] = vc[N::W2 + u * DA + k] * S.s1;
-        }
-        tv[2 * DA * 16 + r] = vc[N::B1 + u] * S.s1;
+            if constexpr (!GRAD) tv[(DA + k) * 16 + r] = vc[N::W2 + u * DA + k] * S.s1;
+        }
+        if constexpr (!GRAD) tv[2 * DA * 16 + r] = vc[N::B1 + u] * S.s1;
     }
     __syncthreads();
     auto op = [&](int o) -> PA {
@@ -477,6 +522,8 @@
 
     f32x16 gW1, gW0, gW1c, gW0c;
     float gW2l[16][DA], gb1l[16], gb2[DA], wsum = 0.0f;
+    float gls[DA];
+    double acc_loss = 0.0, acc_vpg = 0.0;
 #pragma unroll
     for (int r = 0; r < 16; ++r) {
         gW1[r] = 0.0f; gW0[r] = 0.0f; gW1c[r] = 0.0f; gW0c[r] = 0.0f; gb1l[r] = 0.0f;
@@ -484,7 +531,7 @@
         for (int k = 0; k < DA; ++k) gW2l[r][k] = 0.0f;
     }
 #pragma unroll
-    for (int k = 0; k < DA; ++k) gb2[k] = 0.0f;
+    for (int k = 0; k < DA; ++k) { gb2[k] = 0.0f; gls[k] = 0.0f; }
 
     __builtin_amdgcn_s_waitcnt(0x0F70);
     for (int tile = wave_global; tile < n_tiles; tile += waves_total) {
@@ -509,6 +556,13 @@
                     xb[kb][j] = d < DO ? v * S.sx : (d == DO ? S.sb : 0.0f);
                 }
             wgt = xl[32 * DO];
+        }
+        float advb = 0.0f, dmu_[DA];
+        if constexpr (GRAD) {
+            const float* xl = reinterpret_cast<const float*>(xland) + lj;
+            advb = xl[32 * R_ADV];
+#pragma unroll
+            for (int k = 0; k < DA; ++k) dmu_[k] = xl[32 * (R_ACT + k)] - xl[32 * (R_MEAN + k)];
         }
         asm volatile("s_waitcnt lgkmcnt(0)" ::: "memory");
         {
@@ -523,7 +577,8 @@
         const float* tv = tailv + lh * TAILV;
         auto stage = [&]() { asm volatile("" ::: "memory"); };
 
-        PA opcur = op(0);
+        PA opcur;
+        if constexpr (!GRAD) opcur = op(0);
         __builtin_amdgcn_sched_barrier(0);
         PB Xs[KB0], H0s[2];
 #pragma unroll
@@ -531,6 +586,39 @@
         split_frag(h0, H0s);
 
         f32x16 acc;
+        f32x16 dz1, gz1;
+        float gmu[DA];
+        auto rows_of = [&](int which, int k, f32x4 (&out_)[4]) {
+#pragma unroll
+            for (int q = 0; q < 4; ++q) out_[q] = *reinterpret_cast<const f32x4*>(tv + (which * DA + k) * 16 + 4 * q);
+        };
+        if constexpr (GRAD) {
+            wave_sync();
+            tr_store(tr_w, H0s);
+#pragma unroll
+            for (int j = 0; j < 8; ++j) {
+                const f32x2 hh = pair_of(h1, j);
+                set_pair(dz1, j, __builtin_elementwise_fma(-hh, hh, f32x2{1.0f, 1.0f}));
+            }
+            const float c = -(wgt * advb);
+            float zz = 0.0f, sls = 0.0f;
+#pragma unroll
+            for (int k = 0; k < DA; ++k) {
+                const float t = c * (dmu_[k] * ivar[k]);
+                gmu[k] = t * S.eg2;
+                const float z2 = (dmu_[k] * dmu_[k]) * ivar[k];
+                zz += z2;
+                sls += lstd_[k];
+                if (lh == 0 && !floored[k]) gls[k] = __builtin_fmaf(c, z2 - 1.0f, gls[k]);
+            }
+            if (lh == 0) {
+                const float logp = -sls - 0.5f * zz;
+                acc_loss += (double)(wgt * advb);
+                acc_vpg += (double)(wgt * (logp - 0.5f * (float)DA * 1.8378770664093453f) * advb);
+#pragma unroll
+                for (int k = 0; k < DA; ++k) gb2[k] += gmu[k];
+            }
+        } else {
 #pragma unroll
         for (int r = 0; r < 16; ++r) acc[r] = 0.0f;
         acc = chain_ahead(0, KB0, Xs, acc, opcur, KB0);
@@ -548,8 +636,6 @@
             acc = chain_ahead(KB0 + 2, 2, D0s, acc, opcur, -1);
         }
         stage();
-        f32x16 dz1, gz1;
-        float gmu[DA];
 #pragma unroll
         for (int j = 0; j < 8; ++j) {
             const f32x2 hh = pair_of(h1, j);
@@ -557,10 +643,6 @@
             set_pair(dz1, j, d);
             set_pair(acc, j, pair_of(acc, j) * d);
         }
-        auto rows_of = [&](int which, int k, f32x4 (&out_)[4]) {
-#pragma unroll
-            for (int q = 0; q < 4; ++q) out_[q] = *reinterpret_cast<const f32x4*>(tv + (which * DA + k) * 16 + 4 * q);
-        };
 #pragma unroll
         for (int k = 0; k < DA; ++k) {
             f32x4 wq[4], dq[4];
@@ -582,6 +664,7 @@
             wsum += wgt * a.inv_count;
 #pragma unroll
             for (int k = 0; k < DA; ++k) gb2[k] += gmu[k];
+        }
         }
         stage();
         {
@@ -671,9 +754,9 @@
             w2s[r][k] = w;
         }
     }
-    float b2s[DA];
-#pragma unroll
-    for (int k = 0; k < DA; ++k) b2s[k] = wave_sum(gb2[k]);
+    float b2s[DA], lss[DA];
+#pragma unroll
+    for (int k = 0; k < DA; ++k) { b2s[k] = wave_sum(gb2[k]); lss[k] = GRAD ? wave_sum(gls[k]) : 0.0f; }
     const float ws = wave_sum(wsum);
     __syncthreads();
     float* const myrow = reinterpret_cast<float*>(smem) + wave * P;
@@ -699,9 +782,13 @@
 #pragma unroll
         for (int k = 0; k < DA; ++k) {
             myrow[N::B2 + k] = b2s[k] * S.u1;
-            const float vv = var_[k], e = 1e-8f;
-            const float cc = floored[k] ? 0.0f : 4.0f * vv * (2.0f * vv - e) / ((2.0f * vv + e) * (2.0f * vv + e));
-            myrow[N::LSTD + k] = cc * vc[N::LSTD + k] * ws;
+            if constexpr (GRAD) {
+                myrow[N::LSTD + k] = lss[k] * a.inv_count;
+            } else {
+                const float vv = var_[k], e = 1e-8f;
+                const float cc = floored[k] ? 0.0f : 4.0f * vv * (2.0f * vv - e) / ((2.0f * vv + e) * (2.0f * vv + e));
+                myrow[N::LSTD + k] = cc * vc[N::LSTD + k] * ws;
+            }
         }
     }
     __syncthreads();
@@ -711,6 +798,19 @@
 #pragma unroll
         for (int w = 0; w < WAVES; ++w) t += reinterpret_cast<const float*>(smem)[w * P + k];
         row[k] = t;
+    }
+    if constexpr (GRAD) {
+        const double l = wave_sum(acc_loss), v = wave_sum(acc_vpg);
+        __syncthreads();
+        double* const redl = reinterpret_cast<double*>(smem);
+        if (lane == 0) { redl[2 * wave] = l; redl[2 * wave + 1] = v; }
+        __syncthreads();
+        if (threadIdx.x < 4) {
+            double t = 0.0;
+            if ((threadIdx.x & 1) == 0)
+                for (int w = 0; w < WAVES; ++w) t += redl[2 * w + (threadIdx.x >> 1)];
+            a.partial_loss[(size_t)blockIdx.x * 4 + threadIdx.x] = t;
+        }
     }
 }
 
@@ -1199,6 +1299,72 @@
     return launch_reduce_rows(a.partial, grid, N::P, out, st);
 }
 
+template <int DA>
+__global__ void __launch_bounds__(256) grad_bound_kernel(int B, const float* __restrict__ act, const float* __restrict__ mean,
+                                                         const float* __restrict__ adv, const float* __restrict__ weight,
+                                                         const float* __restrict__ log_std, float log_min_std,
+                                                         unsigned* __restrict__ out) {
+    float iv[DA], m = 0.0f;
+#pragma unroll
+    for (int k = 0; k < DA; ++k) iv[k] = inv_var(fmaxf(log_std[k], log_min_std));
+    for (int b = blockIdx.x * blockDim.x + threadIdx.x; b < B; b += gridDim.x * blockDim.x) {
+        const float c = -(weight[b] * adv[b]);
+#pragma unroll
+        for (int k = 0; k < DA; ++k) m = fmaxf(m, fabsf(c * ((act[(size_t)k * B + b] - mean[(size_t)k * B + b]) * iv[k])));
+    }
+    m = wave_max(m);
+    if (threadIdx.x % WV == 0) atomicMax(out, __float_as_uint(m));
+}
+
+template <int DO, int DA>
+static int launch32_grad(const rl_policy_batch* g, const float* bound, void* ws, size_t ws_bytes, double* out, double* out4,
+                         hipStream_t st) {
+    using N = Net<DO, DA, H>;
+    constexpr int WPS = DA <= 2 ? 2 : 1;
+    constexpr int WAVES = 4 * WPS;
+    constexpr int KB0 = (DO + 1 + 15) / 16;
+    constexpr int LDS_BYTES = WAVES * (LAND_BYTES + 2 * 2 * WV * 16 + xland_bytes(DO, DA, true)) + ops_bytes(KB0) +
+                              2 * (16 * DA * 2 + 16) * 4 + WAVES * 5 * 4;
+    Args a = make_args(g, nullptr);
+    a.act = g->actions; a.mean = g->old_means; a.adv = g->advantages;
+    const int n_tiles = a.B / TS;
+    int grid = (n_tiles + WAVES - 1) / WAVES;
+    if (grid > 256) grid = 256;
+    const size_t row_bytes = (((size_t)grid * N::P * sizeof(float)) + 15) & ~(size_t)15;
+    const size_t loss_bytes = (size_t)grid * 4 * sizeof(double);
+    const size_t need = row_bytes + loss_bytes + sizeof(float);
+    if (ws_bytes < need) return set_error(RL_ERR_ARG, "policy pass workspace too small: %zu < %zu bytes", ws_bytes, need);
+    a.partial = (float*)ws;
+    a.partial_loss = (double*)((char*)ws + row_bytes);
+    a.gmax = bound;
+    if (!bound) {
+        float* own = (float*)((char*)ws + row_bytes + loss_bytes);
+        hipError_t e = hipMemsetAsync(own, 0, sizeof(float), st);
+        if (e != hipSuccess) return set_error(RL_ERR_HIP, "hipMemsetAsync(cotangent bound): %s", hipGetErrorString(e));
+        int bg = (a.B + 255) / 256;
+        if (bg > 1024) bg = 1024;
+        hipLaunchKernelGGL(grad_bound_kernel<DA>, dim3(bg), dim3(256), 0, st, a.B, a.act, a.mean, a.adv, a.weight,
+                           a.theta + N::LSTD, a.log_min_std, reinterpret_cast<unsigned*>(own));
+        int rc = check_launch("grad_bound_kernel");
+        if (rc) return rc;
+        a.gmax = own;
+    }
+    auto kern = fvp_splith_kernel<DO, DA, WPS, true>;
+    static bool attr_set = false;
+    if (!attr_set) {
+        hipError_t e = hipFuncSetAttribute(reinterpret_cast<const void*>(kern), hipFuncAttributeMaxDynamicSharedMemorySize,
+                                           LDS_BYTES);
+        if (e != hipSuccess) return set_error(RL_ERR_HIP, "hipFuncSetAttribute: %s", hipGetErrorString(e));
+        attr_set = true;
+    }
+    hipLaunchKernelGGL(kern, dim3(grid), dim3(WAVES * WV), LDS_BYTES, st, a);
+    int rc = check_launch("fvp_splith_kernel<grad>");
+    if (rc) return rc;
+    rc = launch_reduce_rows(a.partial, grid, N::P, out, st);
+    if (rc) return rc;
+    return launch_reduce_loss(a.partial_loss, grid, out4, st);
+}
+
 }
 
 #define SPLITH_SHAPES(X) X(4, 1) X(6, 1) X(11, 1) X(13, 2) X(13, 1) X(20, 3) X(20, 6) X(21, 6)
@@ -1229,4 +1395,23 @@
     return RL_SPLIT_NOT_TAKEN;
 }
 
-}
+bool splith_grad_takes(const rl_policy_batch* g) {
+    return g->activations && g->obs_absmax && g->hidden0 == 32 && g->hidden1 == 32 && g->hidden2 == 0 &&
+           g->activation == RL_ACT_TANH && g->layer_activations == 0 && g->kl_penalty == 0.0f && g->n_samples % TS == 0 &&
+           g->obs_dim == 13 && g->act_dim == 2;
+}
+
+}
+
+extern "C" int rl_policy_grad_loss_cached(const rl_policy_batch* g, const float* cotangent_bound, void* workspace,
+                                          size_t workspace_bytes, double* grad_out, double* out4, void* stream) {
+    using namespace rl;
+    if (!g || g->n_samples <= 0 || !g->theta || !g->obs || !g->weights || !g->actions || !g->advantages || !g->old_means ||
+        !grad_out || !out4 || !workspace)
+        return set_error(RL_ERR_ARG, "rl_policy_grad_loss_cached: bad argument");
+    if (!splith_grad_takes(g))
+        return set_error(RL_ERR_UNSUPPORTED, "rl_policy_grad_loss_cached: needs activations and obs_absmax, two tanh layers of "
+                         "32 units on (obs 13, act 2), whole 32-sample tiles and no KL penalty (obs %d act %d hidden %d,%d,%d "
+                         "samples %d)", g->obs_dim, g->act_dim, g->hidden0, g->hidden1, g->hidden2, g->n_samples);
+    return splith::launch32_grad<13, 2>(g, cotangent_bound, workspace, workspace_bytes, grad_out, out4, (hipStream_t)stream);
+}
diff --git a/rllab_amd/envs/hip_env.py b/rllab_amd/envs/hip_env.py
--- a/rllab_amd/envs/hip_env.py
+++ b/rllab_amd/envs/hip_env.py
@@ -193,8 +193,10 @@
         w0.index_copy_(0, self._pos_index, theta[:kept * h0].view(kept, h0))
         return torch.cat([w0.view(-1), theta[kept * h0:]])
 
+    records_activations = True
+
     def rollout(self, policy, horizon, reset_at_start=True, eps=None, reset_draws=None, action_noise_z=None,
-                obs_noise_z=None, norm=None, scale_reward=None):
+                obs_noise_z=None, norm=None, scale_reward=None, record=None):
         if getattr(policy, "recurrent", False):
             if norm is not None:
                 raise NotImplementedError("NormalizedEnv(normalize_obs / normalize_reward) with a recurrent policy: the "
@@ -257,6 +259,16 @@
             std_layer_activations=0 if dual is None else int(dual[5]), opts=_lib.launch_opts())
         if scale_reward is not None:
             args.scale_reward = float(scale_reward)
+        bufs = None
+        if record is not None and dual is None and self.position_ids is None:
+            bufs = record.recording_buffers(T * n, dev)
+        if bufs is not None:
+            args.activations, args.obs_absmax = bufs[0].data_ptr(), bufs[1].data_ptr()
+            plan = _lib.RolloutPlan()
+            if _lib.lib.rl_rollout_plan_query(ctypes.byref(args), ctypes.byref(plan)) != 0 or \
+                    not plan.name.endswith(b"recording>"):
+                args.activations = args.obs_absmax = None
+                bufs = None
         nrm = None
         if norm is not None:
             nrm = _lib.RunningNorm(
@@ -268,6 +280,8 @@
         _lib.check(_lib.lib.rl_rollout_gaussian_mlp(ctypes.byref(args), _lib.stream_ptr()),
                    "rl_rollout_gaussian_mlp")
         self.step_counter += T + 1
+        if bufs is not None:
+            record.recorded(bufs, obs, act, mean)
         if self._pos_index is not None:
             obs = obs.index_select(0, self._pos_index)
         return Trajectories(obs, act, mean, policy.recorded_log_std(), rew, done,
diff --git a/rllab_amd/policies/fused_ops.py b/rllab_amd/policies/fused_ops.py
--- a/rllab_amd/policies/fused_ops.py
+++ b/rllab_amd/policies/fused_ops.py
@@ -29,6 +29,40 @@
         self._acts = None
         self._absmax = None
         self._acts_tag = None
+        self._rec_buf = None
+        self._recorded = None
+
+    def recording_buffers(self, n_samples, device):
+        if tuple(self.dims) != (13, 2, 32, 32, 0) or self.layout.layer_activations != 0 or n_samples % 32 != 0:
+            return None
+        need = _lib.lib.rl_policy_activation_bytes(n_samples, 32, 32, 0)
+        if need == 0 or need >= 1 << 32:
+            return None
+        buf = self._rec_buf
+        if buf is None or buf[0].numel() < need or buf[0].device != device:
+            self._rec_buf = None
+            buf = (torch.empty(need, dtype=torch.uint8, device=device), torch.zeros(1, dtype=torch.float32, device=device))
+        self._rec_buf = buf
+        self._recorded = None
+        if self._acts is buf[0]:
+            self._acts_tag = None
+        return buf
+
+    def recorded(self, bufs, obs, actions, means):
+        self._recorded = dict(bufs=bufs, planes=(obs, actions, means),
+                              version=(self.policy.flat_params._version, self._epoch))
+
+    def drop_recorded(self):
+        self._recorded = None
+
+    def _recorded_for(self, keep):
+        rec = self._recorded
+        if rec is None or rec["version"] != (self.policy.flat_params._version, self._epoch):
+            return None
+        for mine, theirs in zip((keep[0], keep[1], keep[3]), rec["planes"]):
+            if mine.data_ptr() != theirs.data_ptr() or mine.numel() != theirs.numel() or mine.dtype != theirs.dtype:
+                return None
+        return rec["bufs"]
 
     @property
     def _epoch(self):
@@ -154,22 +188,31 @@
         b.activations = None
         need = _lib.lib.rl_policy_activation_bytes(b.n_samples, self.dims[2], self.dims[3], self.dims[4]) \
             if keep_activations and not vpg else 0
-        if need:
+        tag = self._eval_point(inputs)
+        have_loss = self._loss_cache is not None and self._loss_cache["tag"] == tag
+        rec = self._recorded_for(keep) if need and with_loss and not have_loss else None
+        if rec is not None:
+            self._acts, self._absmax = rec
+            b.activations, b.obs_absmax = rec[0].data_ptr(), rec[1].data_ptr()
+        elif need:
             if self._acts is None or self._acts.numel() < need or self._acts.device != keep[0].device:
                 self._acts = torch.empty(need, dtype=torch.uint8, device=keep[0].device)
             b.activations = self._acts.data_ptr()
             if self._absmax is None or self._absmax.device != keep[0].device:
                 self._absmax = torch.zeros(1, dtype=torch.float32, device=keep[0].device)
             b.obs_absmax = self._absmax.data_ptr()
-        tag = self._eval_point(inputs)
-        have_loss = self._loss_cache is not None and self._loss_cache["tag"] == tag
         try:
             if with_loss and not have_loss:
                 both = torch.empty(self.n_kernel + 4, dtype=torch.float64, device=keep[0].device)
                 out, out4 = both[:self.n_kernel], both[self.n_kernel:]
-                _lib.check(_lib.lib.rl_policy_grad_loss(ctypes.byref(b), int(vpg), _lib.ptr(ws), ws.numel(),
-                                                        _lib.ptr(out), _lib.ptr(out4), _lib.stream_ptr()),
-                           "rl_policy_grad_loss")
+                if rec is not None:
+                    _lib.check(_lib.lib.rl_policy_grad_loss_cached(ctypes.byref(b), None, _lib.ptr(ws), ws.numel(),
+                                                                   _lib.ptr(out), _lib.ptr(out4), _lib.stream_ptr()),
+                               "rl_policy_grad_loss_cached")
+                else:
+                    _lib.check(_lib.lib.rl_policy_grad_loss(ctypes.byref(b), int(vpg), _lib.ptr(ws), ws.numel(),
+                                                            _lib.ptr(out), _lib.ptr(out4), _lib.stream_ptr()),
+                               "rl_policy_grad_loss")
                 if D.is_distributed() and D.peer_reducer() is None:
                     rows = D.all_gather_rows(both)
                     self._loss_record(tag, out4, inv, rows=rows[:, self.n_kernel:].contiguous())
diff --git a/rllab_amd/sampler/vectorized_sampler.py b/rllab_amd/sampler/vectorized_sampler.py
--- a/rllab_amd/sampler/vectorized_sampler.py
+++ b/rllab_amd/sampler/vectorized_sampler.py
@@ -119,6 +119,24 @@
         self._prefetched = None
         if pre is not None and self.vec_env is not None:
             self.vec_env.step_counter = pre[3]
+            ops = getattr(getattr(self.algo, "optimizer", None), "_fused", None)
+            if hasattr(ops, "drop_recorded"):
+                ops.drop_recorded()
+
+    def _update_ops_to_record_for(self, policy, steps, first):
+        algo, v = self.algo, self.vec_env
+        opt = getattr(algo, "optimizer", None)
+        ops = getattr(opt, "_fused", None)
+        if ops is None or not hasattr(ops, "recording_buffers") or getattr(ops, "policy", None) is not policy:
+            return None
+        if not getattr(v, "records_activations", False) or getattr(opt, "_subsample_factor", 1) < 1:
+            return None
+        T = int(algo.max_path_length)
+        if not first or steps != T or getattr(v, "terminates", True):
+            return None
+        if int(algo.batch_size) * D.world_size() > v.n * D.world_size() * T:
+            return None
+        return ops
 
     def obtain_samples(self, itr):
         algo = self.algo
@@ -142,6 +160,9 @@
     def _rollout_chunk(self, policy, steps, first):
         graphable = getattr(self.vec_env, "graphable", True)
         if self._takes_fused_rollout(policy):
+            ops = self._update_ops_to_record_for(policy, steps, first)
+            if ops is not None:
+                return self.vec_env.rollout(policy, steps, reset_at_start=first, record=ops)
             return self.vec_env.rollout(policy, steps, reset_at_start=first)
         if self.use_graph and graphable and not os.environ.get("RLLAB_NO_GRAPH") and hasattr(policy, "recorded_log_std"):
             try:
```

After: 289.4 million, median of 6. Within noise of the previous version (+0.7%).
